# facebookresearch/baspacho

Measured on AMD Instinct MI355X. Metric: factor_gflops_fp64_bal871_schur, higher is better.
Workload: dtype f64; 1 GPU; bal871; description=synthetic BAL-871 stand-in: 871 cams x 9, 527480 pts x 3, 2789783 obs, order=1590279, matrices_per_gpu=1, batch=1, numeric_data=mock: uniform(-1,1) seed 37(+q), damp(0, 1.2*order), as the reference's benches, parallelism=one matrix per GPU x1 (replicas; a single factorisation is not sharded)

## Files before the change

### baspacho_amd/__init__.py

```python
import ctypes
from dataclasses import dataclass
from typing import Optional, Sequence

import numpy as np

from . import _lib

__all__ = ["Settings", "Solver", "Assembly", "create_solver", "SparseStructure", "BackendHip", "BackendCuda",
           "BackendRef", "BackendFast", "AddFillComplete", "AddFillForAutoElims",
           "AddFillForGivenElims", "AddFillNone"]

BackendRef, BackendFast, BackendCuda, BackendHip = 0, 1, 2, 3
AddFillComplete, AddFillForAutoElims, AddFillForGivenElims, AddFillNone = 0, 1, 2, 3

_I64P = ctypes.POINTER(ctypes.c_int64)

_SKEL_IDS = {
    "spanStart": 0, "spanToLump": 1, "lumpStart": 2, "lumpToSpan": 3, "spanOffsetInLump": 4,
    "chainColPtr": 5, "chainRowSpan": 6, "chainData": 7, "chainRowsTillEnd": 8,
    "boardColPtr": 9, "boardRowLump": 10, "boardChainColOrd": 11, "boardRowPtr": 12,
    "boardColLump": 13, "boardColOrd": 14,
}

PROF_KINDS = ["elim_factor", "elim_update", "potrf", "trsm", "update", "chain_update"]


class _CSettings(ctypes.Structure):
    _fields_ = [("find_sparse_elimination_ranges", ctypes.c_int32),
                ("num_threads", ctypes.c_int32), ("backend", ctypes.c_int32),
                ("add_fill_policy", ctypes.c_int32),
                ("computation_model", ctypes.POINTER(ctypes.c_double))]


_HIP_OPTION_INTS = ["lookahead", "due_stream", "split_k", "gather_max_pairs", "gather_overlap",
                    "sub_batch_min", "sub_batches", "tail_blocks", "lazy_plan", "block_solve", "solve_inv",
                    "solve_sweep", "sweep_min_width", "solve_wide", "chain_contraction", "dense_merge", "expected_batch"]
_HIP_OPTION_REALS = ["lookahead_min_gf", "bulk_ahead", "level_cost_us"]


class _CHipOptions(ctypes.Structure):
    _fields_ = [(n, ctypes.c_int32) for n in _HIP_OPTION_INTS] + [(n, ctypes.c_double) for n in _HIP_OPTION_REALS]


class _CPlanStats(ctypes.Structure):
    _fields_ = [(n, ctypes.c_double) for n in
                ["flops", "upd_elems", "upd_flops", "elim_pair_elems", "elim_pair_flops",
                 "elim_col_elems", "upd_flops_direct", "elim_pair_operand_elems",
                 "elim_target_elems", "trsm_flops", "potrf_flops", "trsm_flops_merged",
                 "potrf_flops_fused"]] + \
               [(n, ctypes.c_int64) for n in
                ["num_launches", "num_levels", "num_panels", "num_segs", "num_upd_tasks",
                 "num_trsm_tasks", "chain_tab_entries", "max_panels_in_level",
                 "num_atomic_upd_tasks", "num_gather_groups", "num_fork_levels"]] + \
               [("deferred_flops", ctypes.c_double), ("tail_upd_flops", ctypes.c_double),
                ("num_tail_panels", ctypes.c_int64)]


class _CRunCounters(ctypes.Structure):
    _fields_ = [(n, ctypes.c_int64) for n in
                ["sweep_launches", "sweep_timeouts", "split_lists_used", "sub_batches_enqueued",
                 "lookahead_forks", "sweeps_retired", "sweep_error_pending",
                 "gather_chunks_overlapped", "tail_launches", "sweep_mfma_launches",
                 "solve_wide_launches", "inv_reused", "potrf_folded_levels", "selinv_launches",
                 "selinv_chunks"]]


@dataclass
class Settings:
    findSparseEliminationRanges: bool = True
    numThreads: int = 16
    backend: int = BackendHip
    addFillPolicy: int = AddFillComplete
    computationModel: Optional[Sequence[float]] = None
    hipOptions: Optional[dict] = None


@dataclass
class SparseStructure:
    ptrs: np.ndarray
    inds: np.ndarray

    def __post_init__(self):
        self.ptrs = np.ascontiguousarray(self.ptrs, dtype=np.int64)
        self.inds = np.ascontiguousarray(self.inds, dtype=np.int64)

    def order(self):
        return len(self.ptrs) - 1

    def transpose(self):
        return _ss_op(self, SS_TRANSPOSE)

    def clear(self, clearLower=True):
        return _ss_op(self, SS_CLEAR, flag=int(clearLower))

    def symmetricPermutation(self, mapPerm, lowerHalf=True):
        return _ss_op(self, SS_SYM_PERMUTATION, mapPerm, int(lowerHalf))

    def addIndependentEliminationFill(self, start, end):
        return _ss_op(self, SS_INDEP_ELIM_FILL, [start, end])

    def addFullEliminationFill(self):
        return _ss_op(self, SS_FULL_ELIM_FILL)

    def fillReducingPermutation(self):
        return _ss_op(self, SS_FILL_REDUCING_PERM)

    def extractRightBottom(self, start):
        return _ss_op(self, SS_EXTRACT_RIGHT_BOTTOM, [start])


SS_TRANSPOSE, SS_CLEAR, SS_SYM_PERMUTATION, SS_INDEP_ELIM_FILL, SS_FULL_ELIM_FILL, \
    SS_FILL_REDUCING_PERM, SS_EXTRACT_RIGHT_BOTTOM = range(7)


def _ss_op(ss, op, arg=(), flag=0):
    lib = _lib.load()
    n = ss.order()
    a = _i64(arg)
    cap = max(16, 4 * len(ss.inds) + n)
    while True:
        out_ptrs = np.zeros(n + 2, dtype=np.int64)
        out_inds = np.zeros(cap, dtype=np.int64)
        on, onnz = ctypes.c_int64(0), ctypes.c_int64(0)
        rc = lib.bsp_sparse_structure_op(
            op, ctypes.c_int64(n), ss.ptrs.ctypes.data_as(_I64P), ss.inds.ctypes.data_as(_I64P),
            a.ctypes.data_as(_I64P), ctypes.c_int64(len(a)), ctypes.c_int32(flag),
            out_ptrs.ctypes.data_as(_I64P), out_inds.ctypes.data_as(_I64P), ctypes.c_int64(cap),
            ctypes.byref(on), ctypes.byref(onnz))
        if rc != 0 and onnz.value > cap:
            cap = onnz.value
            continue
        _check(rc)
        if op == SS_FILL_REDUCING_PERM:
            return out_inds[:onnz.value].copy()
        return SparseStructure(out_ptrs[:on.value + 1].copy(), out_inds[:onnz.value].copy())


def _check(rc):
    if rc != 0:
        raise RuntimeError(_lib.load().bsp_last_error().decode("utf-8", "replace"))


def _i64(a):
    return np.ascontiguousarray(a, dtype=np.int64)


def _ptr_of(t):
# ... 85 lines not shown
        _check(self._lib.bsp_skeleton_array(self._h, which, ctypes.byref(p), ctypes.byref(n)))
        if n.value == 0:
            return np.zeros(0, dtype=np.int64)
        return np.ctypeslib.as_array(p, shape=(n.value,)).copy()

    def skel(self):
        if self._skel is None:
            self._skel = {k: self._array(v) for k, v in _SKEL_IDS.items()}
        return self._skel

    def paramToSpan(self):
        return self._array(15)

    def sparseEliminationRanges(self):
        return self._array(16)

    def blockOffset(self, row_param, col_param):
        off, st, fl = ctypes.c_int64(0), ctypes.c_int64(0), ctypes.c_int32(0)
        _check(self._lib.bsp_block_offset(self._h, ctypes.c_int64(row_param),
                                          ctypes.c_int64(col_param), ctypes.byref(off),
                                          ctypes.byref(st), ctypes.byref(fl)))
        return off.value, st.value, bool(fl.value)

    def diagBlockOffset(self, param):
        off, st = ctypes.c_int64(0), ctypes.c_int64(0)
        _check(self._lib.bsp_diag_block_offset(self._h, ctypes.c_int64(param), ctypes.byref(off),
                                               ctypes.byref(st)))
        return off.value, st.value

    def diagBlockOffsetOfSpan(self, span):
        sk = self.skel()
        lump = int(sk["spanToLump"][span])
        idx = span - int(sk["lumpToSpan"][lump])
        off = int(sk["chainData"][int(sk["chainColPtr"][lump]) + idx]) + int(sk["spanOffsetInLump"][span])
        return off, int(sk["lumpStart"][lump + 1] - sk["lumpStart"][lump])

    def deviceAccessor(self):
        arr = (_I64P * 8)()
        _check(self._lib.bsp_device_accessor(self._h, arr))
        return [ctypes.cast(a, ctypes.c_void_p).value for a in arr]

    def setStream(self, stream):
        addr = 0 if stream is None else getattr(stream, "cuda_stream", stream)
        self._lib.bsp_set_stream(self._h, ctypes.c_void_p(addr))
        self._stream = stream

    def _check_data(self, t):
        if t.numel() != self.dataSize():
            raise ValueError("data has %d elements, factor needs %d" % (t.numel(), self.dataSize()))

    def factor(self, data):
        if isinstance(data, (list, tuple)):
            sfx = _suffix(data[0])
            for t in data:
                self._check_data(t)
            ptrs = (ctypes.c_void_p * len(data))(*[_ptr_of(t) for t in data])
            _check(getattr(self._lib, "bsp_factor_batched_" + sfx)(self._h, ptrs,
                                                                   ctypes.c_int32(len(data))))
        else:
            self._check_data(data)
            _check(getattr(self._lib, "bsp_factor_" + _suffix(data))(
                self._h, ctypes.c_void_p(_ptr_of(data))))

    def factorPerOp(self, data):
        self._check_data(data)
        _check(getattr(self._lib, "bsp_factor_per_op_" + _suffix(data))(
            self._h, ctypes.c_void_p(_ptr_of(data))))

    def forcePerOp(self, on=True):
        _check(self._lib.bsp_force_per_op(self._h, ctypes.c_int32(1 if on else 0)))
        solver = self

        class _Scope:
            def __enter__(self_inner):
                return solver

            def __exit__(self_inner, *exc):
                _check(solver._lib.bsp_force_per_op(solver._h, ctypes.c_int32(0)))
                return False
        return _Scope()

    def _testSetFault(self, kind):
        _check(self._lib.bsp_test_set_fault(self._h, ctypes.c_int32(kind)))

    def _testSetSelInvBatchChunk(self, max_matrices):
        _check(self._lib.bsp_test_set_selinv_batch_chunk(self._h, ctypes.c_int32(max_matrices)))

    _SELINV_SMALL_FIELDS = ("lump", "level", "n", "r", "k")
    _SELINV_NODE_FIELDS = ("lump", "level", "c0", "w", "r", "nRest", "kChunk", "nk", "nTiles", "tileBase")

    def _testSelInvPlan(self, upToSpan=None):
        if upToSpan is None:
            def call(buf, cap, need):
                return self._lib.bsp_test_selinv_plan(self._h, buf, cap, need)
        else:
            def call(buf, cap, need):
                return self._lib.bsp_test_selinv_plan_up_to(self._h, ctypes.c_int64(upToSpan), buf, cap, need)
        need = ctypes.c_int64(0)
        _check(call(None, ctypes.c_int64(0), ctypes.byref(need)))
        buf = np.empty(need.value, dtype=np.int64)
        _check(call(buf.ctypes.data_as(_I64P), need, ctypes.byref(need)))
        nlev, ns, nn = (int(x) for x in buf[:3])
        out = {"numLevels": nlev, "linvElems": int(buf[3]), "uElems": int(buf[4]), "pElems": int(buf[5]),
               "wElems": int(buf[6])}
        fs, fn = self._SELINV_SMALL_FIELDS, self._SELINV_NODE_FIELDS
        sm = buf[7:7 + ns * len(fs)].reshape(ns, len(fs))
        nd = buf[7 + ns * len(fs):].reshape(nn, len(fn))
        out["small"] = {f: sm[:, i].copy() for i, f in enumerate(fs)}
        out["node"] = {f: nd[:, i].copy() for i, f in enumerate(fn)}
        return out

    def collectOpStats(self, on=True):
        _check(self._lib.bsp_collect_op_stats(self._h, ctypes.c_int32(1 if on else 0)))

    def opStats(self):
        out = {}
        for which, (name, nsz) in enumerate((("potrf", 1), ("trsm", 2), ("syge", 3), ("asmbl", 2))):
            cnt = ctypes.c_int64(0)
            _check(self._lib.bsp_read_op_stats(self._h, ctypes.c_int32(which), None, ctypes.c_int64(0),
                                               ctypes.byref(cnt)))
            buf = np.zeros((cnt.value, 4))
            if cnt.value:
                _check(self._lib.bsp_read_op_stats(
                    self._h, ctypes.c_int32(which), buf.ctypes.data_as(ctypes.POINTER(ctypes.c_double)),
                    ctypes.c_int64(cnt.value), ctypes.byref(cnt)))
            out[name] = np.concatenate([buf[:, :nsz], buf[:, 3:4]], axis=1)
        return out

    def _factor_partial_batched(self, which, data, span_index):
        for t in data:
            self._check_data(t)
        ptrs = (ctypes.c_void_p * len(data))(*[_ptr_of(t) for t in data])
        _check(getattr(self._lib, "bsp_factor_partial_batched_" + _suffix(data[0]))(
            self._h, ptrs, ctypes.c_int32(len(data)), ctypes.c_int64(span_index), ctypes.c_int32(which)))

    def factorUpTo(self, data, span_index):
        if isinstance(data, (list, tuple)):
            return self._factor_partial_batched(0, data, span_index)
        self._check_data(data)
        _check(getattr(self._lib, "bsp_factor_up_to_" + _suffix(data))(
            self._h, ctypes.c_void_p(_ptr_of(data)), ctypes.c_int64(span_index)))

    def factorFrom(self, data, span_index):
        if isinstance(data, (list, tuple)):
            return self._factor_partial_batched(1, data, span_index)
        self._check_data(data)
        _check(getattr(self._lib, "bsp_factor_from_" + _suffix(data))(
            self._h, ctypes.c_void_p(_ptr_of(data)), ctypes.c_int64(span_index)))

    def doElimination(self, data, elim_range_index):
        self._check_data(data)
        _check(getattr(self._lib, "bsp_do_elimination_" + _suffix(data))(
            self._h, ctypes.c_void_p(_ptr_of(data)), ctypes.c_int64(elim_range_index)))

    def _solve(self, name, mat, vec, stride, nrhs):
        if stride is None:
            stride = self.order()
        if isinstance(mat, (list, tuple)):
            assert isinstance(vec, (list, tuple)) and len(vec) == len(mat)
            for t in mat:
                self._check_data(t)
            which = {"bsp_solve_": 0, "bsp_solve_l_": 1, "bsp_solve_lt_": 2}[name]
            mats = (ctypes.c_void_p * len(mat))(*[_ptr_of(t) for t in mat])
            vecs = (ctypes.c_void_p * len(vec))(*[_ptr_of(t) for t in vec])
            _check(getattr(self._lib, "bsp_solve_batched_" + _suffix(mat[0]))(
                self._h, mats, vecs, ctypes.c_int32(len(mat)), ctypes.c_int64(stride),
# ... 249 lines not shown
            self._check_data(t)
        sfx = _suffix(gs[0])
        if batched:
            def arr(xs):
                return (ctypes.c_void_p * len(xs))(*[_ptr_of(t) for t in xs])
            _check(getattr(self._lib, "bsp_factor_adjoint_up_to_batched_" + sfx)(
                self._h, arr(ps), arr(gs), ctypes.c_int32(len(gs)), ctypes.c_int64(span)))
            return
        _check(getattr(self._lib, "bsp_factor_adjoint_up_to_" + sfx)(
            self._h, ctypes.c_void_p(_ptr_of(ps[0])), ctypes.c_void_p(_ptr_of(gs[0])), ctypes.c_int64(span)))

    def _schur_dense(self, what, name, src, span, out, dest, to_dense):
        import torch
        m = self._schurOrder(span)
        batched = isinstance(src, (list, tuple))
        srcs = list(src) if batched else [src]
        if len(srcs) == 0:
            raise ValueError("%s: empty batch" % what)
        dense_shape, n_dense, n_data = (m, m), m * m, self.dataSize()
        if out is None:
            outs = [torch.empty(dense_shape if to_dense else (n_data,), dtype=t.dtype, device=t.device) for t in srcs]
            out = outs if batched else outs[0]
        batched, (srcs, outs) = self._same_kind(what, "%s and out" % name, src, out)
        for t in srcs:
            if t.numel() != (n_data if to_dense else n_dense):
                raise ValueError("%s: %s has %d elements, expected %d" % (
                    what, name, t.numel(), n_data if to_dense else n_dense))
        for t in outs:
            if t.numel() != (n_dense if to_dense else n_data):
                raise ValueError("%s: out has %d elements, expected %d" % (
                    what, t.numel(), n_dense if to_dense else n_data))
        dp = None
        if dest is not None:
            if dest.dtype != torch.int32 or dest.numel() != m or dest.device != srcs[0].device:
                raise ValueError("%s: dest must be an int32 tensor of %d elements on %s" % (what, m, srcs[0].device))
            dp = _ptr_of(dest)
        sfx = _suffix(srcs[0])
        fn = "bsp_schur_to_dense_" if to_dense else "bsp_schur_from_dense_"
        if batched:
            def arr(xs):
                return (ctypes.c_void_p * len(xs))(*[_ptr_of(t) for t in xs])
            _check(getattr(self._lib, fn + "batched_" + sfx)(
                self._h, arr(srcs), ctypes.c_int64(span), arr(outs), ctypes.c_void_p(dp), ctypes.c_int32(len(outs))))
        else:
            _check(getattr(self._lib, fn + sfx)(
                self._h, ctypes.c_void_p(_ptr_of(srcs[0])), ctypes.c_int64(span), ctypes.c_void_p(_ptr_of(outs[0])),
                ctypes.c_void_p(dp)))
        return out

    def schurComplement(self, P, span, out=None, dest=None):
        return self._schur_dense("schurComplement", "P", P, span, out, dest, True)

    def schurComplementAdjoint(self, gradDense, span, out=None, dest=None):
        return self._schur_dense("schurComplementAdjoint", "gradDense", gradDense, span, out, dest, False)

    def assembly(self, rows, cols, triangle="lower"):
        return Assembly(self, rows, cols, triangle)

    def scalarPermutation(self):
        out = np.empty(self.order(), dtype=np.int64)
        _check(self._lib.bsp_scalar_permutation(self._h, out.ctypes.data_as(_I64P)))
        return out

    def factorFlops(self):
        return float(self._lib.bsp_factor_flops(self._h))

    def planLevels(self):
        self._lib.bsp_plan_levels.restype = ctypes.c_int64
        n = self._lib.bsp_plan_levels(self._h, None, ctypes.c_int64(0))
        if n < 0:
            raise RuntimeError(_lib.load().bsp_last_error().decode("utf-8", "replace"))
        out = np.zeros(n, dtype=np.int64)
        self._lib.bsp_plan_levels(self._h, out.ctypes.data_as(ctypes.POINTER(ctypes.c_int64)), ctypes.c_int64(n))
        return out.reshape(-1, 8)

    def planStats(self):
        st = _CPlanStats()
        _check(self._lib.bsp_plan_stats_full(self._h, ctypes.byref(st)))
        return {n: getattr(st, n) for n, _ in _CPlanStats._fields_}

    def runCounters(self):
        st = _CRunCounters()
        _check(self._lib.bsp_run_counters_get(self._h, ctypes.byref(st)))
        return {n: getattr(st, n) for n, _ in _CRunCounters._fields_}

    def factorProfiled(self, data, in_situ=False, busy=False):
        self._check_data(data)
        ms = (ctypes.c_double * 6)()
        ln = (ctypes.c_int64 * 6)()
        if in_situ and busy:
            bs = (ctypes.c_double * 6)()
            _check(self._lib.bsp_factor_profiled_busy_f64(self._h, ctypes.c_void_p(_ptr_of(data)), ms, ln, bs))
            return {k: (ms[i], ln[i], bs[i]) for i, k in enumerate(PROF_KINDS)}
        fn = self._lib.bsp_factor_profiled_insitu_f64 if in_situ else self._lib.bsp_factor_profiled_f64
        _check(fn(self._h, ctypes.c_void_p(_ptr_of(data)), ms, ln))
        return {k: (ms[i], ln[i]) for i, k in enumerate(PROF_KINDS)}

    def densify(self, data, fill_upper_half=False, start_span_index=0):
        sk = self.skel()
        data = np.asarray(data)
        off = int(sk["spanStart"][start_span_index])
        n = self.order() - off
        dense = np.zeros((n, n), dtype=data.dtype)
        ls, ss = sk["lumpStart"], sk["spanStart"]
        for l in range(int(sk["spanToLump"][start_span_index]), self.numLumps()):
            w = int(ls[l + 1] - ls[l])
            for c in range(int(sk["chainColPtr"][l]), int(sk["chainColPtr"][l + 1])):
                sp = int(sk["chainRowSpan"][c])
                r0, rows = int(ss[sp]) - off, int(ss[sp + 1] - ss[sp])
                d0 = int(sk["chainData"][c])
                dense[r0:r0 + rows, int(ls[l]) - off:int(ls[l]) - off + w] = \
                    data[d0:d0 + rows * w].reshape(rows, w)
        if fill_upper_half:
            dense = np.tril(dense) + np.tril(dense, -1).T
        return dense

    def lowerMask(self):
        sk = self.skel()
        ls = sk["lumpStart"]
        w = (ls[1:] - ls[:-1]).astype(np.int64)
        d0 = sk["chainData"][sk["chainColPtr"][:-1]]
        mask = np.ones(self.dataSize(), dtype=bool)
        for width in np.unique(w):
            if width < 2:
                continue
            i, j = np.triu_indices(int(width), 1)
            upper = (i * width + j).astype(np.int64)
            starts = d0[w == width]
            mask[(starts[:, None] + upper[None, :]).ravel()] = False
        return mask

    def damp(self, data, alpha, beta):
        sk = self.skel()
        ls = sk["lumpStart"]
        w = (ls[1:] - ls[:-1]).astype(np.int64)
        d0 = sk["chainData"][sk["chainColPtr"][:-1]]
        idx = np.concatenate([d0[i] + np.arange(w[i]) * (w[i] + 1) for i in range(len(w))])
        data[idx] = data[idx] * (1 + alpha) + beta
        return data


_TRIANGLES = {"lower": 0, "full": 1}


def _host_indices(a, name):
    if hasattr(a, "detach"):
        a = a.detach().cpu().numpy()
    a = np.asarray(a)
    if a.ndim != 1:
        raise ValueError("assembly: %s must be one-dimensional, got shape %s" % (name, a.shape))
    if a.size and not np.issubdtype(a.dtype, np.integer):
        raise TypeError("assembly: %s must hold integers, got %s" % (name, a.dtype))
    return _i64(a)


class Assembly:

    def __init__(self, solver, rows, cols, triangle="lower"):
        if triangle not in _TRIANGLES:
            raise ValueError("assembly: triangle must be 'lower' or 'full', got %r" % (triangle,))
        self._lib = solver._lib
        self._h = None
        r, c = _host_indices(rows, "rows"), _host_indices(cols, "cols")
        if len(r) != len(c):
            raise ValueError("assembly: %d rows for %d cols" % (len(r), len(c)))
        h = ctypes.c_void_p()
        _check(self._lib.bsp_assembly_create(solver._h, ctypes.c_int64(len(r)), r.ctypes.data_as(_I64P),
                                             c.ctypes.data_as(_I64P), ctypes.c_int32(_TRIANGLES[triangle]),
                                             ctypes.byref(h)))
        self._h = h
        self.solver = solver
        self.nnz = len(r)
        self.triangle = triangle

    def __del__(self):
        h, self._h = getattr(self, "_h", None), None
        if h:
            self._lib.bsp_assembly_destroy(h)

    def entryOffsets(self):
        out = np.empty(self.nnz, dtype=np.int64)
        _check(self._lib.bsp_assembly_entry_offsets(self._h, out.ctypes.data_as(_I64P)))
        return out

    def info(self):
        out = (ctypes.c_int64 * 7)()
        _check(self._lib.bsp_assembly_info(self._h, out))
        keys = ["nnz", "kept", "elements", "max_run", "long_runs", "tiles", "device_bytes"]
        return dict(zip(keys, [int(x) for x in out]))

    def _run(self, name, x, n_in, n_out, out, adjoint):
        import torch
        if not isinstance(x, torch.Tensor):
            raise TypeError("%s: expected a torch.Tensor, got %s" % (name, type(x).__name__))
        if x.dim() not in (1, 2) or x.shape[-1] != n_in:
            raise ValueError("%s: expected [%d] or [B, %d], got shape %s" % (name, n_in, n_in, tuple(x.shape)))
        if x.dim() == 2 and x.shape[0] == 0:
            raise ValueError("%s: empty batch" % name)
        sfx = _suffix(x)
        shape = x.shape[:-1] + (n_out,)
        if out is None:
            out = torch.empty(shape, dtype=x.dtype, device=x.device)
        elif out.shape != shape or out.dtype != x.dtype or out.device != x.device:
            raise ValueError("%s: out must be %s %s on %s, got %s %s on %s" % (
                name, tuple(shape), x.dtype, x.device, tuple(out.shape), out.dtype, out.device))
        _ptr_of(x), _ptr_of(out)
        fn = "bsp_assemble_adjoint_" if adjoint else "bsp_assemble_"
        if x.dim() == 2:
            B_ = x.shape[0]
            ins = (ctypes.c_void_p * B_)(*[x[q].data_ptr() for q in range(B_)])
            outs = (ctypes.c_void_p * B_)(*[out[q].data_ptr() for q in range(B_)])
            _check(getattr(self._lib, fn + "batched_" + sfx)(self.solver._h, self._h, ins, outs,
                                                            ctypes.c_int32(B_)))
        else:
            _check(getattr(self._lib, fn + sfx)(self.solver._h, self._h, ctypes.c_void_p(x.data_ptr()),
                                               ctypes.c_void_p(out.data_ptr())))
        return out

    def assemble(self, values, out=None):
        return self._run("assemble", values, self.nnz, self.solver.dataSize(), out, False)

    def adjoint(self, gradData, out=None):
        return self._run("adjoint", gradData, self.solver.dataSize(), self.nnz, out, True)


def probe_mfma_f64_tflops():
    out = ctypes.c_double(0)
    _check(_lib.load().bsp_probe_mfma_f64(ctypes.byref(out)))
    return out.value


def debug_read_trace(max_records=8192):
    out = np.zeros((max_records, 8), dtype=np.int64)
    n = ctypes.c_int(0)
    _check(_lib.load().bsp_debug_read_trace(out.ctypes.data_as(ctypes.c_void_p), max_records,
                                            ctypes.byref(n)))
    return out[:n.value]


def debug_read_extents(max_launches=2048):
    out = np.zeros((max_launches, 4), dtype=np.uint64)
    n = ctypes.c_int(0)
    _check(_lib.load().bsp_debug_read_extents(out.ctypes.data_as(ctypes.c_void_p), max_launches,
                                              ctypes.byref(n)))
    return out[:n.value]


def create_solver(settings: Optional[Settings], param_sizes, ss: SparseStructure,
                  sparse_elim_ranges=(), elim_last_ids=()) -> Solver:
    lib = _lib.load()
    st = settings or Settings()
    cs = _CSettings(int(st.findSparseEliminationRanges), int(st.numThreads), int(st.backend),
                    int(st.addFillPolicy), None)
    model = None
    if st.computationModel is not None:
        model = (ctypes.c_double * 20)(*[float(x) for x in st.computationModel])
        cs.computation_model = ctypes.cast(model, ctypes.POINTER(ctypes.c_double))
    ps = _i64(param_sizes)
    if len(ps) != ss.order():
        raise ValueError("param_sizes and sparse structure disagree on the number of params")
    er, el = _i64(sparse_elim_ranges), _i64(sorted(elim_last_ids))
    h = ctypes.c_void_p()
    ho = None
    if st.hipOptions:
        ho = _CHipOptions()
        lib.bsp_hip_options_default(ctypes.byref(ho))
        for k, v in st.hipOptions.items():
            if k in _HIP_OPTION_INTS:
                setattr(ho, k, int(v))
            elif k in _HIP_OPTION_REALS:
                setattr(ho, k, float(v))
            else:
                raise ValueError("unknown backend option %r (bsp_hip_options has: %s)" %
                                 (k, ", ".join(_HIP_OPTION_INTS + _HIP_OPTION_REALS)))
    _check(lib.bsp_create_solver_opts(
        ctypes.byref(cs), ctypes.byref(ho) if ho is not None else None,
        ctypes.c_int64(len(ps)), ps.ctypes.data_as(_I64P),
        ss.ptrs.ctypes.data_as(_I64P), ss.inds.ctypes.data_as(_I64P), ctypes.c_int64(len(er)),
        er.ctypes.data_as(_I64P), ctypes.c_int64(len(el)), el.ctypes.data_as(_I64P),
        ctypes.byref(h)))
    return Solver(h)
```

### baspacho_amd/csrc/backend_options.h

```cpp
#pragma once

#include <cmath>
#include <cstdint>

namespace BaSpaCho {

struct HipBackendOptions {
  int32_t lookahead = -1;
  int32_t dueStream = -1;
  int32_t splitK = -1;
  int32_t gatherMaxPairs = -1;
  int32_t gatherOverlap = -1;
  int32_t subBatchMin = -1;
  int32_t subBatches = -1;
  int32_t tailBlocks = -1;
  int32_t lazyPlan = -1;
  int32_t blockSolve = -1;
  int32_t solveInv = -1;
  int32_t solveSweep = -1;
  int32_t sweepMinWidth = -1;
  int32_t solveWide = -1;
  int32_t chainContraction = -1;
  int32_t denseMerge = -1;
  int32_t expectedBatch = -1;
  double lookaheadMinGF = NAN;
  double bulkAhead = NAN;
  double levelCostUs = NAN;

  void applyEnv();
  static bool on(int32_t v, bool dflt) { return v < 0 ? dflt : v != 0; }
};

}
```

### baspacho_amd/csrc/bsp_utils.cpp

```cpp
#include "bsp_utils.h"
#include "backend_options.h"
#include <cstdlib>
#include <algorithm>

#include <chrono>
#include <cmath>
#include <ctime>
#include <iomanip>

namespace BaSpaCho {

void throwError(const char* file, int line, const std::string& msg) {
  using namespace std::chrono;
  auto now = system_clock::now();
  std::time_t tt = system_clock::to_time_t(now);
  struct tm lt;
  localtime_r(&tt, &lt);
  auto ms = duration_cast<milliseconds>(now.time_since_epoch()).count() % 1000;
  std::ostringstream os;
  os << "[" << std::put_time(&lt, "%T") << "." << std::setfill('0') << std::setw(3) << ms << " "
     << file << ":" << line << "] Check failed: " << msg;
  throw std::runtime_error(os.str());
}

int64_t cumSumVec(std::vector<int64_t>& v) {
  int64_t running = 0;
  for (size_t i = 0; i + 1 < v.size(); i++) {
    int64_t cur = v[i];
    v[i] = running;
    running += cur;
  }
  v.back() = running;
  return running;
}

void rewindVec(std::vector<int64_t>& v, int64_t downTo, int64_t value) {
  for (int64_t i = (int64_t)v.size() - 1; i > downTo; i--) v[i] = v[i - 1];
  v[downTo] = value;
}

std::vector<int64_t> inversePermutation(const std::vector<int64_t>& p) {
  std::vector<int64_t> inv(p.size());
  for (size_t i = 0; i < p.size(); i++) inv[p[i]] = (int64_t)i;
  return inv;
}

std::vector<int64_t> composePermutations(const std::vector<int64_t>& v,
                                         const std::vector<int64_t>& w) {
  BASPACHO_CHECK_EQ(v.size(), w.size());
  std::vector<int64_t> out(v.size());
  for (size_t i = 0; i < v.size(); i++) out[i] = v[w[i]];
  return out;
}

std::string secondsToString(double secs, int precision) {
  std::ostringstream os;
  os << std::fixed << std::setprecision(precision);
  if (secs < 1e-3) {
    os << secs * 1e6 << "us";
  } else if (secs < 1.0) {
    os << secs * 1e3 << "ms";
  } else {
    os << secs << "s";
  }
  return os.str();
}

std::string OpStat::toString() const {
  std::ostringstream os;
  os << "#=" << numRuns << ", time=" << secondsToString(totTime)
     << ", last=" << secondsToString(lastTime) << ", max=" << secondsToString(maxTime);
  return os.str();
}

void HipBackendOptions::applyEnv() {
  auto flag = [](const char* name, int32_t& dst, bool invert = false) {
    if (const char* e = std::getenv(name)) dst = ((e[0] != '0') != invert) ? 1 : 0;
  };
  auto num = [](const char* name, int32_t& dst, long lo) {
    if (const char* e = std::getenv(name)) dst = (int32_t)std::max<long>(lo, std::strtol(e, nullptr, 0));
  };
  auto real = [](const char* name, double& dst) {
    if (const char* e = std::getenv(name)) dst = std::atof(e);
  };
  flag("BSP_NO_LOOKAHEAD", lookahead, true);
  flag("BSP_DUE_STREAM", dueStream);
  flag("BSP_SPLIT_K", splitK);
  num("BSP_GATHER_MAX_PAIRS", gatherMaxPairs, 8);
  flag("BSP_GATHER_OVERLAP", gatherOverlap);
  num("BSP_SUB_BATCH_MIN", subBatchMin, 0);
  num("BSP_SUB_BATCHES", subBatches, 2);
  num("BSP_TAIL_BLOCKS", tailBlocks, 0);
  if (std::getenv("BSP_LAZY_PLAN")) lazyPlan = 1;
  flag("BSP_BLOCK_SOLVE", blockSolve);
  flag("BSP_SOLVE_INV", solveInv);
  flag("BSP_SOLVE_SWEEP", solveSweep);
  num("BSP_SWEEP_MIN_WIDTH", sweepMinWidth, 1);
  flag("BSP_SOLVE_WIDE", solveWide);
  flag("BSP_CHAIN_CONTRACTION", chainContraction);
  if (std::getenv("BSP_DENSE_MERGE_OFF")) denseMerge = 0;
  num("BSP_EXPECTED_BATCH", expectedBatch, 1);
  real("BSP_LOOKAHEAD_MIN_GF", lookaheadMinGF);
  real("BSP_BULK_AHEAD", bulkAhead);
  real("BSP_LEVEL_COST_US", levelCostUs);
}

}
```

### baspacho_amd/csrc/c_api.cpp

```cpp
#include "../../include/baspacho_amd.h"

#include <cmath>
#include <cstring>
#include <numeric>
#include <string>
#include <unordered_map>
#include <unordered_set>

#include "assembly.h"
#include "bal_pipeline.h"
#include "../../include/baspacho_amd_testing.h"
#include "computation_model.h"
#include "hip_backend.h"
#include "hip_plan.h"
#include "solver.h"

using namespace BaSpaCho;

struct bsp_solver {
  SolverPtr solver;
  ComputationModel model;
  int64_t balOk[3] = {-1, -1, -1};
};

static thread_local std::string g_lastError;

const char* bsp_last_error(void) { return g_lastError.c_str(); }
const char* bsp_version(void) { return "baspacho_amd 0.1 (gfx950)"; }

#define BSP_TRY try {
#define BSP_CATCH                      \
  }                                    \
  catch (const std::exception& e) {    \
    g_lastError = e.what();            \
    return 1;                          \
  }                                    \
  catch (...) {                        \
    g_lastError = "unknown exception"; \
    return 1;                          \
  }                                    \
  return 0;

void bsp_hip_options_default(bsp_hip_options* o) {
  o->lookahead = o->due_stream = o->split_k = o->gather_max_pairs = o->gather_overlap = o->sub_batch_min =
      o->sub_batches = o->tail_blocks = o->lazy_plan = o->block_solve = o->solve_inv = o->solve_sweep =
          o->sweep_min_width = o->solve_wide = o->chain_contraction = o->dense_merge = o->expected_batch = -1;
  o->lookahead_min_gf = o->bulk_ahead = o->level_cost_us = NAN;
}

int bsp_create_solver_opts(const bsp_settings* st, const bsp_hip_options* ho, int64_t numParams,
                           const int64_t* paramSizes, const int64_t* ptrs, const int64_t* inds,
                           int64_t numElimRanges, const int64_t* elimRanges, int64_t numElimLast,
                           const int64_t* elimLast, bsp_solver** out) {
  BSP_TRY
  BASPACHO_CHECK_NOTNULL(out);
  std::unique_ptr<bsp_solver> h(new bsp_solver);
  Settings settings;
  HipBackendOptions options;
  if (ho) {
    options.lookahead = ho->lookahead;
    options.dueStream = ho->due_stream;
    options.splitK = ho->split_k;
    options.gatherMaxPairs = ho->gather_max_pairs;
    options.gatherOverlap = ho->gather_overlap;
    options.subBatchMin = ho->sub_batch_min;
    options.subBatches = ho->sub_batches;
    options.tailBlocks = ho->tail_blocks;
    options.lazyPlan = ho->lazy_plan;
    options.blockSolve = ho->block_solve;
    options.solveInv = ho->solve_inv;
    options.solveSweep = ho->solve_sweep;
    options.sweepMinWidth = ho->sweep_min_width;
    options.solveWide = ho->solve_wide;
    options.chainContraction = ho->chain_contraction;
    options.denseMerge = ho->dense_merge;
    options.expectedBatch = ho->expected_batch;
    options.lookaheadMinGF = ho->lookahead_min_gf;
    options.bulkAhead = ho->bulk_ahead;
    options.levelCostUs = ho->level_cost_us;
    settings.hipOptions = &options;
  }
  if (st) {
    settings.findSparseEliminationRanges = st->find_sparse_elimination_ranges != 0;
    settings.numThreads = st->num_threads;
    settings.backend = (BackendType)st->backend;
    settings.addFillPolicy = (AddFillPolicy)st->add_fill_policy;
    if (st->computation_model) {
      const double* p = st->computation_model;
      std::copy(p, p + 4, h->model.potrfParams.begin());
      std::copy(p + 4, p + 10, h->model.trsmParams.begin());
      std::copy(p + 10, p + 16, h->model.sygeParams.begin());
      std::copy(p + 16, p + 20, h->model.asmblParams.begin());
      settings.computationModel = &h->model;
    }
  }
  std::vector<int64_t> sizes(paramSizes, paramSizes + numParams);
  SparseStructure ss(std::vector<int64_t>(ptrs, ptrs + numParams + 1),
                     std::vector<int64_t>(inds, inds + ptrs[numParams]));
  std::vector<int64_t> ranges(elimRanges, elimRanges + (elimRanges ? numElimRanges : 0));
  std::unordered_set<int64_t> last(elimLast, elimLast + (elimLast ? numElimLast : 0));
  h->solver = createSolver(settings, sizes, ss, ranges, last);
  *out = h.release();
  BSP_CATCH
}

int bsp_create_solver(const bsp_settings* st, int64_t numParams, const int64_t* paramSizes,
                      const int64_t* ptrs, const int64_t* inds, int64_t numElimRanges,
                      const int64_t* elimRanges, int64_t numElimLast, const int64_t* elimLast,
                      bsp_solver** out) {
  return bsp_create_solver_opts(st, nullptr, numParams, paramSizes, ptrs, inds, numElimRanges, elimRanges,
                                numElimLast, elimLast, out);
}

int bsp_create_solver_from_skeleton(int64_t numSpans, const int64_t* spanStart, int64_t numLumps,
                                    const int64_t* lumpToSpan, const int64_t* colPtr,
                                    const int64_t* rowInd, int64_t numElimRanges,
                                    const int64_t* elimRanges, bsp_solver** out) {
  BSP_TRY
  BASPACHO_CHECK_NOTNULL(out);
  std::vector<int64_t> ss(spanStart, spanStart + numSpans + 1);
  std::vector<int64_t> l2s(lumpToSpan, lumpToSpan + numLumps + 1);
  std::vector<int64_t> cp(colPtr, colPtr + numLumps + 1);
  std::vector<int64_t> ri(rowInd, rowInd + colPtr[numLumps]);
  std::vector<int64_t> ranges(elimRanges, elimRanges + (elimRanges ? numElimRanges : 0));
  CoalescedBlockMatrixSkel skel(ss, l2s, cp, ri);
  std::unique_ptr<bsp_solver> h(new bsp_solver);
  h->solver.reset(new Solver(std::move(skel), std::move(ranges), {}, hipOps()));
  *out = h.release();
  BSP_CATCH
}

void bsp_destroy_solver(bsp_solver* s) { delete s; }

int64_t bsp_order(const bsp_solver* s) { return s->solver->order(); }
int64_t bsp_data_size(const bsp_solver* s) { return s->solver->dataSize(); }
int64_t bsp_num_spans(const bsp_solver* s) { return s->solver->skel().numSpans(); }
int64_t bsp_num_lumps(const bsp_solver* s) { return s->solver->skel().numLumps(); }
int64_t bsp_can_factor_up_to_span(const bsp_solver* s) { return s->solver->canFactorUpToSpan(); }
int64_t bsp_span_vector_offset(const bsp_solver* s, int64_t span) {
  return s->solver->spanVectorOffset(span);
}
int64_t bsp_span_matrix_offset(const bsp_solver* s, int64_t span, int64_t* out) {
  BSP_TRY
  *out = s->solver->spanMatrixOffset(span);
  BSP_CATCH
}

int bsp_skeleton_array(const bsp_solver* s, int which, const int64_t** data, int64_t* len) {
  BSP_TRY
  const CoalescedBlockMatrixSkel& k = s->solver->skel();
  const std::vector<int64_t>* v = nullptr;
  switch (which) {
    case BSP_SKEL_SPAN_START: v = &k.spanStart; break;
    case BSP_SKEL_SPAN_TO_LUMP: v = &k.spanToLump; break;
    case BSP_SKEL_LUMP_START: v = &k.lumpStart; break;
    case BSP_SKEL_LUMP_TO_SPAN: v = &k.lumpToSpan; break;
    case BSP_SKEL_SPAN_OFFSET_IN_LUMP: v = &k.spanOffsetInLump; break;
    case BSP_SKEL_CHAIN_COL_PTR: v = &k.chainColPtr; break;
    case BSP_SKEL_CHAIN_ROW_SPAN: v = &k.chainRowSpan; break;
// ... 72 lines not shown
  s->solver->factor(&v);
  BSP_CATCH
}
int bsp_factor_batched_f32(bsp_solver* s, float* const* ptrs, int32_t batch) {
  BSP_TRY
  std::vector<float*> v(ptrs, ptrs + batch);
  s->solver->factor(&v);
  BSP_CATCH
}
int bsp_factor_up_to_f64(bsp_solver* s, double* d, int64_t span) {
  BSP_TRY
  s->solver->factorUpTo(d, span);
  BSP_CATCH
}
int bsp_factor_from_f64(bsp_solver* s, double* d, int64_t span) {
  BSP_TRY
  s->solver->factorFrom(d, span);
  BSP_CATCH
}
int bsp_factor_up_to_f32(bsp_solver* s, float* d, int64_t span) {
  BSP_TRY
  s->solver->factorUpTo(d, span);
  BSP_CATCH
}
int bsp_factor_from_f32(bsp_solver* s, float* d, int64_t span) {
  BSP_TRY
  s->solver->factorFrom(d, span);
  BSP_CATCH
}

template <typename T>
static void factorPerOp(bsp_solver* s, T* d) {
  SymbolicCtx& sym = s->solver->internalSymbolicContext();
  hipBackendForcePerOp(sym, true);
  try {
    s->solver->factor(d);
  } catch (...) {
    hipBackendForcePerOp(sym, false);
    throw;
  }
  hipBackendForcePerOp(sym, false);
}
int bsp_factor_per_op_f64(bsp_solver* s, double* d) {
  BSP_TRY
  factorPerOp(s, d);
  BSP_CATCH
}
int bsp_factor_per_op_f32(bsp_solver* s, float* d) {
  BSP_TRY
  factorPerOp(s, d);
  BSP_CATCH
}

int bsp_collect_op_stats(bsp_solver* s, int32_t on) {
  BSP_TRY
  SymbolicCtx& sym = s->solver->internalSymbolicContext();
  s->solver->enableStats(on != 0);
  s->solver->resetStats();
  for (OpStat* st : {&sym.potrfStat, &sym.trsmStat, &sym.sygeStat, &sym.asmblStat}) st->keepSamples = on != 0;
  BSP_CATCH
}
int bsp_read_op_stats(bsp_solver* s, int32_t which, double* out, int64_t capacity, int64_t* count) {
  BSP_TRY
  SymbolicCtx& sym = s->solver->internalSymbolicContext();
  const OpStat* sts[4] = {&sym.potrfStat, &sym.trsmStat, &sym.sygeStat, &sym.asmblStat};
  BASPACHO_CHECK(which >= 0 && which < 4);
  const auto& v = sts[which]->samples;
  *count = (int64_t)v.size();
  for (int64_t i = 0; i < std::min<int64_t>(capacity, (int64_t)v.size()); i++) {
    for (int j = 0; j < 4; j++) out[4 * i + j] = v[i][j];
  }
  BSP_CATCH
}

int bsp_force_per_op(bsp_solver* s, int32_t on) {
  BSP_TRY
  hipBackendForcePerOp(s->solver->internalSymbolicContext(), on != 0);
  BSP_CATCH
}

int bsp_test_read_sweep_trace(bsp_solver* s, long long* out, int32_t max_blocks, int32_t* n_blocks) {
  BSP_TRY
  *n_blocks = hipBackendReadSweepTrace(s->solver->internalSymbolicContext(), out, max_blocks);
  BSP_CATCH
}

int bsp_test_set_fault(bsp_solver* s, int32_t kind) {
  BSP_TRY
  hipBackendSetFault(s->solver->internalSymbolicContext(), kind);
  BSP_CATCH
}

static int selinvPlanRecords(const bsp_solver* s, bool upTo, int64_t span, int64_t* buf, int64_t capacity,
                             int64_t* needed);
int bsp_test_selinv_plan(const bsp_solver* s, int64_t* buf, int64_t capacity, int64_t* needed) {
  return selinvPlanRecords(s, false, 0, buf, capacity, needed);
}
int bsp_test_selinv_plan_up_to(const bsp_solver* s, int64_t span, int64_t* buf, int64_t capacity, int64_t* needed) {
  return selinvPlanRecords(s, true, span, buf, capacity, needed);
}
static int selinvPlanRecords(const bsp_solver* s, bool upTo, int64_t span, int64_t* buf, int64_t capacity,
                             int64_t* needed) {
  BSP_TRY
  const CoalescedBlockMatrixSkel& sk = s->solver->skel();
  const SelInvPlanHost p =
      upTo ? buildSelInvPlan(sk, s->solver->partialCutLump("bsp_test_selinv_plan_up_to", span)) : buildSelInvPlan(sk);
  std::unordered_map<int64_t, int64_t> lumpOfOff;
  for (int64_t l = 0; l < sk.numLumps(); l++) lumpOfOff[sk.chainData[sk.chainColPtr[l]]] = l;
  std::vector<int64_t> out = {(int64_t)p.levels.size(), (int64_t)p.smalls.size(), (int64_t)p.nodes.size(),
                              p.linvElems, p.uElems, p.pElems, p.wElems};
  for (int64_t lv = 0; lv < (int64_t)p.levels.size(); lv++) {
    const SelInvLevel& L = p.levels[lv];
    for (int64_t i = L.smallBegin; i < L.smallEnd; i++) {
      const SelInvSmall& q = p.smalls[i];
      out.insert(out.end(), {lumpOfOff.at(q.diagOff), lv, (int64_t)q.n, (int64_t)q.r, (int64_t)q.k});
    }
  }
  for (int64_t lv = 0; lv < (int64_t)p.levels.size(); lv++) {
    const SelInvLevel& L = p.levels[lv];
    for (int64_t i = L.nodeBegin; i < L.nodeEnd; i++) {
      const SelInvNode& q = p.nodes[i];
      out.insert(out.end(), {lumpOfOff.at(q.lumpOff), lv, (int64_t)q.c0, (int64_t)q.w, (int64_t)q.r,
                             (int64_t)q.nRest, (int64_t)q.kChunk, (int64_t)q.nk, (int64_t)q.nTiles,
                             (int64_t)q.tileBase});
    }
  }
  *needed = (int64_t)out.size();
  if (buf != nullptr) std::copy(out.begin(), out.begin() + std::min(capacity, *needed), buf);
  BSP_CATCH
}

template <typename T>
static void doElim(bsp_solver* s, T* d, int64_t idx) {
  const auto& ranges = s->solver->sparseEliminationRanges();
  BASPACHO_CHECK(idx >= 0 && idx + 1 < (int64_t)ranges.size());
  NumericCtxPtr<T> ctx = s->solver->internalSymbolicContext().createNumericCtx<T>(0, d);
  ctx->doElimination(s->solver->internalGetElimCtx((size_t)idx), d, ranges[idx], ranges[idx + 1]);
}
int bsp_do_elimination_f64(bsp_solver* s, double* d, int64_t idx) {
  BSP_TRY
  doElim(s, d, idx);
  BSP_CATCH
}
int bsp_do_elimination_f32(bsp_solver* s, float* d, int64_t idx) {
  BSP_TRY
  doElim(s, d, idx);
  BSP_CATCH
}

int bsp_solve_f64(bsp_solver* s, const double* m, double* v, int64_t stride, int32_t nrhs) {
  BSP_TRY
  s->solver->solve(m, v, stride, nrhs);
  BSP_CATCH
}
int bsp_solve_l_f64(bsp_solver* s, const double* m, double* v, int64_t stride, int32_t nrhs) {
  BSP_TRY
  s->solver->solveL(m, v, stride, nrhs);
  BSP_CATCH
}
int bsp_solve_lt_f64(bsp_solver* s, const double* m, double* v, int64_t stride, int32_t nrhs) {
  BSP_TRY
  s->solver->solveLt(m, v, stride, nrhs);
  BSP_CATCH
}
int bsp_solve_f32(bsp_solver* s, const float* m, float* v, int64_t stride, int32_t nrhs) {
  BSP_TRY
// ... 537 lines not shown
  BSP_CATCH
}
int bsp_bal_fill_hessian_se3_f32(bsp_solver* s, int64_t numPts, int64_t numCams, int64_t numObs,
                                 const int64_t* obsCam, const int64_t* obsPt, const double* Jc,
                                 const double* Jp, const double* res, float lambda, float* data,
                                 float* grad, void* stream) {
  BSP_TRY
  checkBalLayout(s, numPts, numCams, 6);
  balFillHessian<float>(s->solver->deviceAccessor(), 6, numPts, numCams, numObs, obsCam, obsPt, Jc, Jp,
                        res, lambda, data, grad, nullptr, stream);
  BSP_CATCH
}

double bsp_factor_flops(const bsp_solver* s) { return s->solver->factorFlops(); }

int64_t bsp_plan_levels(bsp_solver* s, int64_t* out, int64_t capacity) {
  try {
    std::vector<int64_t> v = hipBackendPlanLevels(s->solver->internalSymbolicContext(), 0,
                                                  s->solver->skel().numLumps());
    const int64_t n = (int64_t)v.size();
    if (out) std::copy(v.begin(), v.begin() + std::min(n, capacity), out);
    return n;
  } catch (const std::exception& e) {
    g_lastError = e.what();
    return -1;
  }
}

int bsp_plan_stats_full(bsp_solver* s, bsp_plan_stats* out) {
  BSP_TRY
  HipPlanStats p = hipBackendPlanStats(s->solver->internalSymbolicContext(), 0,
                                       s->solver->skel().numLumps());
  out->flops = p.flops;
  out->upd_elems = p.updElems;
  out->upd_flops = p.updFlops;
  out->elim_pair_elems = p.elimPairElems;
  out->elim_pair_flops = p.elimPairFlops;
  out->elim_col_elems = p.elimColElems;
  out->upd_flops_direct = p.updFlopsDirect;
  out->elim_pair_operand_elems = p.elimPairOperandElems;
  out->elim_target_elems = p.elimTargetElems;
  out->trsm_flops = p.trsmFlops;
  out->potrf_flops = p.potrfFlops;
  out->trsm_flops_merged = p.trsmFlopsMerged;
  out->potrf_flops_fused = p.potrfFlopsFused;
  out->num_launches = p.numLaunches;
  out->num_levels = p.numLevels;
  out->num_panels = p.numPanels;
  out->num_segs = p.numSegs;
  out->num_upd_tasks = p.numUpdTasks;
  out->num_trsm_tasks = p.numTrsmTasks;
  out->chain_tab_entries = p.chainTabEntries;
  out->max_panels_in_level = p.maxPanelsInLevel;
  out->num_atomic_upd_tasks = p.numAtomicUpdTasks;
  out->num_gather_groups = p.numGatherGroups;
  out->num_fork_levels = p.numForkLevels;
  out->deferred_flops = p.deferredFlops;
  out->tail_upd_flops = p.tailUpdFlops;
  out->num_tail_panels = p.numTailPanels;
  BSP_CATCH
}

int bsp_run_counters_get(bsp_solver* s, bsp_run_counters* out) {
  BSP_TRY
  const HipRunCounters c = hipBackendRunCounters(s->solver->internalSymbolicContext());
  out->sweep_launches = c.sweepLaunches;
  out->sweep_timeouts = c.sweepTimeouts;
  out->split_lists_used = c.splitListsUsed;
  out->sub_batches_enqueued = c.subBatchesEnqueued;
  out->lookahead_forks = c.lookaheadForks;
  out->sweeps_retired = c.sweepsRetired;
  out->sweep_error_pending = c.sweepErrorPending;
  out->gather_chunks_overlapped = c.gatherChunksOverlapped;
  out->tail_launches = c.tailLaunches;
  out->sweep_mfma_launches = c.sweepMfmaLaunches;
  out->solve_wide_launches = c.solveWideLaunches;
  out->inv_reused = c.invReused;
  out->potrf_folded_levels = c.potrfFoldedLevels;
  out->selinv_launches = c.selinvLaunches;
  out->selinv_chunks = c.selinvChunks;
  BSP_CATCH
}

int bsp_probe_mfma_f64(double* tflops) {
  BSP_TRY
  *tflops = hipBackendMfmaF64ProbeTflops();
  BSP_CATCH
}

int bsp_debug_read_extents(unsigned long long* out, int max_launches, int* n) {
  BSP_TRY
  *n = hipBackendReadExtents(out, max_launches);
  BSP_CATCH
}
int bsp_debug_read_trace(long long* out, int max_records, int* n_records) {
  BSP_TRY
  *n_records = hipBackendReadTrace(out, max_records);
  BSP_CATCH
}

static void factorProfiled(bsp_solver* s, double* d, bool inSitu, double ms[6], int64_t launches[6],
                           double* busy = nullptr) {
  HipKernelProfile prof;
  SymbolicCtx& sym = s->solver->internalSymbolicContext();
  hipBackendSetProfile(sym, &prof, inSitu);
  try {
    s->solver->factor(d);
  } catch (...) {
    hipBackendSetProfile(sym, nullptr);
    throw;
  }
  hipBackendSetProfile(sym, nullptr);
  for (int i = 0; i < kProfNumKinds; i++) {
    ms[i] = prof.ms[i];
    launches[i] = prof.launches[i];
    if (busy) busy[i] = prof.busyMs[i];
  }
}
int bsp_factor_profiled_f64(bsp_solver* s, double* d, double ms[6], int64_t launches[6]) {
  BSP_TRY
  factorProfiled(s, d, false, ms, launches);
  BSP_CATCH
}
int bsp_factor_profiled_insitu_f64(bsp_solver* s, double* d, double ms[6], int64_t launches[6]) {
  BSP_TRY
  factorProfiled(s, d, true, ms, launches);
  BSP_CATCH
}
int bsp_factor_profiled_busy_f64(bsp_solver* s, double* d, double ms[6], int64_t launches[6],
                                 double busy_ms[6]) {
  BSP_TRY
  factorProfiled(s, d, true, ms, launches, busy_ms);
  BSP_CATCH
}

static const int64_t kPlanMagic = 0x42535041434d4431LL;

int bsp_plan_serialize(const bsp_solver* s, int64_t* buf, int64_t capacity, int64_t* needed) {
  BSP_TRY
  const CoalescedBlockMatrixSkel& k = s->solver->skel();
  const auto& ranges = s->solver->sparseEliminationRanges();
  const auto& perm = s->solver->paramToSpan();
  const int64_t nSpans = k.numSpans(), nLumps = k.numLumps();
  const int64_t nRow = (int64_t)k.chainRowSpan.size(), nRanges = (int64_t)ranges.size();
  const int64_t total = 6 + (nSpans + 1) + (nLumps + 1) + (nLumps + 1) + nRow + nRanges + nSpans;
  *needed = total;
  if (!buf || capacity < total) return 0;
  int64_t* p = buf;
  *p++ = kPlanMagic;
  *p++ = s->solver->canFactorUpToSpan();
  *p++ = nSpans;
  *p++ = nLumps;
  *p++ = nRow;
  *p++ = nRanges;
  p = std::copy(k.spanStart.begin(), k.spanStart.end(), p);
  p = std::copy(k.lumpToSpan.begin(), k.lumpToSpan.end(), p);
  p = std::copy(k.chainColPtr.begin(), k.chainColPtr.end(), p);
  p = std::copy(k.chainRowSpan.begin(), k.chainRowSpan.end(), p);
  p = std::copy(ranges.begin(), ranges.end(), p);
  p = std::copy(perm.begin(), perm.end(), p);
  BSP_CATCH
}

int bsp_create_solver_from_plan(const int64_t* buf, int64_t len, bsp_solver** out) {
  BSP_TRY
  BASPACHO_CHECK_NOTNULL(out);
// ... 68 lines not shown
```

### baspacho_amd/csrc/hip_backend.h

```cpp
#pragma once

#include <cstdint>
#include <vector>

#include "mat_ops.h"

namespace BaSpaCho {

enum HipProfKind {
  kProfElimFactor = 0,
  kProfElimUpdate = 1,
  kProfPotrf = 2,
  kProfTrsm = 3,
  kProfUpdate = 4,
  kProfChainUpdate = 5,
  kProfNumKinds = 6
};

struct HipKernelProfile {
  double ms[kProfNumKinds] = {0, 0, 0, 0, 0, 0};
  int64_t launches[kProfNumKinds] = {0, 0, 0, 0, 0, 0};
  double busyMs[kProfNumKinds] = {0, 0, 0, 0, 0, 0};
};

struct HipPlanStats {
  double flops = 0, updElems = 0, updFlops = 0, elimPairElems = 0, elimPairFlops = 0,
         elimColElems = 0, updFlopsDirect = 0, elimPairOperandElems = 0, elimTargetElems = 0,
         trsmFlops = 0, potrfFlops = 0, trsmFlopsMerged = 0, potrfFlopsFused = 0;
  int64_t numLaunches = 0, numLevels = 0, numPanels = 0, numSegs = 0, numUpdTasks = 0,
          numTrsmTasks = 0, chainTabEntries = 0, maxPanelsInLevel = 0, numAtomicUpdTasks = 0,
          numGatherGroups = 0,
          numForkLevels = 0;
  double deferredFlops = 0;
  double tailUpdFlops = 0;
  int64_t numTailPanels = 0;
};

void hipBackendSetProfile(SymbolicCtx& sym, HipKernelProfile* prof, bool inSitu = false);

double hipBackendMfmaF64ProbeTflops();
int hipBackendReadTrace(long long* out, int maxRecords);
int hipBackendReadExtents(unsigned long long* out, int maxLaunches);

void hipBackendForcePerOp(SymbolicCtx& sym, bool on);

void hipBackendSetFault(SymbolicCtx& sym, int kind);

struct HipRunCounters {
  int64_t sweepLaunches = 0;
  int64_t sweepTimeouts = 0;
  int64_t splitListsUsed = 0;
  int64_t subBatchesEnqueued = 0;
  int64_t lookaheadForks = 0;
  int64_t gatherChunksOverlapped = 0;
  int64_t tailLaunches = 0;
  int64_t solveWideLaunches = 0;
  int64_t invReused = 0;
  int64_t potrfFoldedLevels = 0;
  int64_t sweepMfmaLaunches = 0;
  int64_t sweepsRetired = 0;
  int64_t sweepErrorPending = 0;
  int64_t selinvLaunches = 0;
  int64_t selinvChunks = 0;
};
HipRunCounters hipBackendRunCounters(SymbolicCtx& sym);
int hipBackendReadSweepTrace(SymbolicCtx& sym, long long* out, int maxBlocks);

std::vector<int64_t> hipBackendPlanLevels(SymbolicCtx& sym, int64_t startLump, int64_t upToLump);

template <typename T>
void hipBackendSelectedInverse(SymbolicCtx& sym, T* data);
template <typename T>
void hipBackendSelectedInverse(SymbolicCtx& sym, const std::vector<T*>& data);
void hipBackendSetSelInvBatchChunk(SymbolicCtx& sym, int64_t maxMatrices);

template <typename T>
void hipBackendLogDet(SymbolicCtx& sym, const T* const* factors, int64_t batch, bool single, T* out);
template <typename T>
struct HipGradArgs {
  int64_t batch = 1;
  bool single = true;
  const T* const* z = nullptr;
  const T* zScale = nullptr;
  const T* const* u = nullptr;
  const T* const* v = nullptr;
  int64_t ld = 0;
  int nRHS = 0;
  T alpha = T(0);
  T* const* out = nullptr;
  bool outer = false;
};
template <typename T>
void hipBackendPatternGrad(SymbolicCtx& sym, const HipGradArgs<T>& a);
template <typename T>
void hipBackendFactorAdjoint(SymbolicCtx& sym, const T* const* L, T* const* grad, int64_t batch, bool single);
template <typename T>
void hipBackendFactorAdjointUpTo(SymbolicCtx& sym, const T* const* P, T* const* grad, int64_t batch, bool single,
                                 int64_t upToLump);
template <typename T>
void hipBackendSchurDense(SymbolicCtx& sym, const T* const* in, T* const* out, int64_t batch, bool single,
                          int64_t fromLump, const int32_t* dest, bool toDense);

struct AssemblyMap;
struct HipAssemblyDev;
template <typename T>
void hipBackendAssemble(SymbolicCtx& sym, const AssemblyMap& map, const T* const* in, T* const* out,
                        int64_t batch, bool single, bool adjoint);
void hipBackendFreeAssembly(HipAssemblyDev* dev);

HipPlanStats hipBackendPlanStats(SymbolicCtx& sym, int64_t startLump, int64_t upToLump);

}
```

### baspacho_amd/csrc/hip_backend.hip

```cpp
#include <hip/hip_runtime.h>

#include <atomic>
#include <cstdlib>
#include <cstring>
#include <map>
#include <mutex>

#include "backend_options.h"
#include "hip_backend.h"
#include "hip_kernels.h"
#include "hip_solve_kernels.h"
#include "hip_sweep_kernels.h"
#include "hip_solve_wide.h"
#include "hip_sweep_mfma.h"
#include "hip_tail_kernel.h"
#include "hip_selinv_kernels.h"
#include "hip_chol_adjoint_kernels.h"
#include "hip_grad_kernels.h"
#include "hip_assembly_kernels.h"
#include "mat_ops.h"

namespace BaSpaCho {

using std::vector;

#define hipCHECK(expr)                                                                    \
  do {                                                                                    \
    hipError_t bsp_err_ = (expr);                                                         \
    if (bsp_err_ != hipSuccess) {                                                         \
      throw std::runtime_error(std::string("HIP error: ") + hipGetErrorString(bsp_err_) + \
                               " in " #expr " (" __FILE__ ":" + std::to_string(__LINE__) + ")"); \
    }                                                                                     \
  } while (0)

namespace {

struct DevBuf {
  void* ptr = nullptr;
  size_t bytes = 0;
  DevBuf() {}
  DevBuf(const DevBuf&) = delete;
  DevBuf& operator=(const DevBuf&) = delete;
  DevBuf(DevBuf&& o) noexcept : ptr(o.ptr), bytes(o.bytes) { o.ptr = nullptr; o.bytes = 0; }
  ~DevBuf() { release(); }
  void release() {
    if (ptr) (void)hipFree(ptr);
    ptr = nullptr;
    bytes = 0;
  }
  void resize(size_t n) {
    if (n <= bytes) return;
    release();
    hipCHECK(hipMalloc(&ptr, n));
    bytes = n;
  }
  template <typename U>
  void upload(const vector<U>& v) {
    resize(std::max<size_t>(v.size() * sizeof(U), 16));
    if (!v.empty()) hipCHECK(hipMemcpy(ptr, v.data(), v.size() * sizeof(U), hipMemcpyHostToDevice));
  }
  template <typename U>
  const U* as() const { return reinterpret_cast<const U*>(ptr); }
};

}

struct HipAssemblyDev {
  DevBuf entryOff, tileFirst, tileLongFirst, runStart, runEntry, destLocal, longDest;
  void upload(const AssemblyMap& m) {
    entryOff.upload(m.entryOff);
    tileFirst.upload(m.tileFirst);
    tileLongFirst.upload(m.tileLongFirst);
    runStart.upload(m.runStart);
    runEntry.upload(m.runEntry);
    destLocal.upload(m.destLocal);
    longDest.upload(m.longDest);
  }
};

namespace {

struct SolveSchedItem {
  enum Kind : int32_t { kLevel = 0, kBlockGroup = 1, kSweep = 2 };
  int32_t kind = kLevel;
  int32_t slot = -1;
  int64_t l = 0, e = 0;
  hipk::SweepDesc sweep{};
  int32_t sweepFwdWgs = 0, sweepBwdWgs = 0;
};
struct SolveInvList {
  bool built = false;
  int64_t count = 0;
  DevBuf list;
  vector<SolveSchedItem> items;
  int32_t numSweeps = 0;
  int64_t sweepInstStride = 0;
  int64_t maxSweepWgs = 0, maxSweepWgsM = 0;
  int32_t maxSweepW = 0, maxSweepBelow = 0;
};

struct DevPlan {
  HipPlanHost host;
  std::map<std::pair<const void*, int>, SolveInvList> solveInvLists;
// ... 370 lines not shown
    partSlices = n;
  }
};

struct SelInvScratch {
  DevBuf linv, dd, U, P, Wp;
  int64_t linvCap = 0, uCap = 0, pCap = 0, wCap = 0;
  bool allocated = false;
  void release() {
    allocated = false;
    for (DevBuf* b : {&linv, &dd, &U, &P, &Wp}) b->release();
    linvCap = uCap = pCap = wCap = 0;
  }
  int64_t slicesFor(const SelInvPlanHost& h) const {
    if (!allocated) return 0;
    int64_t n = INT64_MAX;
    const auto fit = [&n](int64_t cap, int64_t elems) {
      if (elems > 0) n = std::min(n, cap / elems);
    };
    fit(linvCap, h.linvElems);
    fit(uCap, h.uElems);
    fit(pCap, h.pElems);
    fit(wCap, h.wElems);
    return n;
  }
  void reserve(const SelInvPlanHost& h, int64_t n) {
    if (n <= slicesFor(h)) return;
    if (allocated) hipCHECK(hipDeviceSynchronize());
    allocated = false;
    for (DevBuf* b : {&linv, &dd, &U, &P, &Wp}) b->release();
    const int64_t lc = std::max(linvCap, h.linvElems * n), uc = std::max(uCap, h.uElems * n);
    const int64_t pc = std::max(pCap, h.pElems * n), wc = std::max(wCap, h.wElems * n);
    linvCap = uCap = pCap = wCap = 0;
    const auto bytes = [](int64_t elems) { return (size_t)std::max<int64_t>(elems, 1) * sizeof(double); };
    linv.resize(bytes(lc));
    dd.resize(bytes(lc));
    U.resize(bytes(uc));
    P.resize(bytes(pc));
    Wp.resize(bytes(wc));
    linvCap = lc, uCap = uc, pCap = pc, wCap = wc;
    allocated = true;
  }
};

struct SelInvDev {
  SelInvPlanHost host;
  DevBuf smalls, nodes, tiles, zTasks, rowChain, rowLocal, pairOff, pairStr;
  SelInvScratch* scratch = nullptr;
  hipk::SelInvStrides strides() const { return {host.linvElems, host.uElems, host.pElems, host.wElems}; }
  int64_t sliceBytes() const {
    return (2 * host.linvElems + host.uElems + host.pElems + host.wElems) * (int64_t)sizeof(double);
  }
  int64_t slices() const { return scratch->slicesFor(host); }
  void reserve(int64_t n) { scratch->reserve(host, n); }
  void upload(SelInvScratch* sc) {
    scratch = sc;
    smalls.upload(host.smalls);
    nodes.upload(host.nodes);
    tiles.upload(host.tiles);
    zTasks.upload(host.zTasks);
    rowChain.upload(host.rowChain);
    rowLocal.upload(host.rowLocal);
    pairOff.upload(host.pairOff);
    pairStr.upload(host.pairStr);
    reserve(1);
  }
};

struct HipSymbolicCtx : SymbolicCtx {
  HipSymbolicCtx(const CoalescedBlockMatrixSkel& skel_, const vector<int64_t>& permutation_,
                 const HipBackendOptions& o)
      : skel(skel_), permutation(permutation_) {
    lookaheadEnabled = HipBackendOptions::on(o.lookahead, true);
    blockSolve = HipBackendOptions::on(o.blockSolve, true);
    solveInv = HipBackendOptions::on(o.solveInv, true);
    if (o.subBatchMin >= 0) subBatchMin = o.subBatchMin == 0 ? INT32_MAX : std::max(2, o.subBatchMin);
    if (o.subBatches >= 0) subBatchParts = std::max(2, o.subBatches);
    splitK = HipBackendOptions::on(o.splitK, true);
    sweepEnabled = HipBackendOptions::on(o.solveSweep, true);
    solveWide = HipBackendOptions::on(o.solveWide, true);
    gatherOverlap = HipBackendOptions::on(o.gatherOverlap, false);
    if (o.sweepMinWidth >= 0) sweepMinWidth = std::max(1, o.sweepMinWidth);
    lazyPlan = HipBackendOptions::on(o.lazyPlan, false);
    if (!std::isnan(o.lookaheadMinGF)) lookaheadMinFlops = 1e9 * o.lookaheadMinGF;
    planOpts.dueStream = HipBackendOptions::on(o.dueStream, planOpts.dueStream);
    if (o.gatherMaxPairs >= 0) planOpts.gatherMaxPairs = std::max(8, o.gatherMaxPairs);
    if (!std::isnan(o.bulkAhead)) planOpts.bulkAhead = o.bulkAhead;
    if (o.tailBlocks >= 0) planOpts.tailBlocks = o.tailBlocks;
    planOpts.gatherOverlap = gatherOverlap;
    planOpts.applyDeveloperEnv();
    if (const char* e = std::getenv("BSP_TAIL_FLAGS")) tailFlags = std::atoi(e);
    if (const char* e = std::getenv("BSP_GATHER_OVERLAP_LDS")) gatherOverlapLds = (unsigned)std::max(0, std::atoi(e));
    if (const char* e = std::getenv("BSP_SWEEP_TRACE")) sweepTraceOn = e[0] != '0';
    if (const char* e = std::getenv("BSP_SWEEP_MFMA_MIN")) sweepMfmaMinRhs = std::max(1, std::atoi(e));
    if (const char* e = std::getenv("BSP_SWEEP_MFMA_MIN_WIDTH")) sweepMfmaMinWidth = std::max(0, std::atoi(e));
    if (const char* e = std::getenv("BSP_SOLVE_WIDE_MIN")) solveWideMinRhs = std::max(2, std::atoi(e));
    if (const char* e = std::getenv("BSP_POTRF_IN_TRSM")) potrfInTrsm = e[0] != '0';
    if (const char* e = std::getenv("BSP_TAIL_IN_BATCH")) tailInBatch = e[0] != '0';
    if (const char* e = std::getenv("BSP_FOLD_MAX_TILES")) foldMaxTiles = std::min<int64_t>(DevPlan::kFoldMaxTiles, std::max(1, std::atoi(e)));
  }

  virtual ~HipSymbolicCtx() override {
    for (hipEvent_t e : events) (void)hipEventDestroy(e);
    if (sweepHostErr) (void)hipHostFree(sweepHostErr);
  }

  virtual void setSparseElimRanges(const vector<int64_t>& ranges) override {
    sparseElimRanges = ranges;
    plans.clear();
  }

  virtual void prepareFactor(int64_t upToLump) override {
    try {
      prepareDevice(upToLump);
    } catch (const std::exception&) {
      (void)hipGetLastError();
      releaseDeviceState();
      device = -1;
      eagerOnly = false;
      inPrepare = false;
    }
  }

  void releaseDeviceState() {
    plans.clear();
    selinv.reset();
    selinvUpTo.clear();
    selinvScratch.release();
    grad.reset();
    for (hipEvent_t e : events) (void)hipEventDestroy(e);
    events.clear();
    nextEvent = 0;
    dinvScratch.release();
    rawScratch.release();
    yieldBuf.release();
    solveInvScratch.release();
    sweepXchg.release();
    tailCtl.release();
    tailDinv.release();
    for (DevBuf* b : {&dSpanStart, &dSpanToLump, &dLumpStart, &dSpanOffsetInLump, &dChainColPtr,
                      &dChainRowSpan, &dChainData, &dChainRowsTillEnd, &dBoardColPtr,
                      &dBoardChainColOrd, &dPermutation}) {
      b->release();
    }
    skelUploaded = false;
    shared = nullptr;
    sweepAttr[0] = sweepAttr[1] = 0;
  }

  void prepareDevice(int64_t upToLump) {
    int count = 0;
    if (hipGetDeviceCount(&count) != hipSuccess || count <= 0) {
      (void)hipGetLastError();
      return;
    }
    if (lazyPlan) return;
    struct Scope {
      bool& f;
      explicit Scope(bool& f_) : f(f_) { f = true; }
      ~Scope() { f = false; }
    } scope(inPrepare);
    if (upToLump <= 0) return;
    DevPlan& plan = planFor(sparseElimRanges, 0, upToLump, 0);
    ensureSkelOnDevice();
    (void)streams();
    (void)yieldWord();
    dinvScratch.resize((size_t)hipk::kDinvBatchStride * sizeof(double));
    if (plan.host.maxChainRows > 0) {
      rawScratch.resize((size_t)2 * plan.host.maxChainRows * kTile * sizeof(double));
    }
    const size_t wantEvents = 8 + 4 * (size_t)plan.host.numForkLevels;
    while (events.size() < wantEvents) {
      hipEvent_t e;
      hipCHECK(hipEventCreateWithFlags(&e, hipEventDisableTiming));
      events.push_back(e);
    }
    {
      hipStream_t warm = nullptr;
      hipCHECK(hipStreamCreateWithFlags(&warm, hipStreamNonBlocking));
      hipk::warmupKernel<<<1, 64, 0, warm>>>();
      const hipError_t werr = hipStreamSynchronize(warm);
      (void)hipStreamDestroy(warm);
      hipCHECK(werr);
    }
    eagerOnly = true;
  }

  virtual void setStream(void* s) override { stream = (hipStream_t)s; }

  void checkDevice() {
    int cur = -1;
    hipCHECK(hipGetDevice(&cur));
    if (device < 0) device = cur;
    if (cur != device && eagerOnly) {
      releaseDeviceState();
      device = cur;
    }
    if (!inPrepare) eagerOnly = false;
    if (cur != device) {
      throw std::runtime_error("HIP backend: this Solver was first used on device " +
                               std::to_string(device) + " but the current device is " +
                               std::to_string(cur) + " (make its device current before the call)");
    }
  }

  void ensureSkelOnDevice() {
    if (skelUploaded) return;
    checkDevice();
    dSpanStart.upload(skel.spanStart);
    dSpanToLump.upload(skel.spanToLump);
    dLumpStart.upload(skel.lumpStart);
    dSpanOffsetInLump.upload(skel.spanOffsetInLump);
    dChainColPtr.upload(skel.chainColPtr);
    dChainRowSpan.upload(skel.chainRowSpan);
    dChainData.upload(skel.chainData);
    dChainRowsTillEnd.upload(skel.chainRowsTillEnd);
    dBoardColPtr.upload(skel.boardColPtr);
    dBoardChainColOrd.upload(skel.boardChainColOrd);
    dPermutation.upload(permutation);
    skelUploaded = true;
  }

  hipk::SkelDev skelDev() {
    ensureSkelOnDevice();
    hipk::SkelDev d;
    d.spanStart = dSpanStart.as<int64_t>();
    d.spanToLump = dSpanToLump.as<int64_t>();
    d.lumpStart = dLumpStart.as<int64_t>();
    d.spanOffsetInLump = dSpanOffsetInLump.as<int64_t>();
    d.chainColPtr = dChainColPtr.as<int64_t>();
    d.chainRowSpan = dChainRowSpan.as<int64_t>();
    d.chainData = dChainData.as<int64_t>();
    d.chainRowsTillEnd = dChainRowsTillEnd.as<int64_t>();
    d.boardColPtr = dBoardColPtr.as<int64_t>();
    d.boardChainColOrd = dBoardChainColOrd.as<int64_t>();
    return d;
  }

  virtual PermutedCoalescedAccessor deviceAccessor() override {
    ensureSkelOnDevice();
    PermutedCoalescedAccessor acc;
    acc.init(dSpanStart.as<int64_t>(), dSpanToLump.as<int64_t>(), dLumpStart.as<int64_t>(),
             dSpanOffsetInLump.as<int64_t>(), dChainColPtr.as<int64_t>(),
             dChainRowSpan.as<int64_t>(), dChainData.as<int64_t>(), dPermutation.as<int64_t>());
    return acc;
  }

  virtual SymElimCtxPtr prepareElimination(int64_t lumpsBegin, int64_t lumpsEnd) override {
    HipSymElimCtx* e = new HipSymElimCtx;
    e->lumpsBegin = lumpsBegin;
    e->lumpsEnd = lumpsEnd;
    return SymElimCtxPtr(e);
  }

  template <typename T>
// ... 273 lines not shown
      p->upload(&selinvScratch);
      slot = std::move(p);
    }
    return *slot;
  }

  template <typename T>
  void selInvLevels(const SelInvDev& d, hipk::DataRef<T> data, unsigned nMats) {
    const hipk::SkelDev sk = skelDev();
    const hipk::SelInvStrides st = d.strides();
    T* linv = reinterpret_cast<T*>(d.scratch->linv.ptr);
    T* dd = reinterpret_cast<T*>(d.scratch->dd.ptr);
    T* U = reinterpret_cast<T*>(d.scratch->U.ptr);
    T* P = reinterpret_cast<T*>(d.scratch->P.ptr);
    T* Wp = reinterpret_cast<T*>(d.scratch->Wp.ptr);
    const SelInvNode* nodes = d.nodes.as<SelInvNode>();
    const int2* tiles = d.tiles.as<int2>();
    const int4* zTasks = d.zTasks.as<int4>();
    int64_t launches = 0;
    for (const SelInvLevel& L : d.host.levels) {
      if (L.smallEnd > L.smallBegin) {
        hipk::selinvSmallLumps<T><<<dim3((unsigned)(L.smallEnd - L.smallBegin), nMats), 64, 0, stream>>>(
            d.smalls.as<SelInvSmall>() + L.smallBegin, sk, data);
        launches++;
      }
      const unsigned nNodes = (unsigned)(L.nodeEnd - L.nodeBegin);
      if (nNodes == 0) continue;
      const SelInvNode* nd = nodes + L.nodeBegin;
      hipk::selinvDiagInverse<T><<<dim3(nNodes, nMats), 256, 0, stream>>>(nd, data, linv, dd, st);
      const unsigned nTiles = (unsigned)(L.tileEnd - L.tileBegin);
      if (nTiles > 0) {
        hipk::selinvFormU<T><<<dim3(nTiles, nMats), 256, 0, stream>>>(nd, tiles + L.tileBegin, data, linv, U, st);
        hipk::selinvZrrTimesU<T><<<dim3((unsigned)(L.zEnd - L.zBegin), nMats), 256, 0, stream>>>(
            nd, zTasks + L.zBegin, d.rowChain.as<int32_t>(), d.rowLocal.as<int32_t>(),
            d.pairOff.as<int64_t>(), d.pairStr.as<int32_t>(), data, U, P, st);
        hipk::selinvReduceZ<T><<<dim3(nTiles, nMats), 256, 0, stream>>>(nd, tiles + L.tileBegin, data, U, P, Wp, st);
        launches += 3;
      }
      hipk::selinvDiagBlock<T><<<dim3(nNodes, nMats), 256, 0, stream>>>(nd, data, dd, Wp, st);
      launches += 2;
    }
    counters.selinvLaunches += launches;
    counters.selinvChunks++;
  }

  DevPlan& planFor(const vector<int64_t>& ranges, int64_t startLump, int64_t upToLump, int tag) {
    checkDevice();
    auto key = std::make_tuple(tag, startLump, upToLump);
    auto it = plans.find(key);
    if (it == plans.end()) {
      std::unique_ptr<DevPlan> p(new DevPlan);
      HipPlanOptions po = planOpts;
      if (tag == 2) po.tailBlocks = 0;
      p->host = buildHipPlan(skel, ranges, startLump, upToLump, po);
      p->upload();
      it = plans.emplace(key, std::move(p)).first;
    }
    return *it->second;
  }

  virtual NumericCtxBase* createNumericCtxForType(std::type_index tIdx, int64_t tempBufSize,
                                                  int batchSize) override;

  virtual SolveCtxBase* createSolveCtxForType(std::type_index tIdx, int nRHS,
                                              int batchSize) override;

  SharedStreams& streams() {
    if (!shared) {
      checkDevice();
      shared = &sharedStreams();
    }
    return *shared;
  }
  hipStream_t sideStream() { return streams().side; }
  unsigned* yieldWord() {
    if (!yieldBuf.ptr) {
      const size_t bytes = 256;
      yieldBuf.resize(bytes);
      hipCHECK(hipMemset(yieldBuf.ptr, 0, bytes));
    }
    return reinterpret_cast<unsigned*>(yieldBuf.ptr);
  }
  hipStream_t dueSideStream() { return streams().due; }
  hipEvent_t eventFromPool() {
    if (nextEvent == events.size()) {
      hipEvent_t e;
      hipCHECK(hipEventCreateWithFlags(&e, hipEventDisableTiming));
      events.push_back(e);
    }
    return events[nextEvent++];
  }
  void resetEventPool() { nextEvent = 0; }

  const CoalescedBlockMatrixSkel& skel;
  vector<int64_t> permutation;
  vector<int64_t> sparseElimRanges;
  hipStream_t stream = nullptr;
  HipKernelProfile* profile = nullptr;
  bool profileInSitu = false;
  bool lookaheadEnabled = true;
  bool lazyPlan = false;
  static constexpr unsigned bulkExtraLds = 6 * 1024, dueExtraLds = 6 * 1024;
  bool forcePerOp = false;
  bool faultDropElimUpdate = false;
  SharedStreams* shared = nullptr;
  HipPlanOptions planOpts;
  double lookaheadMinFlops = HipPlanHost::kMinDeferredFlopsPerFork;
  bool blockSolve = true;
  bool tailInBatch = false;
  bool potrfInTrsm = true;
  int64_t foldMaxTiles = 512;
  bool splitK = true;
  unsigned gatherOverlapLds = 0;
  bool gatherOverlap = false;
  static constexpr int64_t splitKMaxWgs = 1024;
  int subBatchMin = 16;
  int subBatchParts = 2;
  vector<hipEvent_t> events;
  size_t nextEvent = 0;
  int device = -1;
  bool inPrepare = false;
  bool eagerOnly = false;
  int traceLaunchId = 0;
  DevBuf dinvScratch, rawScratch, yieldBuf;
  DevBuf solveInvScratch;
  uint64_t solveInvGen = 0;
  bool solveInv = true;
  bool sweepEnabled = true;
  int sweepMinWidth = 768;
  int sweepMfmaMinWidth = 7000;
  int sweepMfmaMinRhs = 8;
  bool sweepBroken = false;
  int sweepFault = 0;
  double sweepSpinLimitS = 2.0;
  int tailFlags = 1;
  DevBuf tailCtl, tailDinv;
  bool solveWide = true;
  int solveWideMinRhs = 2;
  size_t solveWideMaxBytes = (size_t)1 << 30;
  DevBuf solveWideBuf;
  DevBuf sweepXchg;
  DevBuf sweepTrace;
  bool sweepTraceOn = false;
  unsigned* sweepHostErr = nullptr;
  unsigned* sweepHostErrDev = nullptr;
  int sweepCapacity = 0;
  size_t sweepMaxLds = 0;
  int sweepAttr[2] = {0, 0};
  struct RunCounters {
    int64_t sweepLaunches = 0, sweepTimeouts = 0, splitListsUsed = 0, subBatchesEnqueued = 0,
            lookaheadForks = 0, gatherChunksOverlapped = 0, tailLaunches = 0, sweepMfmaLaunches = 0, invReused = 0, solveWideLaunches = 0, potrfFoldedLevels = 0;
    int64_t selinvLaunches = 0, selinvChunks = 0;
  } counters;
  void checkAsyncError() {
    if (sweepHostErr && *reinterpret_cast<volatile unsigned*>(sweepHostErr) != 0u) {
      *reinterpret_cast<volatile unsigned*>(sweepHostErr) = 0u;
      sweepBroken = true;
      counters.sweepTimeouts++;
      if (planOpts.tailBlocks > 0) {
        (void)hipDeviceSynchronize();
        planOpts.tailBlocks = 0;
        plans.clear();
      }
      throw std::runtime_error(
          "HIP backend: a persistent launch (solve sweep / factor tail) of an EARLIER call on this "
          "Solver timed out (watchdog); the result of that call is invalid.  The persistent kernels "
          "are retired for this Solver: it takes the multi-launch paths from now on");
    }
  }
  bool sweepUsable() {
    checkAsyncError();
    return sweepEnabled && !sweepBroken && solveInv && blockSolve;
  }
  long long* tailTrace() {
    if (!sweepTraceOn) return nullptr;
    if (!sweepTrace.ptr) {
      sweepTrace.resize(8 * 4096 * sizeof(long long));
      hipCHECK(hipMemset(sweepTrace.ptr, 0, 8 * 4096 * sizeof(long long)));
    }
    return reinterpret_cast<long long*>(sweepTrace.ptr);
  }
  unsigned* asyncErrWord() {
    if (!sweepHostErr) {
      void* hp = nullptr;
      hipCHECK(hipHostMalloc(&hp, 64, hipHostMallocMapped));
      sweepHostErr = reinterpret_cast<unsigned*>(hp);
      *sweepHostErr = 0u;
      void* dp = nullptr;
      hipCHECK(hipHostGetDevicePointer(&dp, hp, 0));
      sweepHostErrDev = reinterpret_cast<unsigned*>(dp);
    }
    return sweepHostErrDev;
  }
  template <typename BT>
  bool sweepReady() {
    int& st = sweepAttr[sizeof(BT) == 8 ? 0 : 1];
    if (st == 0) {
      st = -1;
      checkDevice();
      hipDeviceProp_t prop;
      if (hipGetDeviceProperties(&prop, device) == hipSuccess) {
        sweepCapacity = prop.multiProcessorCount;
        sweepMaxLds = std::min<size_t>(prop.maxSharedMemoryPerMultiProcessor, 160 * 1024) - 1024;
        const int lds = (int)sweepMaxLds;
        bool ok = hipFuncSetAttribute(reinterpret_cast<const void*>(&hipk::solveSweep<BT, false>),
                                      hipFuncAttributeMaxDynamicSharedMemorySize, lds) == hipSuccess;
        ok = ok && hipFuncSetAttribute(reinterpret_cast<const void*>(&hipk::solveSweep<BT, true>),
                                       hipFuncAttributeMaxDynamicSharedMemorySize, lds) == hipSuccess;
        ok = ok && hipFuncSetAttribute(reinterpret_cast<const void*>(&hipk::solveSweepM<BT, false>),
                                       hipFuncAttributeMaxDynamicSharedMemorySize, lds) == hipSuccess;
        ok = ok && hipFuncSetAttribute(reinterpret_cast<const void*>(&hipk::solveSweepM<BT, true>),
                                       hipFuncAttributeMaxDynamicSharedMemorySize, lds) == hipSuccess;
        if (ok && !sweepHostErr) {
          void* hp = nullptr;
          ok = hipHostMalloc(&hp, 64, hipHostMallocMapped) == hipSuccess;
          if (ok) {
            sweepHostErr = reinterpret_cast<unsigned*>(hp);
            *sweepHostErr = 0u;
            void* dp = nullptr;
            ok = hipHostGetDevicePointer(&dp, hp, 0) == hipSuccess;
            sweepHostErrDev = reinterpret_cast<unsigned*>(dp);
          }
        }
        if (ok) st = 1;
      }
      if (st < 0) (void)hipGetLastError();
    }
    return st > 0;
  }
#ifndef BSP_UPD_PREFETCH_MAX_WGS
#define BSP_UPD_PREFETCH_MAX_WGS 2048
#endif
  static constexpr int64_t updPrefetchMaxWgs = BSP_UPD_PREFETCH_MAX_WGS;
  PtrRing ptrRing;
  std::map<std::pair<int64_t, int64_t>, std::pair<std::unique_ptr<DevBuf>, size_t>> addMvTileLists;

  bool skelUploaded = false;
  DevBuf dSpanStart, dSpanToLump, dLumpStart, dSpanOffsetInLump, dChainColPtr, dChainRowSpan,
      dChainData, dChainRowsTillEnd, dBoardColPtr, dBoardChainColOrd, dPermutation;
  std::map<std::tuple<int, int64_t, int64_t>, std::unique_ptr<DevPlan>> plans;
  std::unique_ptr<SelInvDev> selinv;
  std::map<int64_t, std::unique_ptr<SelInvDev>> selinvUpTo;
  SelInvScratch selinvScratch;
  std::unique_ptr<GradDev> grad;
  int64_t selInvChunkCap = 0;
};

template <typename T>
struct HipNumericCtx : NumericCtx<T> {
  using BT = BaseType<T>;

  HipNumericCtx(HipSymbolicCtx& sym_, int batchSize_, int64_t tempBufSize_)
      : sym(sym_), batchSize(batchSize_), tempBufSize(std::max<int64_t>(tempBufSize_, 1)) {}

  hipk::DataRef<BT> makeRef(T* data);

  void launchUpdate(DevPlan& plan, int64_t begin, int64_t end, hipk::DataRef<BT> ref,
                    hipStream_t stream, BT* altTarget = nullptr, int64_t altStride = 0,
                    unsigned extraLds = 0, int atomicMask = 1) {
    if (altTarget == nullptr && end < (int64_t)plan.slowPrefix.size() &&
        plan.slowPrefix[end] == plan.slowPrefix[begin]) {
      const unsigned pad = extraLds ? extraLds + 3072 : 0;
      const unsigned* yf = (extraLds && batchSize == 1) ? sym.yieldWord() : nullptr;
      hipk::updateTileBulk<BT><<<dim3((unsigned)(end - begin), (unsigned)batchSize), 256, pad,
                                stream>>>(plan.updTasksFat.as<UpdTaskFat>() + begin, ref, yf, atomicMask);
      return;
    }
    const int64_t wgs = (end - begin) * (int64_t)batchSize;
    const bool few = wgs <= sym.updPrefetchMaxWgs;
    auto kern = few ? hipk::updateTile<BT, true> : hipk::updateTile<BT, false>;
    kern<<<dim3((unsigned)(end - begin), (unsigned)batchSize), 256, extraLds, stream>>>(
        plan.updTasksWide.as<UpdTaskWide>() + begin,
        plan.chainOffTab.as<int64_t>(), plan.rowChain.as<int32_t>(), plan.rowLocal.as<int32_t>(),
        plan.rowColOff.as<int32_t>(), ref, altTarget, altStride, atomicMask);
  }

  bool lookaheadOn() const {
    return (sym.profile == nullptr || sym.profileInSitu) && sym.lookaheadEnabled;
  }

  void launchLevels(DevPlan& plan, const vector<LevelRange>& levels, hipk::DataRef<BT> ref,
                    LaunchTimer& timer) {
    const dim3 gy(1, (unsigned)batchSize, 1);
    const bool lookahead = lookaheadOn() && plan.host.lookaheadPays(batchSize, sym.lookaheadMinFlops);
    vector<hipEvent_t> defDone(levels.size(), nullptr);
    vector<hipEvent_t> optDone(levels.size(), nullptr);
    const bool dueStream = plan.host.opts.dueStream && sizeof(BT) == 8;
    const int sideMask = dueStream ? 3 : 1;
    int64_t nFold = 0;
    if (sym.potrfInTrsm && &levels == &plan.host.levels) {
      while (nFold < (int64_t)plan.foldTiles.size() &&
             plan.foldTiles[nFold] * (int64_t)batchSize <= sym.foldMaxTiles) {
        nFold++;
      }
    }
    auto prevFork = [&](int64_t f) -> int64_t { return f >= 0 ? levels[f].waitDefLevel : -1; };
    auto waitDeferred = [&](int64_t f) {
      if (f < 0 || !defDone[f]) return;
      hipCHECK(hipStreamWaitEvent(sym.stream, defDone[f], 0));
      const int64_t pf = prevFork(f);
      if (dueStream && pf >= 0 && optDone[pf]) hipCHECK(hipStreamWaitEvent(sym.stream, optDone[pf], 0));
    };
    bool potrfFused = false;
    bool sideUsed = false, dueUsed = false;
    const int64_t scratchBatch = std::max<int64_t>(batchSize, subBatchTotal);
    sym.dinvScratch.resize((size_t)scratchBatch * hipk::kDinvBatchStride * sizeof(BT));
    BT* dinvBase = const_cast<BT*>(sym.dinvScratch.as<BT>()) + (size_t)subBatchBase * hipk::kDinvBatchStride;
    int dinvSlot = 0;
    const int64_t rawSlot = plan.host.maxChainRows * kTile;
    BT* rawBase = nullptr;
    if (rawSlot > 0) {
      sym.rawScratch.resize((size_t)scratchBatch * 2 * rawSlot * sizeof(BT));
      rawBase = const_cast<BT*>(sym.rawScratch.as<BT>()) + (size_t)subBatchBase * 2 * rawSlot;
    }
    bool rawValid = false;
    int extraApplied = 0;
    bool extraBroken = false;
    const bool chunks = &levels == &plan.host.levels && !gatherChunkDone.empty();
    int waitedExec = 0, waitedDue = 0, waitedSide = 0;
    hipEvent_t lastOpt = nullptr;
    auto waitChunk = [&](hipStream_t st, int& waited, int32_t chunk) {
      if (!chunks || chunk <= waited || chunk >= (int32_t)gatherChunkDone.size()) return;
      hipCHECK(hipStreamWaitEvent(st, gatherChunkDone[chunk], 0));
      waited = chunk;
    };
    for (size_t li = 0; li < levels.size(); li++) {
      const LevelRange& lr = levels[li];
      const unsigned nP = (unsigned)(lr.panelEnd - lr.panelBegin);
      const unsigned nT = (unsigned)(lr.trsmEnd - lr.trsmBegin);
      const bool direct = lr.directPanel >= 0;
      waitChunk(sym.stream, waitedExec, lr.gatherNow);
      if (lr.tail) {
        if (lr.tail == 1) {
          auto joinStream = [&](hipStream_t st) {
            hipEvent_t e = sym.eventFromPool();
            hipCHECK(hipEventRecord(e, st));
            hipCHECK(hipStreamWaitEvent(sym.stream, e, 0));
          };
          if (sideUsed) joinStream(sym.sideStream());
          if (dueUsed) joinStream(sym.dueSideStream());
          sideUsed = dueUsed = false;
          const PanelDesc& p0 = plan.host.panels[lr.directPanel];
          hipk::TailDesc td;
          td.diagOff = p0.diagOff;
          td.lda = p0.lda;
          td.K = p0.nb + p0.nRest;
          td.nP = (td.K + kTile - 1) / kTile;
          td.ctlStride = hipk::tailCtlWords(td.nP);
          td.flags = sym.tailFlags;
          td.pad = 0;
          BASPACHO_CHECK_EQ(td.nP, lr.tailPanels);
          const size_t ctlBytes = ((size_t)td.ctlStride * scratchBatch * sizeof(unsigned) + 255) / 256 * 256;
          const size_t xchPerMat = (size_t)td.nP * kTile * kTile * sizeof(BT);
          sym.tailCtl.resize(ctlBytes + xchPerMat * scratchBatch);
          sym.tailDinv.resize((size_t)scratchBatch * td.nP * hipk::kDinvSlot * sizeof(BT));
          unsigned* ctl = reinterpret_cast<unsigned*>(sym.tailCtl.ptr) + (size_t)subBatchBase * td.ctlStride;
          BT* xch = reinterpret_cast<BT*>(reinterpret_cast<char*>(sym.tailCtl.ptr) + ctlBytes + xchPerMat * subBatchBase);
          BT* tdinv = const_cast<BT*>(sym.tailDinv.as<BT>()) + (size_t)subBatchBase * td.nP * hipk::kDinvSlot;
          if (subBatchTotal > 0) {
            hipCHECK(hipMemsetAsync(ctl, 0xff, (size_t)td.ctlStride * batchSize * sizeof(unsigned), sym.stream));
            hipCHECK(hipMemsetAsync(xch, 0xff, xchPerMat * batchSize, sym.stream));
          } else {
            hipCHECK(hipMemsetAsync(sym.tailCtl.ptr, 0xff, ctlBytes + xchPerMat * scratchBatch, sym.stream));
          }
          timer.begin(kProfChainUpdate);
          hipk::tailFactor<BT><<<dim3((unsigned)hipk::tailRoles(td.nP), gy.y), 256, 0, sym.stream>>>(
              td, ref, tdinv, ctl, xch, sym.asyncErrWord(), (long long)(sym.sweepSpinLimitS * 1e8), sym.tailTrace());
          timer.end();
          sym.counters.tailLaunches++;
        }
        rawValid = false;
        potrfFused = false;
        continue;
      }
      const int slot = dinvSlot;
      dinvSlot ^= 1;
      BT* dinvCur = dinvBase + slot * hipk::kDinvSlot;
      BT* dinvNext = dinvBase + (slot ^ 1) * hipk::kDinvSlot;
      BT* rawCur = rawBase ? rawBase + slot * rawSlot : nullptr;
      BT* rawNext = rawBase ? rawBase + (slot ^ 1) * rawSlot : nullptr;
      const bool fold = nFold > 0 && !potrfFused && plan.foldRank[li] >= 0 && plan.foldRank[li] < nFold;
      if (potrfFused) {
        potrfFused = false;
      } else if (fold) {
        sym.counters.potrfFoldedLevels++;
      } else if (nP) {
        timer.begin(kProfPotrf);
        if (direct) {
          hipk::potrfPanelDirect<BT><<<dim3(1, gy.y), 256, 0, sym.stream>>>(
              plan.host.panels[lr.directPanel], ref, dinvCur);
        } else {
          hipk::potrfPanel<BT><<<dim3(nP, gy.y), 256, 0, sym.stream>>>(
              plan.levelPanelDescs.as<PanelDesc>() + lr.panelBegin, ref);
        }
        timer.end();
      }
      const bool fuse = direct && lr.directSeg >= 0 && lr.fuseNext && li + 1 < levels.size() &&
                        levels[li + 1].directPanel >= 0 && lr.updEnd > lr.updBegin;
      int splitK = (fuse && nT) ? lr.splitK : 0;
      const bool directUpd = direct && lr.directSeg >= 0 && lr.updEnd > lr.updBegin;
      const bool stage = rawBase && directUpd && lr.rawNext && li + 1 < levels.size() &&
                         levels[li + 1].directPanel >= 0;
      const PanelDesc nextPanel = (stage || fuse) ? plan.host.panels[levels[li + 1].directPanel]
                                                  : PanelDesc{};
      bool merged = false;
      int64_t memOff = 0;
      int kMem = 0;
      if (rawValid && directUpd && nT) {
        const SegDesc& sd = plan.host.segs[lr.directSeg];
        const SrcDesc& sr = plan.host.srcs[sd.src];
        const PanelDesc& pdc = plan.host.panels[lr.directPanel];
        if (!sd.outer && sr.K == pdc.nb) {
          merged = true;
        } else if (sd.outer == 1 && sr.K > pdc.nb && (sr.K - pdc.nb) % kTile == 0 &&
                   sr.rowsBelow == pdc.rowsBelow && sr.lda == pdc.lda) {
          merged = true;
          memOff = sr.off;
          kMem = sr.K - pdc.nb;
        }
      }
      if (merged) splitK = 0;
      bool waitedDef = false;
      if (splitK && lookahead && lr.waitDefLevel >= 0 && defDone[lr.waitDefLevel]) {
        waitDeferred(lr.waitDefLevel);
        waitedDef = true;
      }
      if (nT && !merged) {
        timer.begin(kProfTrsm);
        if (splitK) {
          const SegDesc& sd = plan.host.segs[lr.directSeg];
          SrcDesc part = plan.host.srcs[sd.src];
          part.K = splitK;
          hipk::trsmPanelDirectPlus<BT><<<dim3(nT + 1, gy.y), 256, 0, sym.stream>>>(
              plan.host.panels[lr.directPanel], part, sd, ref, dinvCur);
        } else if (direct) {
          hipk::trsmPanelDirect<BT><<<dim3(nT, gy.y), 256, 0, sym.stream>>>(
              plan.host.panels[lr.directPanel], ref, dinvCur);
        } else if (fold) {
          hipk::trsmPanelPotrf<BT><<<dim3(nT, gy.y), 256, 0, sym.stream>>>(
              plan.trsmTasksFat.as<TrsmTaskFat>() + lr.trsmBegin, ref);
        } else {
          hipk::trsmPanel<BT><<<dim3(nT, gy.y), 256, 0, sym.stream>>>(
              plan.trsmTasksFat.as<TrsmTaskFat>() + lr.trsmBegin, ref);
        }
        timer.end();
      }
      if (!waitedDef && lookahead && lr.waitDefLevel >= 0 && defDone[lr.waitDefLevel]) {
        waitDeferred(lr.waitDefLevel);
      }
      const bool anyDef = lr.defEnd > lr.defBegin;
      auto forkSide = [&]() {
        hipEvent_t fork = sym.eventFromPool();
        hipCHECK(hipEventRecord(fork, sym.stream));
        hipCHECK(hipStreamWaitEvent(sym.sideStream(), fork, 0));
        sym.counters.lookaheadForks++;
        if (dueStream) {
          hipStream_t due = sym.dueSideStream();
          hipCHECK(hipStreamWaitEvent(due, fork, 0));
          waitChunk(due, waitedDue, lr.gatherDue);
          waitChunk(sym.sideStream(), waitedSide, lr.gatherOpt);
          if (lr.flushDue && lastOpt) hipCHECK(hipStreamWaitEvent(due, lastOpt, 0));
          const int64_t f2 = lr.optWaitLevel;
          if (f2 >= 0 && optDone[f2]) hipCHECK(hipStreamWaitEvent(due, optDone[f2], 0));
          if (lr.defMid > lr.defBegin) {
            timer.begin(kProfUpdate, due);
            launchUpdate(plan, lr.defBegin, lr.defMid, ref, due, nullptr, 0, sym.dueExtraLds, sideMask);
            timer.end();
          }
          defDone[li] = sym.eventFromPool();
          hipCHECK(hipEventRecord(defDone[li], due));
          if (lr.defEnd > lr.defMid) {
            timer.begin(kProfUpdate, sym.sideStream());
            launchUpdate(plan, lr.defMid, lr.defEnd, ref, sym.sideStream(), nullptr, 0, sym.bulkExtraLds, sideMask);
            timer.end();
            optDone[li] = sym.eventFromPool();
            hipCHECK(hipEventRecord(optDone[li], sym.sideStream()));
            lastOpt = optDone[li];
          }
          sideUsed = dueUsed = true;
          return;
        }
        waitChunk(sym.sideStream(), waitedSide, std::max(lr.gatherDue, lr.gatherOpt));
        if (lr.defMid > lr.defBegin) {
          timer.begin(kProfUpdate, sym.sideStream());
          launchUpdate(plan, lr.defBegin, lr.defMid, ref, sym.sideStream(), nullptr, 0, sym.bulkExtraLds, sideMask);
          timer.end();
        }
        defDone[li] = sym.eventFromPool();
        hipCHECK(hipEventRecord(defDone[li], sym.sideStream()));
        if (lr.defEnd > lr.defMid) {
          timer.begin(kProfUpdate, sym.sideStream());
          launchUpdate(plan, lr.defMid, lr.defEnd, ref, sym.sideStream(), nullptr, 0, sym.bulkExtraLds, sideMask);
          timer.end();
        }
        sideUsed = true;
      };
      const bool forkEarly = !merged;
      if (lookahead && anyDef && forkEarly) forkSide();
      const int64_t updBegin = lr.updBegin;
      if (lr.updEnd > updBegin) {
        timer.begin(direct && lr.directSeg >= 0 ? kProfChainUpdate : kProfUpdate);
        const unsigned nUpd = (unsigned)(lr.updEnd - updBegin);
        if (merged) {
          int kMem0 = kMem, extra = 0;
          if (kMem == 0) {
            kMem0 = 0;
            if (lr.extraDiag && !extraBroken && fuse) {
              extra = 1;
              extraApplied++;
            } else {
              extraBroken = true;
            }
          } else {
            kMem0 = std::max(0, kMem - kTile * extraApplied);
            extraApplied = 0;
            extraBroken = false;
          }
          hipk::chainStep<BT><<<dim3(nUpd + extra, gy.y), 256, 0, sym.stream>>>(
              plan.host.panels[lr.directPanel], plan.host.segs[lr.directSeg], (int)nUpd, nextPanel,
              fuse ? 1 : 0, ref, rawCur, stage ? rawNext : nullptr, 2 * rawSlot, dinvCur, dinvNext,
              memOff, kMem, (lookahead && batchSize == 1) ? sym.yieldWord() : nullptr,
              sym.traceLaunchId++, kMem0, extra);
          potrfFused = fuse;
        } else if (fuse) {
          if (extraApplied > 0) {
            throw std::runtime_error("HIP backend: internal error (early diagonal updates applied "
                                     "before a step that is not merged)");
          }
          extraBroken = true;
          const SegDesc& sd = plan.host.segs[lr.directSeg];
          hipk::updateTileDirectPotrf<BT><<<dim3(nUpd, gy.y), 256, 0, sym.stream>>>(
              plan.host.srcs[sd.src], sd, (int)nUpd, nextPanel, ref, splitK, dinvNext,
              stage ? rawNext : nullptr, 2 * rawSlot);
          potrfFused = true;
        } else if (direct && lr.directSeg >= 0) {
          if (extraApplied > 0) {
            throw std::runtime_error("HIP backend: internal error (early diagonal updates applied "
                                     "before a step that is not merged)");
          }
          extraBroken = true;
          const SegDesc& sd = plan.host.segs[lr.directSeg];
          hipk::updateTileDirect<BT><<<dim3(nUpd, gy.y), 256, 0, sym.stream>>>(
              plan.host.srcs[sd.src], sd, (int)nUpd, ref, stage ? rawNext : nullptr, nextPanel.nb,
              2 * rawSlot);
        } else {
          auto sp = sym.splitK ? plan.splitRange.find(updBegin) : plan.splitRange.end();
          if (sp != plan.splitRange.end() &&
              (sp->second.second - sp->second.first) * (int64_t)batchSize <= sym.splitKMaxWgs) {
            sym.counters.splitListsUsed++;
            hipk::updateTile<BT, true><<<dim3((unsigned)(sp->second.second - sp->second.first),
                                              (unsigned)batchSize), 256, 0, sym.stream>>>(
                plan.updTasksSplit.as<UpdTaskWide>() + sp->second.first, plan.chainOffTab.as<int64_t>(),
                plan.rowChain.as<int32_t>(), plan.rowLocal.as<int32_t>(), plan.rowColOff.as<int32_t>(), ref,
                nullptr, 0, 1);
          } else {
            launchUpdate(plan, updBegin, lr.updEnd, ref, sym.stream);
          }
        }
        timer.end();
      }
      rawValid = stage;
      if (lookahead && anyDef && !forkEarly) forkSide();
      if (!lookahead) {
        if (lr.defMid > lr.defBegin) {
          timer.begin(kProfUpdate);
          launchUpdate(plan, lr.defBegin, lr.defMid, ref, sym.stream);
          timer.end();
        }
        if (lr.defEnd > lr.defMid) {
          timer.begin(kProfUpdate);
          launchUpdate(plan, lr.defMid, lr.defEnd, ref, sym.stream);
          timer.end();
        }
      }
    }
    if (nFold > 0) {
      timer.begin(kProfPotrf);
      hipk::potrfPanel<BT><<<dim3((unsigned)plan.foldPanelEnd[nFold - 1], gy.y), 256, 0, sym.stream>>>(
          plan.foldDescs.as<PanelDesc>(), ref);
      timer.end();
    }
    if (sideUsed) {
      hipEvent_t join = sym.eventFromPool();
      hipCHECK(hipEventRecord(join, sym.sideStream()));
      hipCHECK(hipStreamWaitEvent(sym.stream, join, 0));
    }
    if (dueUsed) {
      hipEvent_t join = sym.eventFromPool();
      hipCHECK(hipEventRecord(join, sym.dueSideStream()));
      hipCHECK(hipStreamWaitEvent(sym.stream, join, 0));
    }
    if (chunks) {
      waitChunk(sym.stream, waitedExec, (int32_t)gatherChunkDone.size() - 1);
      gatherChunkDone.clear();
    }
  }

  void launchElim(DevPlan& plan, const ElimRangePlan& er, hipk::DataRef<BT> ref,
                  LaunchTimer& timer) {
    hipk::SkelDev sk = sym.skelDev();
    const unsigned gy = (unsigned)batchSize;
    const int64_t nLumps = er.lumpEnd - er.lumpBegin;
    if (nLumps <= 0) return;
    const unsigned gF = (unsigned)((nLumps + 3) / 4);
    timer.begin(kProfElimFactor);
    if (er.maxWidth <= 4) {
      const int64_t perWg = 4 * hipk::kTinyPerWave;
      hipk::elimFactorTinyStaged<BT><<<dim3((unsigned)((nLumps + perWg - 1) / perWg), gy), 256, 0,
                                      sym.stream>>>(
          plan.elimLumpDesc.as<ElimLumpDesc>() + er.descBegin, ref, (int)nLumps);
    } else if (er.maxWidth <= 8) {
      hipk::elimFactorSmall<BT, 8><<<dim3(gF, gy), 256, 0, sym.stream>>>(sk, ref, er.lumpBegin,
                                                                        er.lumpEnd);
    } else {
      hipk::elimFactorSmall<BT, kElimSmallMax><<<dim3(gF, gy), 256, 0, sym.stream>>>(
          sk, ref, er.lumpBegin, er.lumpEnd);
    }
    timer.end();
    launchLevels(plan, er.bigLevels, ref, timer);
    const int64_t nChains = er.chainEnd - er.chainBegin;
    if (sym.faultDropElimUpdate) {
      static std::atomic<bool> warned{false};
      if (!warned.exchange(true)) {
        fprintf(stderr, "baspacho_amd: FAULT INJECTION ACTIVE -- sparse-elimination update dropped (tests only)\n");
      }
      return;
    }
    if (er.useGather) {
      const int64_t nItems = er.itemEnd - er.itemBegin;
      auto gatherRange = [&](int64_t b, int64_t e, hipStream_t st, unsigned extraLds = 0) {
        if (e <= b) return;
        timer.begin(kProfElimUpdate, st);
        hipk::elimGatherMfma<BT><<<dim3((unsigned)((e - b + 3) / 4), gy), 256, extraLds, st>>>(
            plan.elimItems.as<ElimGatherItem>() + b, plan.elimPairOffJ.as<uint32_t>(),
            plan.elimPairOffI.as<uint32_t>(), ref, (int)(e - b));
        timer.end();
      };
      gatherChunkDone.clear();
      if (!er.chunkItemPtr.empty()) {
        const size_t nChunks = er.chunkItemPtr.size() - 1;
        const bool overlap = er.overlapLump >= 0 && sym.gatherOverlap && lookaheadOn() &&
                             plan.host.lookaheadPays(batchSize, sym.lookaheadMinFlops);
        if (overlap) {
          hipStream_t gs = sym.streams().batch[0];
          hipEvent_t factored = sym.eventFromPool();
          hipCHECK(hipEventRecord(factored, sym.stream));
          hipCHECK(hipStreamWaitEvent(gs, factored, 0));
          gatherRange(er.chunkItemPtr[0], er.chunkItemPtr[1], sym.stream);
          gatherChunkDone.assign(nChunks, nullptr);
          for (size_t c = 1; c < nChunks; c++) {
            gatherRange(er.chunkItemPtr[c], er.chunkItemPtr[c + 1], gs, sym.gatherOverlapLds);
            gatherChunkDone[c] = sym.eventFromPool();
            hipCHECK(hipEventRecord(gatherChunkDone[c], gs));
          }
          sym.counters.gatherChunksOverlapped += (int64_t)nChunks - 1;
        } else {
          for (size_t c = 0; c < nChunks; c++) gatherRange(er.chunkItemPtr[c], er.chunkItemPtr[c + 1], sym.stream);
        }
      } else {
        gatherRange(er.itemBegin, er.itemBegin + nItems, sym.stream);
      }
      const int64_t nWide = er.ldsEnd - er.ldsBegin;
      if (nWide > 0) {
        timer.begin(kProfElimUpdate);
        hipk::elimGather<BT><<<dim3((unsigned)((nWide + 3) / 4), gy), 256, 0, sym.stream>>>(
            plan.elimItems.as<ElimGatherItem>() + er.ldsBegin, plan.elimPairOffJ.as<uint32_t>(),
            plan.elimPairOffI.as<uint32_t>(), ref, (int)nWide);
        timer.end();
      }
      const int64_t nTiny9 = er.tiny9End - er.tinyBegin, nTiny = er.tinyEnd - er.tiny9End;
      if (nTiny9 > 0) {
        timer.begin(kProfElimUpdate);
        hipk::elimGatherTiny<BT, 9><<<dim3((unsigned)((nTiny9 + 27) / 28), gy), 256, 0, sym.stream>>>(
            plan.elimItems.as<ElimGatherItem>() + er.tinyBegin, plan.elimPairOffJ.as<uint32_t>(),
            plan.elimPairOffI.as<uint32_t>(), ref, (int)nTiny9);
        timer.end();
      }
      if (nTiny > 0) {
        timer.begin(kProfElimUpdate);
        hipk::elimGatherTiny<BT, 16><<<dim3((unsigned)((nTiny + 15) / 16), gy), 256, 0, sym.stream>>>(
            plan.elimItems.as<ElimGatherItem>() + er.tiny9End, plan.elimPairOffJ.as<uint32_t>(),
            plan.elimPairOffI.as<uint32_t>(), ref, (int)nTiny);
        timer.end();
      }
    } else if (nChains > 0) {
      timer.begin(kProfElimUpdate);
      hipk::elimUpdate<BT><<<dim3((unsigned)((nChains + 3) / 4), gy), 256, 0, sym.stream>>>(
          sk, plan.elimChainLump.as<int32_t>() + er.chainLumpOff, ref, er.chainBegin, er.chainEnd);
      timer.end();
    }
  }

  virtual bool hasFusedFactor() const override { return !sym.forcePerOp; }

  void enqueueFactor(DevPlan& plan, hipk::DataRef<BT> ref, LaunchTimer& timer) {
    sym.resetEventPool();
    const bool lookahead = lookaheadOn() && plan.host.lookaheadPays(batchSize, sym.lookaheadMinFlops);
    if (ref.many && !lookahead && sym.profile == nullptr && batchSize >= sym.subBatchMin) {
      const int total = batchSize;
      const int parts = std::max(2, std::min({sym.subBatchParts, 4, total / std::max(1, sym.subBatchMin / 2)}));
      hipStream_t mainStream = sym.stream;
      hipEvent_t fork = sym.eventFromPool();
      hipCHECK(hipEventRecord(fork, mainStream));
      struct Restore {
        HipNumericCtx& c;
        hipStream_t st;
        int bs;
        ~Restore() {
          c.sym.stream = st;
          c.batchSize = bs;
          c.subBatchBase = c.subBatchTotal = 0;
        }
      } restore{*this, mainStream, total};
      subBatchTotal = total;
      for (int g = 0; g < parts; g++) {
        const int b0 = (int)((int64_t)total * g / parts), b1 = (int)((int64_t)total * (g + 1) / parts);
        subBatchBase = b0;
        batchSize = b1 - b0;
        sym.stream = g ? sym.streams().batch[g - 1] : mainStream;
        if (g) hipCHECK(hipStreamWaitEvent(sym.stream, fork, 0));
        sym.counters.subBatchesEnqueued++;
        hipk::DataRef<BT> sub{nullptr, ref.many + subBatchBase};
        for (const ElimRangePlan& er : plan.host.elimRanges) launchElim(plan, er, sub, timer);
        launchLevels(plan, plan.host.levels, sub, timer);
        if (g) {
          hipEvent_t join = sym.eventFromPool();
          hipCHECK(hipEventRecord(join, sym.stream));
          hipCHECK(hipStreamWaitEvent(mainStream, join, 0));
        }
      }
      return;
    }
    for (const ElimRangePlan& er : plan.host.elimRanges) launchElim(plan, er, ref, timer);
    launchLevels(plan, plan.host.levels, ref, timer);
  }

  virtual void factorRange(T* data, int64_t startLump, int64_t upToLump) override {
    sym.checkAsyncError();
    DevPlan* planPtr = &sym.planFor(sym.sparseElimRanges, startLump, upToLump, 0);
    if (batchSize > 1 && planPtr->host.hasTail && !sym.tailInBatch) {
      planPtr = &sym.planFor(sym.sparseElimRanges, startLump, upToLump, 2);
    }
    DevPlan& plan = *planPtr;
    hipk::DataRef<BT> ref = makeRef(data);
    LaunchTimer timer(sym.stream, sym.profile);
    enqueueFactor(plan, ref, timer);
    hipCHECK(hipGetLastError());
    timer.finish();
  }

  void dataPointers(T* data, vector<BT*>& out);

  virtual void doElimination(const SymElimCtx& elimData, T* data, int64_t lumpsBegin,
                             int64_t lumpsEnd) override {
    const HipSymElimCtx* e = dynamic_cast<const HipSymElimCtx*>(&elimData);
    BASPACHO_CHECK_NOTNULL(e);
    BASPACHO_CHECK_EQ(e->lumpsBegin, lumpsBegin);
    BASPACHO_CHECK_EQ(e->lumpsEnd, lumpsEnd);
    DevPlan& plan = sym.planFor({lumpsBegin, lumpsEnd}, lumpsBegin, lumpsEnd, 1);
    hipk::DataRef<BT> ref = makeRef(data);
    LaunchTimer timer(sym.stream, sym.profile);
    sym.resetEventPool();
    for (const ElimRangePlan& er : plan.host.elimRanges) launchElim(plan, er, ref, timer);
    hipCHECK(hipGetLastError());
    timer.finish();
  }

  DevPlan& adoptPlan(HipPlanHost&& host) {
    opPlans.emplace_back(new DevPlan);
    opPlans.back()->host = std::move(host);
    opPlans.back()->upload();
    return *opPlans.back();
  }

  virtual void potrf(int64_t n, T* data, int64_t offA) override {
    sym.potrfBiggestN = std::max(sym.potrfBiggestN, n);
    DevPlan& plan = adoptPlan(buildDenseOpPlan(n, 0, offA, true));
    OpTimer opTimer(sym.potrfStat, sym.stream, (double)n);
    LaunchTimer timer(sym.stream, nullptr);
    {
      FlagOff noLookahead(sym.lookaheadEnabled);
      launchLevels(plan, plan.host.levels, makeRef(data), timer);
    }
    hipCHECK(hipGetLastError());
  }

  virtual void trsm(int64_t n, int64_t k, T* data, int64_t offA, int64_t offB) override {
    BASPACHO_CHECK_EQ(offB, offA + n * n);
    DevPlan& plan = adoptPlan(buildDenseOpPlan(n, k, offA, false));
    OpTimer opTimer(sym.trsmStat, sym.stream, (double)n, (double)k);
    LaunchTimer timer(sym.stream, nullptr);
    {
      FlagOff noLookahead(sym.lookaheadEnabled);
      launchLevels(plan, plan.host.levels, makeRef(data), timer);
    }
    hipCHECK(hipGetLastError());
  }

  virtual void saveSyrkGemm(int64_t m, int64_t n, int64_t k, const T* data, int64_t offset) override {
    BASPACHO_CHECK_LE(m * n, tempBufSize);
    temp.resize((size_t)(tempBufSize * batchSize) * sizeof(BT));
    hipCHECK(hipMemsetAsync(temp.ptr, 0, (size_t)(tempBufSize * batchSize) * sizeof(BT), sym.stream));
    HipPlanHost host;
    SrcDesc sr{};
    sr.off = offset;
    sr.lda = (int32_t)k;
    sr.K = (int32_t)k;
    sr.rowsBelow = (int32_t)n;
    sr.nRest = (int32_t)n;
    host.srcs.push_back(sr);
    SegDesc sd{};
    sd.src = 0;
    sd.kind = kSegIntra;
    sd.q0 = 0;
    sd.m = (int32_t)m;
    sd.tgtBase = 0;
    sd.tgtStride = (int32_t)m;
    host.segs.push_back(sd);
    for (int32_t cT = 0; cT < m; cT += kTile) {
      for (int32_t rT = cT; rT < n; rT += kTile) host.updTasks.push_back({0, rT, cT, 0});
    }
    DevPlan& plan = adoptPlan(std::move(host));
    sym.gemmCalls++;
    OpTimer opTimer(sym.sygeStat, sym.stream, (double)m, (double)n, (double)k);
    launchUpdate(plan, 0, plan.numUpdTasks, makeRef(const_cast<T*>(data)),
                 sym.stream, temp.as<BT>() ? const_cast<BT*>(temp.as<BT>()) : nullptr, tempBufSize);
    hipCHECK(hipGetLastError());
  }

  virtual void prepareAssemble(int64_t targetLump) override {
    hipk::SkelDev sk = sym.skelDev();
    spanToChainOffset.resize((size_t)(sym.skel.numSpans() + 1) * sizeof(int64_t));
    const int64_t n = sym.skel.chainColPtr[targetLump + 1] - sym.skel.chainColPtr[targetLump];
    hipk::prepareAssembleKernel<<<dim3((unsigned)((n + 255) / 256)), 256, 0, sym.stream>>>(
        sk, reinterpret_cast<int64_t*>(spanToChainOffset.ptr), targetLump);
  }

  virtual void assemble(T* data, int64_t rectRowBegin, int64_t dstStride, int64_t srcColDataOffset,
                        int64_t srcRectWidth, int64_t numBlockRows, int64_t numBlockCols) override {
    hipk::SkelDev sk = sym.skelDev();
    OpTimer opTimer(sym.asmblStat, sym.stream, (double)numBlockRows, (double)numBlockCols);
    hipk::assembleKernel<BT><<<dim3((unsigned)numBlockRows, (unsigned)batchSize), 256, 0, sym.stream>>>(
        sk, spanToChainOffset.as<int64_t>(), temp.as<BT>(), tempBufSize, makeRef(data),
        rectRowBegin, dstStride, srcColDataOffset, srcRectWidth, numBlockRows, numBlockCols);
    hipCHECK(hipGetLastError());
  }

  virtual void pseudoFactorSpans(T* data, int64_t spanBegin, int64_t spanEnd) override {
    if (spanEnd <= spanBegin) return;
    const CoalescedBlockMatrixSkel& sk = sym.skel;
    hipk::DataRef<BT> ref = makeRef(data);
    auto narrowRun = [&](int64_t b, int64_t e) {
      if (e <= b) return;
      hipk::pseudoFactorSpansKernel<BT><<<dim3((unsigned)((e - b + 3) / 4), (unsigned)batchSize), 256,
                                          0, sym.stream>>>(sym.skelDev(), ref, b, e);
    };
    FlagOff noLookahead(sym.lookaheadEnabled);
    int64_t runBegin = spanBegin;
    for (int64_t s = spanBegin; s < spanEnd; s++) {
      const int64_t n = sk.spanStart[s + 1] - sk.spanStart[s];
      if (n <= kElimSmallMax) continue;
      narrowRun(runBegin, s);
      runBegin = s + 1;
      const int64_t lump = sk.spanToLump[s];
      const int64_t lda = sk.lumpStart[lump + 1] - sk.lumpStart[lump];
      const int64_t c0 = sk.chainColPtr[lump], nCh = sk.chainColPtr[lump + 1] - c0;
      const int64_t idxInLump = s - sk.lumpToSpan[lump];
      const int64_t offD = sk.chainData[c0 + idxInLump] + sk.spanOffsetInLump[s];
      const int64_t rowsBelow = sk.chainRowsTillEnd[c0 + nCh - 1] - sk.chainRowsTillEnd[c0 + idxInLump];
      LaunchTimer timer(sym.stream, nullptr);
      DevPlan& pf = adoptPlan(buildDenseOpPlan(n, 0, offD, true, 0, lda));
      launchLevels(pf, pf.host.levels, ref, timer);
      if (rowsBelow > 0) {
        DevPlan& ps = adoptPlan(buildDenseOpPlan(n, rowsBelow, offD, false, 0, lda));
        launchLevels(ps, ps.host.levels, ref, timer);
      }
    }
    narrowRun(runBegin, spanEnd);
    hipCHECK(hipGetLastError());
  }

  HipSymbolicCtx& sym;
  int batchSize;
  int subBatchBase = 0, subBatchTotal = 0;
  vector<hipEvent_t> gatherChunkDone;
  int64_t tempBufSize = 0;
  DevBuf temp, spanToChainOffset;
  vector<std::unique_ptr<DevPlan>> opPlans;
};

template <>
hipk::DataRef<double> HipNumericCtx<double>::makeRef(double* data) {
  return {data, nullptr};
}
template <>
hipk::DataRef<float> HipNumericCtx<float>::makeRef(float* data) {
  return {data, nullptr};
}
template <>
void HipNumericCtx<double>::dataPointers(double* data, vector<double*>& out) { out = {data}; }
template <>
void HipNumericCtx<float>::dataPointers(float* data, vector<float*>& out) { out = {data}; }
template <>
void HipNumericCtx<vector<double*>>::dataPointers(vector<double*>* data, vector<double*>& out) {
  BASPACHO_CHECK_EQ((int)data->size(), batchSize);
  out = *data;
}
template <>
void HipNumericCtx<vector<float*>>::dataPointers(vector<float*>* data, vector<float*>& out) {
  BASPACHO_CHECK_EQ((int)data->size(), batchSize);
  out = *data;
}
template <>
hipk::DataRef<double> HipNumericCtx<vector<double*>>::makeRef(vector<double*>* data) {
  BASPACHO_CHECK_EQ((int)data->size(), batchSize);
  return {nullptr, (double* const*)sym.ptrRing.push(data->data(), data->size() * sizeof(double*),
                                                    sym.stream)};
}
template <>
hipk::DataRef<float> HipNumericCtx<vector<float*>>::makeRef(vector<float*>* data) {
  BASPACHO_CHECK_EQ((int)data->size(), batchSize);
  return {nullptr, (float* const*)sym.ptrRing.push(data->data(), data->size() * sizeof(float*),
                                                   sym.stream)};
}

NumericCtxBase* HipSymbolicCtx::createNumericCtxForType(std::type_index tIdx, int64_t tempSize,
                                                        int batch) {
  if (tIdx == std::type_index(typeid(double))) return new HipNumericCtx<double>(*this, 1, tempSize);
  if (tIdx == std::type_index(typeid(float))) return new HipNumericCtx<float>(*this, 1, tempSize);
  if (tIdx == std::type_index(typeid(vector<double*>))) {
    return new HipNumericCtx<vector<double*>>(*this, batch, tempSize);
  }
  if (tIdx == std::type_index(typeid(vector<float*>))) {
    return new HipNumericCtx<vector<float*>>(*this, batch, tempSize);
  }
  return nullptr;
}

template <typename T>
struct HipSolveCtx : SolveCtx<T> {
  using BT = BaseType<T>;
  HipSolveCtx(HipSymbolicCtx& sym_, int nRHS_, int batch_) : sym(sym_), nRHS(nRHS_), batch(batch_) {}

  virtual bool hasFusedSolve() const override { return !sym.forcePerOp; }

  dim3 grid(unsigned x) const { return dim3(x, (unsigned)nRHS, (unsigned)batch); }

  template <bool BACKWARD>
  void elimRange(DevPlan& plan, const ElimRangePlan& er, hipk::SolveRef<BT> ref) {
    hipk::SkelDev sk = sym.skelDev();
    const int64_t nLumps = er.lumpEnd - er.lumpBegin;
    if (nLumps <= 0) return;
    auto small = [&] {
      const dim3 gL = grid((unsigned)((nLumps + 255) / 256));
      plan.ensureSolveGather(sym.skel);
      if (BACKWARD) {
        if (er.maxWidth <= 4) {
          const int64_t d0 = plan.solveGather.rangeLumpDesc[&er - plan.host.elimRanges.data()];
          auto launch = [&](auto kern, int rb) {
            kern<<<dim3((unsigned)((nLumps + 15) / 16), (unsigned)((nRHS + rb - 1) / rb), (unsigned)batch),
                   256, 0, sym.stream>>>(plan.solveLumpDescs.as<SolveLumpDesc>() + d0,
                                         plan.solveLumpBlocks.as<SolveLumpBlock>(), ref, (int)nLumps, nRHS);
          };
          const auto wide = plan.solveGather.rangeWide[&er - plan.host.elimRanges.data()];
          const int64_t wideRows = sym.skel.order() - wide.rowBelow;
          const int64_t wideSpans = (int64_t)sym.skel.spanStart.size() - 1 - wide.spanBelow;
          const unsigned wideGroups = (unsigned)((nRHS + hipk::kWideRhs - 1) / hipk::kWideRhs);
          const size_t wideBytes = (size_t)hipk::wideGroupStride(wideRows) * wideGroups * (size_t)batch * sizeof(BT);
// ... 555 lines not shown
int hipBackendReadExtents(unsigned long long* out, int maxLaunches) {
#if defined(BSP_KTRACE) && defined(BSP_TRACE_TILE)
  hipCHECK(hipDeviceSynchronize());
  const int n = std::min(maxLaunches, 2048);
  hipCHECK(hipMemcpyFromSymbol(out, HIP_SYMBOL(hipk::bspLaunchExtent), sizeof(unsigned long long) * 4 * n));
  std::vector<unsigned long long> init(2048 * 4, 0ull);
  for (int i = 0; i < 2048; i++) init[4 * i] = ~0ull;
  hipCHECK(hipMemcpyToSymbol(HIP_SYMBOL(hipk::bspLaunchExtent), init.data(), sizeof(unsigned long long) * 4 * 2048));
  return n;
#else
  (void)out;
  (void)maxLaunches;
  return 0;
#endif
}

int hipBackendReadTrace(long long* out, int maxRecords) {
#if defined(BSP_KTRACE) || defined(BSP_TRACE_UPD)
  unsigned n = 0;
  hipCHECK(hipDeviceSynchronize());
  hipCHECK(hipMemcpyFromSymbol(&n, HIP_SYMBOL(hipk::bspTraceCount), sizeof n));
  const int cnt = (int)std::min<unsigned>(n, (unsigned)std::min(maxRecords, 8192));
  hipCHECK(hipMemcpyFromSymbol(out, HIP_SYMBOL(hipk::bspTrace), sizeof(long long) * hipk::kTraceW * cnt));
  n = 0;
  hipCHECK(hipMemcpyToSymbol(HIP_SYMBOL(hipk::bspTraceCount), &n, sizeof n));
  return cnt;
#else
  (void)out;
  (void)maxRecords;
  return 0;
#endif
}

double hipBackendMfmaF64ProbeTflops() {
  const int blocks = 1024, iters = 4000;
  double* out = nullptr;
  hipCHECK(hipMalloc(&out, sizeof(double) * 256 * blocks));
  hipEvent_t a, b;
  hipCHECK(hipEventCreate(&a));
  hipCHECK(hipEventCreate(&b));
  hipk::mfmaF64Probe<<<blocks, 256>>>(out, iters);
  hipCHECK(hipEventRecord(a, nullptr));
  hipk::mfmaF64Probe<<<blocks, 256>>>(out, iters);
  hipCHECK(hipEventRecord(b, nullptr));
  hipCHECK(hipEventSynchronize(b));
  float ms = 0;
  hipCHECK(hipEventElapsedTime(&ms, a, b));
  (void)hipEventDestroy(a);
  (void)hipEventDestroy(b);
  (void)hipFree(out);
  return double(blocks) * 4 * iters * 4 * 2048.0 / (ms * 1e-3) / 1e12;
}

void hipBackendForcePerOp(SymbolicCtx& sym, bool on) {
  HipSymbolicCtx* h = dynamic_cast<HipSymbolicCtx*>(&sym);
  BASPACHO_CHECK_NOTNULL(h);
  h->forcePerOp = on;
}

std::vector<int64_t> hipBackendPlanLevels(SymbolicCtx& sym, int64_t startLump, int64_t upToLump) {
  HipSymbolicCtx* h = dynamic_cast<HipSymbolicCtx*>(&sym);
  BASPACHO_CHECK_NOTNULL(h);
  HipPlanHost p = buildHipPlan(h->skel, h->sparseElimRanges, startLump, upToLump, h->planOpts);
  std::vector<int64_t> out;
  auto emit = [&](const vector<LevelRange>& levels, int64_t range) {
    for (const LevelRange& lr : levels) {
      int64_t maxNb = 0, maxRows = 0, sumRows = 0;
      for (int64_t q = lr.panelBegin; q < lr.panelEnd; q++) {
        const PanelDesc& pd = p.panels[p.levelPanels[q]];
        maxNb = std::max<int64_t>(maxNb, pd.nb);
        maxRows = std::max<int64_t>(maxRows, pd.rowsBelow);
        sumRows += pd.rowsBelow;
      }
      const int64_t row[8] = {range, lr.panelEnd - lr.panelBegin, maxNb, maxRows, lr.trsmEnd - lr.trsmBegin,
                              lr.updEnd - lr.updBegin, lr.defEnd - lr.defBegin, sumRows};
      out.insert(out.end(), row, row + 8);
    }
  };
  for (size_t r = 0; r < p.elimRanges.size(); r++) emit(p.elimRanges[r].bigLevels, (int64_t)r);
  emit(p.levels, -1);
  return out;
}

void hipBackendSetFault(SymbolicCtx& sym, int kind) {
  HipSymbolicCtx* h = dynamic_cast<HipSymbolicCtx*>(&sym);
  BASPACHO_CHECK_NOTNULL(h);
  h->faultDropElimUpdate = kind == 1;
  h->sweepFault = kind == 2 ? 2 : 0;
  h->sweepSpinLimitS = kind == 2 ? 0.05 : 2.0;
}

int hipBackendReadSweepTrace(SymbolicCtx& sym, long long* out, int maxBlocks) {
  HipSymbolicCtx* h = dynamic_cast<HipSymbolicCtx*>(&sym);
  BASPACHO_CHECK_NOTNULL(h);
  if (!h->sweepTrace.ptr) return 0;
  hipCHECK(hipDeviceSynchronize());
  const int n = std::min(maxBlocks, 4096);
  hipCHECK(hipMemcpy(out, h->sweepTrace.ptr, (size_t)n * 4 * sizeof(long long), hipMemcpyDeviceToHost));
  return n;
}

HipRunCounters hipBackendRunCounters(SymbolicCtx& sym) {
  HipSymbolicCtx* h = dynamic_cast<HipSymbolicCtx*>(&sym);
  BASPACHO_CHECK_NOTNULL(h);
  HipRunCounters c;
  c.sweepLaunches = h->counters.sweepLaunches;
  c.sweepTimeouts = h->counters.sweepTimeouts;
  c.splitListsUsed = h->counters.splitListsUsed;
  c.subBatchesEnqueued = h->counters.subBatchesEnqueued;
  c.lookaheadForks = h->counters.lookaheadForks;
  c.gatherChunksOverlapped = h->counters.gatherChunksOverlapped;
  c.tailLaunches = h->counters.tailLaunches;
  c.sweepMfmaLaunches = h->counters.sweepMfmaLaunches;
  c.solveWideLaunches = h->counters.solveWideLaunches;
  c.invReused = h->counters.invReused;
  c.potrfFoldedLevels = h->counters.potrfFoldedLevels;
  c.selinvLaunches = h->counters.selinvLaunches;
  c.selinvChunks = h->counters.selinvChunks;
  c.sweepsRetired = h->sweepBroken ? 1 : 0;
  c.sweepErrorPending = (h->sweepHostErr && *reinterpret_cast<volatile unsigned*>(h->sweepHostErr)) ? 1 : 0;
  return c;
}

void hipBackendSetProfile(SymbolicCtx& sym, HipKernelProfile* prof, bool inSitu) {
  HipSymbolicCtx* h = dynamic_cast<HipSymbolicCtx*>(&sym);
  BASPACHO_CHECK_NOTNULL(h);
  h->profile = prof;
  h->profileInSitu = prof != nullptr && inSitu;
}

HipPlanStats hipBackendPlanStats(SymbolicCtx& sym, int64_t startLump, int64_t upToLump) {
  HipSymbolicCtx* h = dynamic_cast<HipSymbolicCtx*>(&sym);
  BASPACHO_CHECK_NOTNULL(h);
  HipPlanHost p = buildHipPlan(h->skel, h->sparseElimRanges, startLump, upToLump, h->planOpts);
  HipPlanStats s;
  s.flops = p.flops;
  s.updElems = p.updElems;
  s.updFlops = p.updFlops;
  s.elimPairElems = p.elimPairElems;
  s.elimPairFlops = p.elimPairFlops;
  s.elimColElems = p.elimColElems;
  s.updFlopsDirect = p.updFlopsDirect;
  s.elimPairOperandElems = p.elimPairOperandElems;
  s.elimTargetElems = p.elimTargetElems;
  s.trsmFlops = p.trsmFlops;
  s.potrfFlops = p.potrfFlops;
  s.trsmFlopsMerged = p.trsmFlopsMerged;
  s.potrfFlopsFused = p.potrfFlopsFused;
  s.numLaunches = p.numLaunches;
  s.numLevels = (int64_t)p.levels.size();
  s.numPanels = (int64_t)p.panels.size();
  s.numSegs = (int64_t)p.segs.size();
  s.numUpdTasks = (int64_t)p.updTasks.size();
  s.numTrsmTasks = (int64_t)p.trsmTasks.size();
  s.chainTabEntries = (int64_t)p.chainOffTab.size();
  s.maxPanelsInLevel = p.maxPanelsInLevel;
  int64_t atomicTasks = 0;
  for (auto& t : p.updTasks) atomicTasks += t.atomic ? 1 : 0;
  s.numAtomicUpdTasks = atomicTasks;
  s.numForkLevels = p.numForkLevels;
  s.deferredFlops = p.deferredFlops;
  s.tailUpdFlops = p.tailUpdFlops;
  for (const LevelRange& lr : p.levels) s.numTailPanels += lr.tail ? 1 : 0;
  return s;
}

template <typename T>
void hipBackendSelectedInverse(SymbolicCtx& sym, T* data) {
  HipSymbolicCtx* h = dynamic_cast<HipSymbolicCtx*>(&sym);
  BASPACHO_CHECK_NOTNULL(h);
  h->selectedInverse(data);
}
template void hipBackendSelectedInverse<double>(SymbolicCtx&, double*);
template void hipBackendSelectedInverse<float>(SymbolicCtx&, float*);

template <typename T>
void hipBackendSelectedInverse(SymbolicCtx& sym, const vector<T*>& data) {
  HipSymbolicCtx* h = dynamic_cast<HipSymbolicCtx*>(&sym);
  BASPACHO_CHECK_NOTNULL(h);
  h->selectedInverse(data);
}
template void hipBackendSelectedInverse<double>(SymbolicCtx&, const vector<double*>&);
template void hipBackendSelectedInverse<float>(SymbolicCtx&, const vector<float*>&);

void hipBackendSetSelInvBatchChunk(SymbolicCtx& sym, int64_t maxMatrices) {
  HipSymbolicCtx* h = dynamic_cast<HipSymbolicCtx*>(&sym);
  BASPACHO_CHECK_NOTNULL(h);
  BASPACHO_CHECK_GE(maxMatrices, 0);
  h->selInvChunkCap = maxMatrices;
}

template <typename T>
void hipBackendLogDet(SymbolicCtx& sym, const T* const* factors, int64_t batch, bool single, T* out) {
  HipSymbolicCtx* h = dynamic_cast<HipSymbolicCtx*>(&sym);
  BASPACHO_CHECK_NOTNULL(h);
  h->logDet(factors, batch, single, out);
}
template void hipBackendLogDet<double>(SymbolicCtx&, const double* const*, int64_t, bool, double*);
template void hipBackendLogDet<float>(SymbolicCtx&, const float* const*, int64_t, bool, float*);

template <typename T>
// ... 57 lines not shown
```

### baspacho_amd/csrc/hip_plan.cpp

```cpp
#include "hip_plan.h"

#include <algorithm>
#include <chrono>
#include <cstdlib>
#include <iostream>
#include <atomic>
#include <map>
#include <thread>

namespace BaSpaCho {

using std::vector;

namespace {

struct LumpCols {
  int64_t width, diagOff, rowsBelow, diagChains, chain0, nChains;
};

LumpCols lumpCols(const CoalescedBlockMatrixSkel& sk, int64_t l) {
  LumpCols g;
  g.width = sk.lumpStart[l + 1] - sk.lumpStart[l];
  g.chain0 = sk.chainColPtr[l];
  g.nChains = sk.chainColPtr[l + 1] - g.chain0;
// ... 696 lines not shown
            if (forks.empty() || forks.back() != levelIdx) {
              if (forks.size() >= 2) lr.optWaitLevel = std::max(lr.optWaitLevel, forks[forks.size() - 2]);
              forks.push_back(levelIdx);
            }
            lastDeferredLevel[sd.lump] = levelIdx;
          }
          const double R = double(sr.rowsBelow - sd.q0), m = double(sd.m);
          plan.updElems += m * R - m * (m - 1) / 2;
          plan.updFlops += 2.0 * sr.K * (m * R - m * (m - 1) / 2);
          if (anyDeferred) plan.deferredFlops += 2.0 * sr.K * (m * R - m * (m - 1) / 2);
        }
      }
      lr.panelEnd = (int64_t)plan.levelPanels.size();
      lr.trsmEnd = (int64_t)plan.trsmTasks.size();
      lr.updEnd = (int64_t)plan.updTasks.size();
      lr.defBegin = lr.updEnd;
      plan.updTasks.insert(plan.updTasks.end(), deferred.begin(), deferred.end());
      lr.defMid = (int64_t)plan.updTasks.size();
      plan.updTasks.insert(plan.updTasks.end(), deferredLate.begin(), deferredLate.end());
      lr.defEnd = (int64_t)plan.updTasks.size();
      auto xcdOrder = [&](int64_t begin, int64_t end) {
        const int64_t cnt = end - begin;
        if (cnt < 64) return;
        vector<UpdTask> tmp(plan.updTasks.begin() + begin, plan.updTasks.begin() + end);
        const int64_t base = cnt / 8, extra = cnt % 8;
        int64_t chunkStart[9];
        chunkStart[0] = 0;
        for (int x = 0; x < 8; x++) chunkStart[x + 1] = chunkStart[x] + base + (x < extra ? 1 : 0);
        for (int64_t p = 0; p < cnt; p++) {
          const int64_t x = p % 8, k = p / 8;
          plan.updTasks[begin + p] = tmp[chunkStart[x] + k];
        }
      };
      if (lr.defEnd > lr.defBegin) {
        plan.hasDeferred = true;
        plan.numForkLevels++;
      }
      if (bucket.size() == 1) {
        lr.directPanel = bucket[0].panel;
        if (nowSegs == 1 && nowPlain) {
          lr.directSeg = nowSeg;
          const SegDesc& sd = plan.segs[nowSeg];
          const SrcDesc& sr = plan.srcs[sd.src];
          const double R = double(sr.rowsBelow - sd.q0);
          const double m = double(sd.outer ? std::min<int32_t>(sd.m, kOuterWidth) : sd.m);
          plan.updFlopsDirect += 2.0 * sr.K * (m * R - m * (m - 1) / 2);
        }
        if (chain && lr.directSeg >= 0) {
          const SegDesc& sd = plan.segs[lr.directSeg];
          const PanelDesc& next = plan.panels[buckets[bi + 1][0].panel];
          {
            const PanelDesc& pd0 = plan.panels[bucket[0].panel];
            const SrcDesc& sr0 = plan.srcs[sd.src];
            if (!sd.outer && sd.kind == kSegIntra && sd.q0 == 0 && sr0.K == pd0.nb &&
                pd0.nb == kPanelWidth && pd0.nRest - sd.m >= kTile) {
              lr.extraDiag = 1;
            }
          }
          if (sd.q0 == 0 && sd.rowMin == 0 && sd.tgtBase == next.diagOff &&
              sd.tgtStride == next.lda) {
            lr.rawNext = 1;
            plan.maxChainRows = std::max<int64_t>(plan.maxChainRows, next.rowsBelow);
          }
          if (sd.q0 == 0 && sd.rowMin == 0 && sd.tgtBase == next.diagOff && next.nb == kTile &&
              sd.tgtStride == next.lda && lr.updEnd - lr.updBegin >= 2) {
            lr.fuseNext = 1;
            const SrcDesc& sr = plan.srcs[sd.src];
            const int32_t nbLast = plan.panels[bucket[0].panel].nb;
            if (sd.outer && sr.K > nbLast) lr.splitK = sr.K - nbLast;
          }
        }
      }
      xcdOrder(lr.updBegin, lr.updEnd);
      xcdOrder(lr.defBegin, lr.defMid);
      xcdOrder(lr.defMid, lr.defEnd);
      plan.maxPanelsInLevel = std::max<int64_t>(plan.maxPanelsInLevel, lr.panelEnd - lr.panelBegin);
      plan.numLaunches += 1 + (lr.trsmEnd > lr.trsmBegin) + (lr.updEnd > lr.updBegin) +
                          (lr.defEnd > lr.defBegin);
      out.push_back(lr);
    }
    for (size_t li = 1; li < out.size(); li++) {
      if (out[li].tail == 1) out[li - 1].flushDue = 1;
    }
    for (size_t li = 0; li < out.size(); li++) {
      const LevelRange& lr = out[li];
      const bool directUpd = lr.directPanel >= 0 && lr.directSeg >= 0 && lr.updEnd > lr.updBegin;
      const bool nextDirect = li + 1 < out.size() && out[li + 1].directPanel >= 0;
      if (directUpd && lr.fuseNext && nextDirect) {
        const double nb = plan.panels[out[li + 1].directPanel].nb;
        plan.potrfFlopsFused += nb * nb * nb / 3.0;
      }
      if (li > 0 && directUpd && lr.trsmEnd > lr.trsmBegin) {
        const LevelRange& pr = out[li - 1];
        const bool staged = pr.directPanel >= 0 && pr.directSeg >= 0 && pr.updEnd > pr.updBegin &&
                            pr.rawNext;
        const SegDesc& sd = plan.segs[lr.directSeg];
        const PanelDesc& pd = plan.panels[lr.directPanel];
        const SrcDesc& sr = plan.srcs[sd.src];
        const bool intraStep = !sd.outer && sr.K == pd.nb;
        const bool blockLast = sd.outer == 1 && sr.K > pd.nb && (sr.K - pd.nb) % kTile == 0 &&
                               sr.rowsBelow == pd.rowsBelow && sr.lda == pd.lda;
        if (staged && (intraStep || blockLast)) {
          plan.trsmFlopsMerged += double(pd.rowsBelow) * pd.nb * pd.nb;
        }
      }
    }
  };
  for (size_t r = 0; r < plan.elimRanges.size(); r++) {
    emitLevels(elimBigBuckets[r], plan.elimRanges[r].bigLevels);
    plan.numLaunches += 2;
  }
  emitLevels(levelBuckets, plan.levels);
  for (ElimRangePlan& er : plan.elimRanges) {
    if (er.chunkItemPtr.empty()) continue;
    bool ok = !plan.levels.empty();
    for (const LevelRange& lr : plan.levels) {
      ok = ok && lr.directPanel >= 0 && plan.panels[lr.directPanel].lump == er.overlapLump;
    }
    if (!ok) {
      er.overlapLump = -1;
      continue;
    }
    const int64_t nBlk = (int64_t)er.chunkOfColBlock.size();
    for (LevelRange& lr : plan.levels) {
      const PanelDesc& pd = plan.panels[lr.directPanel];
      const int64_t b = (pd.lda - pd.nRest - pd.nb) / kOuterWidth;
      lr.gatherNow = er.chunkOfColBlock[std::min(b + 1, nBlk - 1)];
      auto maxChunk = [&](int64_t begin, int64_t end) {
        int32_t m = -1;
        for (int64_t t = begin; t < end; t++) {
          const int64_t cb = std::min(nBlk - 1, (kOuterWidth * (b + 1) + plan.updTasks[t].colTile) / kOuterWidth);
          m = std::max(m, er.chunkOfColBlock[cb]);
        }
        return m;
      };
      lr.gatherDue = maxChunk(lr.defBegin, lr.defMid);
      lr.gatherOpt = maxChunk(lr.defMid, lr.defEnd);
    }
  }

  for (auto& s : plan.segs) {
    if (s.kind == kSegBoard) s.tgtBase = 0;
  }
  BASPACHO_CHECK_LT((int64_t)plan.segs.size(), (int64_t)INT32_MAX);
  return plan;
}

HipPlanHost buildDenseOpPlan(int64_t n, int64_t k, int64_t offA, bool potrfOnly, int64_t vecOff,
                             int64_t ldaIn) {
  HipPlanHost plan;
  const int64_t ld = ldaIn > 0 ? ldaIn : n;
  BASPACHO_CHECK_GE(ld, n);
  BASPACHO_CHECK_LT(ld, (int64_t)INT32_MAX);
  BASPACHO_CHECK_LT(n + k, (int64_t)INT32_MAX);
  const int64_t rowsB = potrfOnly ? 0 : k;
  for (int64_t blockStart = 0; blockStart < n; blockStart += kOuterWidth) {
    const int64_t blockEnd = std::min<int64_t>(n, blockStart + kOuterWidth);
    for (int64_t c0 = blockStart; c0 < blockEnd; c0 += kPanelWidth) {
      const int32_t nb = (int32_t)std::min<int64_t>(kPanelWidth, blockEnd - c0);
      LevelRange lr{};
      lr.waitDefLevel = -1;
      PanelDesc pd{};
      pd.diagOff = offA + c0 * ld + c0;
      pd.lda = (int32_t)ld;
      pd.nb = nb;
      pd.nRest = (int32_t)(n - c0 - nb);
// ... 276 lines not shown
```

### baspacho_amd/csrc/hip_plan.h

```cpp
#pragma once

#include <cstdint>
#include <vector>

#include "skeleton.h"

namespace BaSpaCho {

constexpr int kPanelWidth = 64;
constexpr int kOuterWidth = 256;
constexpr int kTile = 64;
constexpr int kElimSmallMax = 16;

struct PanelDesc {
  int64_t diagOff;
  int32_t lda;
  int32_t nb;
  int32_t rowsBelow;
  int32_t nRest;
  int32_t lumpRowBase;
  int32_t lump;
  int32_t vecOff;
  int32_t pad;
};

struct SrcDesc {
  int64_t off;
  int32_t lda;
  int32_t K;
  int32_t rowsBelow;
  int32_t nRest;
  int32_t lumpRowBase;
  int32_t pad;
};

enum SegKind : int32_t { kSegIntra = 0, kSegBoard = 1 };

struct SegDesc {
  int32_t src;
  int32_t kind;
  int32_t q0;
  int32_t m;
  int64_t tgtBase;
  int32_t tgtStride;
  int32_t firstChainOrd;
  int64_t chainTabPtr;
  int32_t outer;
  int32_t lump;
  int32_t rowMin;
  int32_t pad;
};

struct UpdTask {
  int32_t seg;
  int32_t rowTile;
  int32_t colTile;
  int32_t atomic;
};

struct UpdTaskFat {
  int64_t srcOff;
  int64_t tgtBase;
  int32_t lda, K, rowsBelow, segEnd;
  int32_t rowTile, colTile, tgtStride, rowMin;
  int32_t atomic, fast, pad0, pad1;
};
static_assert(sizeof(UpdTaskFat) == 64, "one scalar load");

struct UpdTaskWide {
  int64_t srcOff;
  int64_t tgtBase;
  int64_t chainTabPtr;
  int32_t lda, K, rowsBelow, nRest;
  int32_t lumpRowBase, kind, segEnd, tgtStride;
  int32_t firstChainOrd, rowMin, rowTile, colTile;
  int32_t atomic, pad0, pad1, pad2, pad3, pad4;
};
static_assert(sizeof(UpdTaskWide) == 96, "two scalar loads");

struct TrsmTask {
  int32_t panel;
  int32_t rowTile;
};

struct TrsmTaskFat {
  int64_t diagOff;
  int32_t lda, nb, rowsBelow, rowTile;
  int32_t pad0, pad1;
};
static_assert(sizeof(TrsmTaskFat) == 32, "one scalar load");

struct LevelRange {
  int64_t panelBegin, panelEnd;
  int64_t trsmBegin, trsmEnd;
  int64_t updBegin, updEnd;
  int64_t defBegin, defEnd;
  int64_t defMid = 0;
  int32_t directPanel = -1, directSeg = -1;
  int32_t fuseNext = 0;
  int32_t splitK = 0;
  int32_t rawNext = 0;
  int64_t waitDefLevel;
  int32_t extraDiag = 0;
  int64_t optWaitLevel = -1;
  int32_t gatherNow = -1, gatherDue = -1, gatherOpt = -1;
  int32_t tail = 0, tailPanels = 0;
  int32_t flushDue = 0;
};

struct ElimGatherItem {
  int64_t tgtOff;
  int32_t pairBegin;
  int32_t pairEnd;
  int32_t tgtStride;
  int16_t rows, cols;
  int16_t n;
  int16_t flags;
  uint32_t firstJ, firstI;
};
constexpr int kGatherMaxElems = 256;
constexpr int kGatherMaxPairs = 64;
constexpr uint32_t kGatherChunkElems = 0xffffffffu;

struct ElimLumpDesc {
  int64_t diagOff;
  int32_t n;
  int32_t rowsBelow;
};

struct ElimRangePlan {
  int64_t lumpBegin, lumpEnd;
  int64_t chainBegin, chainEnd;
  int64_t chainLumpOff;
  int32_t maxWidth;
  int64_t descBegin = 0;
  std::vector<LevelRange> bigLevels;
  bool useGather = false;
  int64_t itemBegin = 0, itemEnd = 0;
  int64_t tinyBegin = 0, tinyEnd = 0;
  int64_t tiny9End = 0;
  int64_t ldsBegin = 0, ldsEnd = 0;
  std::vector<int64_t> chunkItemPtr;
  std::vector<int32_t> chunkOfColBlock;
  int64_t overlapLump = -1;
};

struct HipPlanOptions {
  bool dueStream = true;
  bool planTiming = false;
  int32_t gatherMaxPairs = kGatherMaxPairs;
  double bulkAhead = 0.8;
  bool gatherOverlap = false;
  int32_t overlapFirst = 2;
  int32_t overlapStep = 3;
  int32_t overlapMinBlocks = 8;
  int32_t tailBlocks = 6;
  int32_t tailMinBlocks = 6;
  bool tailWholeNarrow = true;
  int32_t tailNarrowMin = 2;
  int32_t solveSortWindow = 16;
  void applyDeveloperEnv();
};

struct HipPlanHost {
  HipPlanOptions opts;
  bool hasTail = false;
  int64_t startLump = 0, upToLump = 0;
  std::vector<ElimRangePlan> elimRanges;
  std::vector<int32_t> elimChainLump;
  std::vector<ElimLumpDesc> elimLumpDesc;
  std::vector<ElimGatherItem> elimItems;
  std::vector<uint32_t> elimPairOffJ, elimPairOffI;

  std::vector<PanelDesc> panels;
  std::vector<SrcDesc> srcs;
  std::vector<SegDesc> segs;
  std::vector<int64_t> chainOffTab;
  std::vector<int32_t> rowChain, rowLocal, rowColOff;
  std::vector<int32_t> rowGlobal;

  double tailUpdFlops = 0;
  double updFlopsDirect = 0, elimPairOperandElems = 0, elimTargetElems = 0, trsmFlops = 0,
         potrfFlops = 0;
  double trsmFlopsMerged = 0, potrfFlopsFused = 0;
  std::vector<int32_t> levelPanels;
  std::vector<TrsmTask> trsmTasks;
  std::vector<UpdTask> updTasks;
  std::vector<LevelRange> levels;

  double flops = 0;
// ... 109 lines not shown
```

### include/baspacho_amd.h

```cpp
#ifndef BASPACHO_AMD_H_
#define BASPACHO_AMD_H_

#include <stdint.h>

#ifdef __cplusplus
extern "C" {
#endif

typedef struct bsp_solver bsp_solver;

enum { BSP_BACKEND_REF = 0, BSP_BACKEND_FAST = 1, BSP_BACKEND_CUDA = 2, BSP_BACKEND_HIP = 3 };
enum {
  BSP_FILL_COMPLETE = 0,
  BSP_FILL_FOR_AUTO_ELIMS = 1,
  BSP_FILL_FOR_GIVEN_ELIMS = 2,
  BSP_FILL_NONE = 3
};

typedef struct bsp_settings {
  int32_t find_sparse_elimination_ranges;
  int32_t num_threads;
  int32_t backend;
  int32_t add_fill_policy;
  const double* computation_model;
} bsp_settings;

typedef struct bsp_hip_options {
  int32_t lookahead;
  int32_t due_stream;
  int32_t split_k;
  int32_t gather_max_pairs;
  int32_t gather_overlap;
  int32_t sub_batch_min;
  int32_t sub_batches;
  int32_t tail_blocks;
  int32_t lazy_plan;
  int32_t block_solve;
  int32_t solve_inv;
  int32_t solve_sweep;
  int32_t sweep_min_width;
  int32_t solve_wide;
  int32_t chain_contraction;
  int32_t dense_merge;
  int32_t expected_batch;
  double lookahead_min_gf;
  double bulk_ahead;
  double level_cost_us;
} bsp_hip_options;
void bsp_hip_options_default(bsp_hip_options* out);

const char* bsp_last_error(void);
const char* bsp_version(void);

int bsp_create_solver(const bsp_settings* settings, int64_t num_params, const int64_t* param_sizes,
                      const int64_t* ptrs, const int64_t* inds, int64_t num_elim_ranges,
                      const int64_t* elim_ranges, int64_t num_elim_last, const int64_t* elim_last,
                      bsp_solver** out);

int bsp_create_solver_opts(const bsp_settings* settings, const bsp_hip_options* options,
                           int64_t num_params, const int64_t* param_sizes, const int64_t* ptrs,
                           const int64_t* inds, int64_t num_elim_ranges, const int64_t* elim_ranges,
                           int64_t num_elim_last, const int64_t* elim_last, bsp_solver** out);

int bsp_create_solver_from_skeleton(int64_t num_spans, const int64_t* span_start,
                                    int64_t num_lumps, const int64_t* lump_to_span,
                                    const int64_t* col_ptr, const int64_t* row_ind,
                                    int64_t num_elim_ranges, const int64_t* elim_ranges,
                                    bsp_solver** out);

void bsp_destroy_solver(bsp_solver* s);

int64_t bsp_order(const bsp_solver* s);
int64_t bsp_data_size(const bsp_solver* s);
int64_t bsp_num_spans(const bsp_solver* s);
int64_t bsp_num_lumps(const bsp_solver* s);
int64_t bsp_can_factor_up_to_span(const bsp_solver* s);
int64_t bsp_span_vector_offset(const bsp_solver* s, int64_t span);
int64_t bsp_span_matrix_offset(const bsp_solver* s, int64_t span, int64_t* out);

enum {
  BSP_SKEL_SPAN_START = 0,
  BSP_SKEL_SPAN_TO_LUMP = 1,
  BSP_SKEL_LUMP_START = 2,
  BSP_SKEL_LUMP_TO_SPAN = 3,
  BSP_SKEL_SPAN_OFFSET_IN_LUMP = 4,
  BSP_SKEL_CHAIN_COL_PTR = 5,
  BSP_SKEL_CHAIN_ROW_SPAN = 6,
  BSP_SKEL_CHAIN_DATA = 7,
  BSP_SKEL_CHAIN_ROWS_TILL_END = 8,
  BSP_SKEL_BOARD_COL_PTR = 9,
  BSP_SKEL_BOARD_ROW_LUMP = 10,
  BSP_SKEL_BOARD_CHAIN_COL_ORD = 11,
  BSP_SKEL_BOARD_ROW_PTR = 12,
  BSP_SKEL_BOARD_COL_LUMP = 13,
  BSP_SKEL_BOARD_COL_ORD = 14,
  BSP_SKEL_PARAM_TO_SPAN = 15,
  BSP_SKEL_SPARSE_ELIM_RANGES = 16
};
int bsp_skeleton_array(const bsp_solver* s, int which, const int64_t** data, int64_t* len);

int bsp_block_offset(const bsp_solver* s, int64_t row_param, int64_t col_param, int64_t* offset,
                     int64_t* stride, int32_t* flipped);
int bsp_diag_block_offset(const bsp_solver* s, int64_t param, int64_t* offset, int64_t* stride);

int bsp_device_accessor(bsp_solver* s, const int64_t* out_device_arrays[8]);

void bsp_set_stream(bsp_solver* s, void* stream);

int bsp_factor_f64(bsp_solver* s, double* dev_data);
int bsp_factor_f32(bsp_solver* s, float* dev_data);
int bsp_factor_batched_f64(bsp_solver* s, double* const* dev_ptrs, int32_t batch);
int bsp_factor_batched_f32(bsp_solver* s, float* const* dev_ptrs, int32_t batch);
int bsp_factor_up_to_f64(bsp_solver* s, double* dev_data, int64_t span_index);
int bsp_factor_from_f64(bsp_solver* s, double* dev_data, int64_t span_index);
int bsp_factor_up_to_f32(bsp_solver* s, float* dev_data, int64_t span_index);
int bsp_factor_from_f32(bsp_solver* s, float* dev_data, int64_t span_index);
int bsp_factor_per_op_f64(bsp_solver* s, double* dev_data);
int bsp_factor_per_op_f32(bsp_solver* s, float* dev_data);
int bsp_collect_op_stats(bsp_solver* s, int32_t on);
int bsp_read_op_stats(bsp_solver* s, int32_t which, double* out, int64_t capacity, int64_t* count);
int bsp_force_per_op(bsp_solver* s, int32_t on);
int64_t bsp_plan_levels(bsp_solver* s, int64_t* out, int64_t capacity);
int bsp_do_elimination_f64(bsp_solver* s, double* dev_data, int64_t elim_range_index);
int bsp_do_elimination_f32(bsp_solver* s, float* dev_data, int64_t elim_range_index);

int bsp_solve_f64(bsp_solver* s, const double* dev_mat, double* dev_vec, int64_t stride,
                  int32_t nrhs);
// ... 91 lines not shown
                             float* dev_grad_values);
int bsp_assemble_adjoint_batched_f64(bsp_solver* s, const bsp_assembly* a, const double* const* dev_grad_data,
                                     double* const* dev_grad_values, int32_t batch);
int bsp_assemble_adjoint_batched_f32(bsp_solver* s, const bsp_assembly* a, const float* const* dev_grad_data,
                                     float* const* dev_grad_values, int32_t batch);
int bsp_scalar_permutation(const bsp_solver* s, int64_t* out);
int bsp_solve_batched_f64(bsp_solver* s, const double* const* dev_mats, double* const* dev_vecs,
                          int32_t batch, int64_t stride, int32_t nrhs, int32_t which);
int bsp_solve_batched_f32(bsp_solver* s, const float* const* dev_mats, float* const* dev_vecs,
                          int32_t batch, int64_t stride, int32_t nrhs, int32_t which);
int bsp_factor_partial_batched_f64(bsp_solver* s, double* const* dev_ptrs, int32_t batch,
                                   int64_t span_index, int32_t which);
int bsp_factor_partial_batched_f32(bsp_solver* s, float* const* dev_ptrs, int32_t batch,
                                   int64_t span_index, int32_t which);
int bsp_solve_partial_batched_f64(bsp_solver* s, const double* const* dev_mats,
                                  double* const* dev_vecs, int32_t batch, int64_t stride,
                                  int32_t nrhs, int32_t which, int64_t span_index);
int bsp_solve_partial_batched_f32(bsp_solver* s, const float* const* dev_mats, float* const* dev_vecs,
                                  int32_t batch, int64_t stride, int32_t nrhs, int32_t which,
                                  int64_t span_index);

int bsp_bal_linearize_f64(int64_t num_obs, const int64_t* obs_cam, const int64_t* obs_pt,
                          const double* obs_xy, const double* cams, const double* pts, double* res,
                          double* Jc, double* Jp, void* stream);
int bsp_bal_fill_hessian_f64(bsp_solver* s, int64_t num_pts, int64_t num_cams, int64_t num_obs,
                             const int64_t* obs_cam, const int64_t* obs_pt, const double* Jc,
                             const double* Jp, const double* res, double lambda, double* dev_data,
                             double* dev_grad, int64_t* dev_dbg, void* stream);
int bsp_bal_fill_hessian_f32(bsp_solver* s, int64_t num_pts, int64_t num_cams, int64_t num_obs,
                             const int64_t* obs_cam, const int64_t* obs_pt, const double* Jc,
                             const double* Jp, const double* res, float lambda, float* dev_data,
                             float* dev_grad, int64_t* dev_dbg, void* stream);

int bsp_bal_linearize_se3_f64(int64_t num_obs, const int64_t* obs_cam, const int64_t* obs_pt,
                              const double* obs_xy, const double* cams, const double* pts,
                              double* res, double* Jc, double* Jp, void* stream);
int bsp_bal_fill_hessian_se3_f64(bsp_solver* s, int64_t num_pts, int64_t num_cams, int64_t num_obs,
                                 const int64_t* obs_cam, const int64_t* obs_pt, const double* Jc,
                                 const double* Jp, const double* res, double lambda, double* dev_data,
                                 double* dev_grad, void* stream);
int bsp_bal_fill_hessian_se3_f32(bsp_solver* s, int64_t num_pts, int64_t num_cams, int64_t num_obs,
                                 const int64_t* obs_cam, const int64_t* obs_pt, const double* Jc,
                                 const double* Jp, const double* res, float lambda, float* dev_data,
                                 float* dev_grad, void* stream);

double bsp_factor_flops(const bsp_solver* s);

typedef struct bsp_plan_stats {
  double flops, upd_elems, upd_flops, elim_pair_elems, elim_pair_flops, elim_col_elems,
      upd_flops_direct,
      elim_pair_operand_elems,
      elim_target_elems,
      trsm_flops, potrf_flops,
      trsm_flops_merged,
      potrf_flops_fused;
  int64_t num_launches, num_levels, num_panels, num_segs, num_upd_tasks, num_trsm_tasks,
      chain_tab_entries, max_panels_in_level, num_atomic_upd_tasks,
      num_gather_groups,
      num_fork_levels;
  double deferred_flops;
  double tail_upd_flops;
  int64_t num_tail_panels;
} bsp_plan_stats;
int bsp_plan_stats_full(bsp_solver* s, bsp_plan_stats* out);

typedef struct bsp_run_counters {
  int64_t sweep_launches;
  int64_t sweep_timeouts;
  int64_t split_lists_used;
  int64_t sub_batches_enqueued;
  int64_t lookahead_forks;
  int64_t sweeps_retired;
  int64_t sweep_error_pending;
  int64_t gather_chunks_overlapped;
  int64_t tail_launches;
  int64_t sweep_mfma_launches;
  int64_t solve_wide_launches;
  int64_t inv_reused;
  int64_t potrf_folded_levels;
  int64_t selinv_launches;
  int64_t selinv_chunks;
} bsp_run_counters;
int bsp_run_counters_get(bsp_solver* s, bsp_run_counters* out);

enum {
  BSP_PROF_ELIM_FACTOR = 0,
  BSP_PROF_ELIM_UPDATE = 1,
  BSP_PROF_POTRF = 2,
  BSP_PROF_TRSM = 3,
  BSP_PROF_UPDATE = 4,
  BSP_PROF_CHAIN_UPDATE = 5,
  BSP_PROF_NUM_KINDS = 6
};
int bsp_factor_profiled_f64(bsp_solver* s, double* dev_data, double ms[6], int64_t launches[6]);
int bsp_factor_profiled_insitu_f64(bsp_solver* s, double* dev_data, double ms[6],
                                   int64_t launches[6]);
int bsp_factor_profiled_busy_f64(bsp_solver* s, double* dev_data, double ms[6], int64_t launches[6],
                                 double busy_ms[6]);

int bsp_probe_mfma_f64(double* tflops);

int bsp_debug_read_trace(long long* out, int max_records, int* n_records);
int bsp_debug_read_extents(unsigned long long* out, int max_launches, int* n);

int bsp_plan_serialize(const bsp_solver* s, int64_t* buf, int64_t capacity, int64_t* needed);
int bsp_create_solver_from_plan(const int64_t* buf, int64_t len, bsp_solver** out);

enum {
  BSP_SS_TRANSPOSE = 0,
  BSP_SS_CLEAR = 1,
  BSP_SS_SYM_PERMUTATION = 2,
  BSP_SS_INDEP_ELIM_FILL = 3,
  BSP_SS_FULL_ELIM_FILL = 4,
  BSP_SS_FILL_REDUCING_PERM = 5,
  BSP_SS_EXTRACT_RIGHT_BOTTOM = 6
};
int bsp_sparse_structure_op(int op, int64_t n, const int64_t* ptrs, const int64_t* inds,
                            const int64_t* arg, int64_t arg_len, int32_t flag, int64_t* out_ptrs,
                            int64_t* out_inds, int64_t capacity, int64_t* out_n, int64_t* out_nnz);

#ifdef __cplusplus
}
#endif
#endif
```

### include/baspacho_amd_testing.h

```cpp
#ifndef BASPACHO_AMD_TESTING_H
#define BASPACHO_AMD_TESTING_H

#include "baspacho_amd.h"

#ifdef __cplusplus
extern "C" {
#endif

int bsp_test_set_fault(bsp_solver* s, int32_t kind);

int bsp_test_selinv_plan(const bsp_solver* s, int64_t* buf, int64_t capacity, int64_t* needed);
int bsp_test_selinv_plan_up_to(const bsp_solver* s, int64_t span, int64_t* buf, int64_t capacity, int64_t* needed);

int bsp_test_set_selinv_batch_chunk(bsp_solver* s, int32_t max_matrices);

int bsp_test_read_sweep_trace(bsp_solver* s, long long* out, int32_t max_blocks, int32_t* n_blocks);

#ifdef __cplusplus
}
#endif

#endif
```

Measured before the change: 27850 GF/s.

## Elide redundant cross-stream waits via vector clocks and use device-scope events

Adds a host-side vector-clock tracker (StreamOrder) that skips hipStreamWaitEvent calls already implied by earlier synchronisation. Event records on the due stream are dropped when the plan marks them as never waited on. By default, new events are created with device-scope (no system fence) flags to cut fence cost at each inter-stream handoff. The intent is to lower per-level sync overhead in the lookahead schedule. The risk is a missed dependency if the clock logic is wrong, though a bypass switch and test hooks are included.

Result: no change. 28000 GF/s (median of 6 runs) (+0.5%).

```diff
diff --git a/baspacho_amd/__init__.py b/baspacho_amd/__init__.py
--- a/baspacho_amd/__init__.py
+++ b/baspacho_amd/__init__.py
@@ -34,7 +34,8 @@
 
 _HIP_OPTION_INTS = ["lookahead", "due_stream", "split_k", "gather_max_pairs", "gather_overlap",
                     "sub_batch_min", "sub_batches", "tail_blocks", "lazy_plan", "block_solve", "solve_inv",
-                    "solve_sweep", "sweep_min_width", "solve_wide", "chain_contraction", "dense_merge", "expected_batch"]
+                    "solve_sweep", "sweep_min_width", "solve_wide", "chain_contraction", "dense_merge", "expected_batch",
+                    "device_scope_events"]
 _HIP_OPTION_REALS = ["lookahead_min_gf", "bulk_ahead", "level_cost_us"]
 
 
@@ -63,6 +64,10 @@
                  "gather_chunks_overlapped", "tail_launches", "sweep_mfma_launches",
                  "solve_wide_launches", "inv_reused", "potrf_folded_levels", "selinv_launches",
                  "selinv_chunks"]]
+
+
+class _CStreamCounters(ctypes.Structure):
+    _fields_ = [(n, ctypes.c_int64) for n in ["stream_waits", "event_records"]]
 
 
 @dataclass
@@ -314,6 +319,9 @@
 
     def _testSetFault(self, kind):
         _check(self._lib.bsp_test_set_fault(self._h, ctypes.c_int32(kind)))
+
+    def _testSetStreamOrderBypass(self, on):
+        _check(self._lib.bsp_test_set_stream_order_bypass(self._h, ctypes.c_int32(1 if on else 0)))
 
     def _testSetSelInvBatchChunk(self, max_matrices):
         _check(self._lib.bsp_test_set_selinv_batch_chunk(self._h, ctypes.c_int32(max_matrices)))
@@ -729,7 +737,11 @@
     def runCounters(self):
         st = _CRunCounters()
         _check(self._lib.bsp_run_counters_get(self._h, ctypes.byref(st)))
-        return {n: getattr(st, n) for n, _ in _CRunCounters._fields_}
+        out = {n: getattr(st, n) for n, _ in _CRunCounters._fields_}
+        so = _CStreamCounters()
+        _check(self._lib.bsp_stream_counters_get(self._h, ctypes.byref(so)))
+        out.update({n: getattr(so, n) for n, _ in _CStreamCounters._fields_})
+        return out
 
     def factorProfiled(self, data, in_situ=False, busy=False):
         self._check_data(data)
@@ -891,6 +903,14 @@
     _check(_lib.load().bsp_debug_read_extents(out.ctypes.data_as(ctypes.c_void_p), max_launches,
                                               ctypes.byref(n)))
     return out[:n.value]
+
+
+def _test_stream_order(ops):
+    a = np.ascontiguousarray(np.asarray(ops, dtype=np.int32).reshape(-1, 3))
+    out = np.zeros(len(a), dtype=np.int32)
+    _check(_lib.load().bsp_test_stream_order(a.ctypes.data_as(ctypes.c_void_p), ctypes.c_int64(len(a)),
+                                             out.ctypes.data_as(ctypes.c_void_p)))
+    return out.tolist()
 
 
 def create_solver(settings: Optional[Settings], param_sizes, ss: SparseStructure,
diff --git a/baspacho_amd/csrc/backend_options.h b/baspacho_amd/csrc/backend_options.h
--- a/baspacho_amd/csrc/backend_options.h
+++ b/baspacho_amd/csrc/backend_options.h
@@ -15,6 +15,7 @@
   int32_t subBatches = -1;
   int32_t tailBlocks = -1;
   int32_t lazyPlan = -1;
+  int32_t deviceScopeEvents = -1;
   int32_t blockSolve = -1;
   int32_t solveInv = -1;
   int32_t solveSweep = -1;
diff --git a/baspacho_amd/csrc/bsp_utils.cpp b/baspacho_amd/csrc/bsp_utils.cpp
--- a/baspacho_amd/csrc/bsp_utils.cpp
+++ b/baspacho_amd/csrc/bsp_utils.cpp
@@ -92,6 +92,7 @@
   num("BSP_SUB_BATCHES", subBatches, 2);
   num("BSP_TAIL_BLOCKS", tailBlocks, 0);
   if (std::getenv("BSP_LAZY_PLAN")) lazyPlan = 1;
+  num("BSP_DEVICE_SCOPE_EVENTS", deviceScopeEvents, 0);
   flag("BSP_BLOCK_SOLVE", blockSolve);
   flag("BSP_SOLVE_INV", solveInv);
   flag("BSP_SOLVE_SWEEP", solveSweep);
diff --git a/baspacho_amd/csrc/c_api.cpp b/baspacho_amd/csrc/c_api.cpp
--- a/baspacho_amd/csrc/c_api.cpp
+++ b/baspacho_amd/csrc/c_api.cpp
@@ -14,6 +14,7 @@
 #include "hip_backend.h"
 #include "hip_plan.h"
 #include "solver.h"
+#include "stream_order.h"
 
 using namespace BaSpaCho;
 
@@ -44,7 +45,8 @@
 void bsp_hip_options_default(bsp_hip_options* o) {
   o->lookahead = o->due_stream = o->split_k = o->gather_max_pairs = o->gather_overlap = o->sub_batch_min =
       o->sub_batches = o->tail_blocks = o->lazy_plan = o->block_solve = o->solve_inv = o->solve_sweep =
-          o->sweep_min_width = o->solve_wide = o->chain_contraction = o->dense_merge = o->expected_batch = -1;
+          o->sweep_min_width = o->solve_wide = o->chain_contraction = o->dense_merge = o->expected_batch =
+              o->device_scope_events = -1;
   o->lookahead_min_gf = o->bulk_ahead = o->level_cost_us = NAN;
 }
 
@@ -75,6 +77,7 @@
     options.chainContraction = ho->chain_contraction;
     options.denseMerge = ho->dense_merge;
     options.expectedBatch = ho->expected_batch;
+    options.deviceScopeEvents = ho->device_scope_events;
     options.lookaheadMinGF = ho->lookahead_min_gf;
     options.bulkAhead = ho->bulk_ahead;
     options.levelCostUs = ho->level_cost_us;
@@ -313,6 +316,37 @@
 int bsp_test_read_sweep_trace(bsp_solver* s, long long* out, int32_t max_blocks, int32_t* n_blocks) {
   BSP_TRY
   *n_blocks = hipBackendReadSweepTrace(s->solver->internalSymbolicContext(), out, max_blocks);
+  BSP_CATCH
+}
+
+int bsp_test_set_stream_order_bypass(bsp_solver* s, int32_t on) {
+  BSP_TRY
+  hipBackendSetStreamOrderBypass(s->solver->internalSymbolicContext(), on != 0);
+  BSP_CATCH
+}
+
+int bsp_test_stream_order(const int32_t* ops, int64_t n, int32_t* out) {
+  BSP_TRY
+  StreamOrder order;
+  static const char handles[StreamOrder::kMaxStreams + 1] = {};
+  int32_t events = 0;
+  for (int64_t i = 0; i < n; i++) {
+    const int32_t op = ops[3 * i], st = ops[3 * i + 1], ev = ops[3 * i + 2];
+    if (op != 0 && (st < 0 || st > StreamOrder::kMaxStreams)) throw std::runtime_error("bsp_test_stream_order: bad stream");
+    out[i] = 0;
+    if (op == 0) {
+      order.reset();
+      events = 0;
+    } else if (op == 1) {
+      out[i] = order.record(order.streamIndex(handles + st));
+      events++;
+    } else if (op == 2) {
+      if (ev < 0 || ev >= events) throw std::runtime_error("bsp_test_stream_order: unknown event");
+      out[i] = order.wait(order.streamIndex(handles + st), ev) ? 1 : 0;
+    } else {
+      throw std::runtime_error("bsp_test_stream_order: bad op");
+    }
+  }
   BSP_CATCH
 }
 
@@ -1016,6 +1050,14 @@
   BSP_CATCH
 }
 
+int bsp_stream_counters_get(bsp_solver* s, bsp_stream_counters* out) {
+  BSP_TRY
+  const HipRunCounters c = hipBackendRunCounters(s->solver->internalSymbolicContext());
+  out->stream_waits = c.streamWaits;
+  out->event_records = c.eventRecords;
+  BSP_CATCH
+}
+
 int bsp_probe_mfma_f64(double* tflops) {
   BSP_TRY
   *tflops = hipBackendMfmaF64ProbeTflops();
diff --git a/baspacho_amd/csrc/hip_backend.h b/baspacho_amd/csrc/hip_backend.h
--- a/baspacho_amd/csrc/hip_backend.h
+++ b/baspacho_amd/csrc/hip_backend.h
@@ -45,6 +45,7 @@
 void hipBackendForcePerOp(SymbolicCtx& sym, bool on);
 
 void hipBackendSetFault(SymbolicCtx& sym, int kind);
+void hipBackendSetStreamOrderBypass(SymbolicCtx& sym, bool on);
 
 struct HipRunCounters {
   int64_t sweepLaunches = 0;
@@ -62,6 +63,8 @@
   int64_t sweepErrorPending = 0;
   int64_t selinvLaunches = 0;
   int64_t selinvChunks = 0;
+  int64_t streamWaits = 0;
+  int64_t eventRecords = 0;
 };
 HipRunCounters hipBackendRunCounters(SymbolicCtx& sym);
 int hipBackendReadSweepTrace(SymbolicCtx& sym, long long* out, int maxBlocks);
diff --git a/baspacho_amd/csrc/hip_backend.hip b/baspacho_amd/csrc/hip_backend.hip
--- a/baspacho_amd/csrc/hip_backend.hip
+++ b/baspacho_amd/csrc/hip_backend.hip
@@ -19,6 +19,7 @@
 #include "hip_grad_kernels.h"
 #include "hip_assembly_kernels.h"
 #include "mat_ops.h"
+#include "stream_order.h"
 
 namespace BaSpaCho {
 
@@ -555,6 +556,7 @@
     gatherOverlap = HipBackendOptions::on(o.gatherOverlap, false);
     if (o.sweepMinWidth >= 0) sweepMinWidth = std::max(1, o.sweepMinWidth);
     lazyPlan = HipBackendOptions::on(o.lazyPlan, false);
+    deviceScopeEvents = o.deviceScopeEvents < 0 ? 1 : std::min(o.deviceScopeEvents, 2);
     if (!std::isnan(o.lookaheadMinGF)) lookaheadMinFlops = 1e9 * o.lookaheadMinGF;
     planOpts.dueStream = HipBackendOptions::on(o.dueStream, planOpts.dueStream);
     if (o.gatherMaxPairs >= 0) planOpts.gatherMaxPairs = std::max(8, o.gatherMaxPairs);
@@ -575,6 +577,7 @@
 
   virtual ~HipSymbolicCtx() override {
     for (hipEvent_t e : events) (void)hipEventDestroy(e);
+    for (hipEvent_t e : devEvents) (void)hipEventDestroy(e);
     if (sweepHostErr) (void)hipHostFree(sweepHostErr);
   }
 
@@ -603,7 +606,9 @@
     grad.reset();
     for (hipEvent_t e : events) (void)hipEventDestroy(e);
     events.clear();
-    nextEvent = 0;
+    for (hipEvent_t e : devEvents) (void)hipEventDestroy(e);
+    devEvents.clear();
+    nextEvent = nextDevEvent = 0;
     dinvScratch.release();
     rawScratch.release();
     yieldBuf.release();
@@ -643,7 +648,13 @@
       rawScratch.resize((size_t)2 * plan.host.maxChainRows * kTile * sizeof(double));
     }
     const size_t wantEvents = 8 + 4 * (size_t)plan.host.numForkLevels;
-    while (events.size() < wantEvents) {
+    vector<hipEvent_t>& pool = deviceScopeEvents ? devEvents : events;
+    while (pool.size() < wantEvents) {
+      hipEvent_t e;
+      hipCHECK(hipEventCreateWithFlags(&e, deviceScopeEvents ? deviceEventFlags() : hipEventDisableTiming));
+      pool.push_back(e);
+    }
+    while (events.size() < 8) {
       hipEvent_t e;
       hipCHECK(hipEventCreateWithFlags(&e, hipEventDisableTiming));
       events.push_back(e);
@@ -1083,15 +1094,42 @@
     return reinterpret_cast<unsigned*>(yieldBuf.ptr);
   }
   hipStream_t dueSideStream() { return streams().due; }
-  hipEvent_t eventFromPool() {
-    if (nextEvent == events.size()) {
+  unsigned deviceEventFlags() const {
+    return hipEventDisableTiming | (deviceScopeEvents == 2 ? hipEventReleaseToDevice : hipEventDisableSystemFence);
+  }
+  hipEvent_t eventFromPool(bool deviceScope = false) {
+    const bool dev = deviceScope && deviceScopeEvents != 0;
+    vector<hipEvent_t>& pool = dev ? devEvents : events;
+    size_t& next = dev ? nextDevEvent : nextEvent;
+    if (next == pool.size()) {
       hipEvent_t e;
-      hipCHECK(hipEventCreateWithFlags(&e, hipEventDisableTiming));
-      events.push_back(e);
-    }
-    return events[nextEvent++];
-  }
-  void resetEventPool() { nextEvent = 0; }
+      hipCHECK(hipEventCreateWithFlags(&e, dev ? deviceEventFlags() : hipEventDisableTiming));
+      pool.push_back(e);
+    }
+    return pool[next++];
+  }
+  void resetEventPool() {
+    nextEvent = nextDevEvent = 0;
+    order.reset();
+  }
+  struct PoolEvent {
+    hipEvent_t ev = nullptr;
+    int id = -1;
+    explicit operator bool() const { return ev != nullptr; }
+  };
+  PoolEvent recordEvent(hipStream_t on, bool deviceScope = true) {
+    PoolEvent e;
+    e.ev = eventFromPool(deviceScope);
+    hipCHECK(hipEventRecord(e.ev, on));
+    e.id = order.record(order.streamIndex(on));
+    counters.eventRecords++;
+    return e;
+  }
+  void waitEvent(hipStream_t st, const PoolEvent& e) {
+    if (!order.wait(order.streamIndex(st), e.id) && !streamOrderBypass) return;
+    hipCHECK(hipStreamWaitEvent(st, e.ev, 0));
+    counters.streamWaits++;
+  }
 
   const CoalescedBlockMatrixSkel& skel;
   vector<int64_t> permutation;
@@ -1101,6 +1139,8 @@
   bool profileInSitu = false;
   bool lookaheadEnabled = true;
   bool lazyPlan = false;
+  int deviceScopeEvents = 1;
+  bool streamOrderBypass = false;
   static constexpr unsigned bulkExtraLds = 6 * 1024, dueExtraLds = 6 * 1024;
   bool forcePerOp = false;
   bool faultDropElimUpdate = false;
@@ -1117,8 +1157,9 @@
   static constexpr int64_t splitKMaxWgs = 1024;
   int subBatchMin = 16;
   int subBatchParts = 2;
-  vector<hipEvent_t> events;
-  size_t nextEvent = 0;
+  vector<hipEvent_t> events, devEvents;
+  size_t nextEvent = 0, nextDevEvent = 0;
+  StreamOrder order;
   int device = -1;
   bool inPrepare = false;
   bool eagerOnly = false;
@@ -1152,6 +1193,7 @@
     int64_t sweepLaunches = 0, sweepTimeouts = 0, splitListsUsed = 0, subBatchesEnqueued = 0,
             lookaheadForks = 0, gatherChunksOverlapped = 0, tailLaunches = 0, sweepMfmaLaunches = 0, invReused = 0, solveWideLaunches = 0, potrfFoldedLevels = 0;
     int64_t selinvLaunches = 0, selinvChunks = 0;
+    int64_t streamWaits = 0, eventRecords = 0;
   } counters;
   void checkAsyncError() {
     if (sweepHostErr && *reinterpret_cast<volatile unsigned*>(sweepHostErr) != 0u) {
@@ -1284,8 +1326,9 @@
                     LaunchTimer& timer) {
     const dim3 gy(1, (unsigned)batchSize, 1);
     const bool lookahead = lookaheadOn() && plan.host.lookaheadPays(batchSize, sym.lookaheadMinFlops);
-    vector<hipEvent_t> defDone(levels.size(), nullptr);
-    vector<hipEvent_t> optDone(levels.size(), nullptr);
+    using PoolEvent = typename HipSymbolicCtx::PoolEvent;
+    vector<PoolEvent> defDone(levels.size());
+    vector<PoolEvent> optDone(levels.size());
     const bool dueStream = plan.host.opts.dueStream && sizeof(BT) == 8;
     const int sideMask = dueStream ? 3 : 1;
     int64_t nFold = 0;
@@ -1298,9 +1341,9 @@
     auto prevFork = [&](int64_t f) -> int64_t { return f >= 0 ? levels[f].waitDefLevel : -1; };
     auto waitDeferred = [&](int64_t f) {
       if (f < 0 || !defDone[f]) return;
-      hipCHECK(hipStreamWaitEvent(sym.stream, defDone[f], 0));
+      sym.waitEvent(sym.stream, defDone[f]);
       const int64_t pf = prevFork(f);
-      if (dueStream && pf >= 0 && optDone[pf]) hipCHECK(hipStreamWaitEvent(sym.stream, optDone[pf], 0));
+      if (dueStream && pf >= 0 && optDone[pf]) sym.waitEvent(sym.stream, optDone[pf]);
     };
     bool potrfFused = false;
     bool sideUsed = false, dueUsed = false;
@@ -1318,26 +1361,20 @@
     int extraApplied = 0;
     bool extraBroken = false;
     const bool chunks = &levels == &plan.host.levels && !gatherChunkDone.empty();
-    int waitedExec = 0, waitedDue = 0, waitedSide = 0;
-    hipEvent_t lastOpt = nullptr;
-    auto waitChunk = [&](hipStream_t st, int& waited, int32_t chunk) {
-      if (!chunks || chunk <= waited || chunk >= (int32_t)gatherChunkDone.size()) return;
-      hipCHECK(hipStreamWaitEvent(st, gatherChunkDone[chunk], 0));
-      waited = chunk;
+    PoolEvent lastOpt;
+    auto waitChunk = [&](hipStream_t st, int32_t chunk) {
+      if (!chunks || chunk <= 0 || chunk >= (int32_t)gatherChunkDone.size()) return;
+      sym.waitEvent(st, gatherChunkDone[chunk]);
     };
     for (size_t li = 0; li < levels.size(); li++) {
       const LevelRange& lr = levels[li];
       const unsigned nP = (unsigned)(lr.panelEnd - lr.panelBegin);
       const unsigned nT = (unsigned)(lr.trsmEnd - lr.trsmBegin);
       const bool direct = lr.directPanel >= 0;
-      waitChunk(sym.stream, waitedExec, lr.gatherNow);
+      waitChunk(sym.stream, lr.gatherNow);
       if (lr.tail) {
         if (lr.tail == 1) {
-          auto joinStream = [&](hipStream_t st) {
-            hipEvent_t e = sym.eventFromPool();
-            hipCHECK(hipEventRecord(e, st));
-            hipCHECK(hipStreamWaitEvent(sym.stream, e, 0));
-          };
+          auto joinStream = [&](hipStream_t st) { sym.waitEvent(sym.stream, sym.recordEvent(st)); };
           if (sideUsed) joinStream(sym.sideStream());
           if (dueUsed) joinStream(sym.dueSideStream());
           sideUsed = dueUsed = false;
@@ -1451,44 +1488,42 @@
       }
       const bool anyDef = lr.defEnd > lr.defBegin;
       auto forkSide = [&]() {
-        hipEvent_t fork = sym.eventFromPool();
-        hipCHECK(hipEventRecord(fork, sym.stream));
-        hipCHECK(hipStreamWaitEvent(sym.sideStream(), fork, 0));
+        const PoolEvent fork = sym.recordEvent(sym.stream);
+        sym.waitEvent(sym.sideStream(), fork);
         sym.counters.lookaheadForks++;
         if (dueStream) {
           hipStream_t due = sym.dueSideStream();
-          hipCHECK(hipStreamWaitEvent(due, fork, 0));
-          waitChunk(due, waitedDue, lr.gatherDue);
-          waitChunk(sym.sideStream(), waitedSide, lr.gatherOpt);
-          if (lr.flushDue && lastOpt) hipCHECK(hipStreamWaitEvent(due, lastOpt, 0));
+          sym.waitEvent(due, fork);
+          waitChunk(due, lr.gatherDue);
+          waitChunk(sym.sideStream(), lr.gatherOpt);
+          if (lr.flushDue && lastOpt) sym.waitEvent(due, lastOpt);
           const int64_t f2 = lr.optWaitLevel;
-          if (f2 >= 0 && optDone[f2]) hipCHECK(hipStreamWaitEvent(due, optDone[f2], 0));
+          if (f2 >= 0 && optDone[f2]) sym.waitEvent(due, optDone[f2]);
           if (lr.defMid > lr.defBegin) {
             timer.begin(kProfUpdate, due);
             launchUpdate(plan, lr.defBegin, lr.defMid, ref, due, nullptr, 0, sym.dueExtraLds, sideMask);
             timer.end();
           }
-          defDone[li] = sym.eventFromPool();
-          hipCHECK(hipEventRecord(defDone[li], due));
+          if (lr.defWaited || sym.streamOrderBypass) defDone[li] = sym.recordEvent(due);
           if (lr.defEnd > lr.defMid) {
             timer.begin(kProfUpdate, sym.sideStream());
             launchUpdate(plan, lr.defMid, lr.defEnd, ref, sym.sideStream(), nullptr, 0, sym.bulkExtraLds, sideMask);
             timer.end();
-            optDone[li] = sym.eventFromPool();
-            hipCHECK(hipEventRecord(optDone[li], sym.sideStream()));
-            lastOpt = optDone[li];
+            if (lr.optWaited || sym.streamOrderBypass) {
+              optDone[li] = sym.recordEvent(sym.sideStream());
+              lastOpt = optDone[li];
+            }
           }
           sideUsed = dueUsed = true;
           return;
         }
-        waitChunk(sym.sideStream(), waitedSide, std::max(lr.gatherDue, lr.gatherOpt));
+        waitChunk(sym.sideStream(), std::max(lr.gatherDue, lr.gatherOpt));
         if (lr.defMid > lr.defBegin) {
           timer.begin(kProfUpdate, sym.sideStream());
           launchUpdate(plan, lr.defBegin, lr.defMid, ref, sym.sideStream(), nullptr, 0, sym.bulkExtraLds, sideMask);
           timer.end();
         }
-        defDone[li] = sym.eventFromPool();
-        hipCHECK(hipEventRecord(defDone[li], sym.sideStream()));
+        if (lr.defWaited || sym.streamOrderBypass) defDone[li] = sym.recordEvent(sym.sideStream());
         if (lr.defEnd > lr.defMid) {
           timer.begin(kProfUpdate, sym.sideStream());
           launchUpdate(plan, lr.defMid, lr.defEnd, ref, sym.sideStream(), nullptr, 0, sym.bulkExtraLds, sideMask);
@@ -1581,18 +1616,10 @@
           plan.foldDescs.as<PanelDesc>(), ref);
       timer.end();
     }
-    if (sideUsed) {
-      hipEvent_t join = sym.eventFromPool();
-      hipCHECK(hipEventRecord(join, sym.sideStream()));
-      hipCHECK(hipStreamWaitEvent(sym.stream, join, 0));
-    }
-    if (dueUsed) {
-      hipEvent_t join = sym.eventFromPool();
-      hipCHECK(hipEventRecord(join, sym.dueSideStream()));
-      hipCHECK(hipStreamWaitEvent(sym.stream, join, 0));
-    }
+    if (sideUsed) sym.waitEvent(sym.stream, sym.recordEvent(sym.sideStream(), false));
+    if (dueUsed) sym.waitEvent(sym.stream, sym.recordEvent(sym.dueSideStream(), false));
     if (chunks) {
-      waitChunk(sym.stream, waitedExec, (int32_t)gatherChunkDone.size() - 1);
+      waitChunk(sym.stream, (int32_t)gatherChunkDone.size() - 1);
       gatherChunkDone.clear();
     }
   }
@@ -1644,15 +1671,12 @@
                              plan.host.lookaheadPays(batchSize, sym.lookaheadMinFlops);
         if (overlap) {
           hipStream_t gs = sym.streams().batch[0];
-          hipEvent_t factored = sym.eventFromPool();
-          hipCHECK(hipEventRecord(factored, sym.stream));
-          hipCHECK(hipStreamWaitEvent(gs, factored, 0));
+          sym.waitEvent(gs, sym.recordEvent(sym.stream));
           gatherRange(er.chunkItemPtr[0], er.chunkItemPtr[1], sym.stream);
-          gatherChunkDone.assign(nChunks, nullptr);
+          gatherChunkDone.assign(nChunks, {});
           for (size_t c = 1; c < nChunks; c++) {
             gatherRange(er.chunkItemPtr[c], er.chunkItemPtr[c + 1], gs, sym.gatherOverlapLds);
-            gatherChunkDone[c] = sym.eventFromPool();
-            hipCHECK(hipEventRecord(gatherChunkDone[c], gs));
+            gatherChunkDone[c] = sym.recordEvent(gs);
           }
           sym.counters.gatherChunksOverlapped += (int64_t)nChunks - 1;
         } else {
@@ -1701,8 +1725,7 @@
       const int total = batchSize;
       const int parts = std::max(2, std::min({sym.subBatchParts, 4, total / std::max(1, sym.subBatchMin / 2)}));
       hipStream_t mainStream = sym.stream;
-      hipEvent_t fork = sym.eventFromPool();
-      hipCHECK(hipEventRecord(fork, mainStream));
+      const auto fork = sym.recordEvent(mainStream, false);
       struct Restore {
         HipNumericCtx& c;
         hipStream_t st;
@@ -1719,15 +1742,13 @@
         subBatchBase = b0;
         batchSize = b1 - b0;
         sym.stream = g ? sym.streams().batch[g - 1] : mainStream;
-        if (g) hipCHECK(hipStreamWaitEvent(sym.stream, fork, 0));
+        if (g) sym.waitEvent(sym.stream, fork);
         sym.counters.subBatchesEnqueued++;
         hipk::DataRef<BT> sub{nullptr, ref.many + subBatchBase};
         for (const ElimRangePlan& er : plan.host.elimRanges) launchElim(plan, er, sub, timer);
         launchLevels(plan, plan.host.levels, sub, timer);
         if (g) {
-          hipEvent_t join = sym.eventFromPool();
-          hipCHECK(hipEventRecord(join, sym.stream));
-          hipCHECK(hipStreamWaitEvent(mainStream, join, 0));
+          sym.waitEvent(mainStream, sym.recordEvent(sym.stream, false));
         }
       }
       return;
@@ -1884,7 +1905,7 @@
   HipSymbolicCtx& sym;
   int batchSize;
   int subBatchBase = 0, subBatchTotal = 0;
-  vector<hipEvent_t> gatherChunkDone;
+  vector<typename HipSymbolicCtx::PoolEvent> gatherChunkDone;
   int64_t tempBufSize = 0;
   DevBuf temp, spanToChainOffset;
   vector<std::unique_ptr<DevPlan>> opPlans;
@@ -2606,6 +2627,12 @@
   return out;
 }
 
+void hipBackendSetStreamOrderBypass(SymbolicCtx& sym, bool on) {
+  HipSymbolicCtx* h = dynamic_cast<HipSymbolicCtx*>(&sym);
+  BASPACHO_CHECK_NOTNULL(h);
+  h->streamOrderBypass = on;
+}
+
 void hipBackendSetFault(SymbolicCtx& sym, int kind) {
   HipSymbolicCtx* h = dynamic_cast<HipSymbolicCtx*>(&sym);
   BASPACHO_CHECK_NOTNULL(h);
@@ -2641,6 +2668,8 @@
   c.potrfFoldedLevels = h->counters.potrfFoldedLevels;
   c.selinvLaunches = h->counters.selinvLaunches;
   c.selinvChunks = h->counters.selinvChunks;
+  c.streamWaits = h->counters.streamWaits;
+  c.eventRecords = h->counters.eventRecords;
   c.sweepsRetired = h->sweepBroken ? 1 : 0;
   c.sweepErrorPending = (h->sweepHostErr && *reinterpret_cast<volatile unsigned*>(h->sweepHostErr)) ? 1 : 0;
   return c;
diff --git a/baspacho_amd/csrc/hip_plan.cpp b/baspacho_amd/csrc/hip_plan.cpp
--- a/baspacho_amd/csrc/hip_plan.cpp
+++ b/baspacho_amd/csrc/hip_plan.cpp
@@ -802,6 +802,17 @@
     for (size_t li = 1; li < out.size(); li++) {
       if (out[li].tail == 1) out[li - 1].flushDue = 1;
     }
+    int64_t lastOptLevel = -1;
+    for (size_t li = 0; li < out.size(); li++) {
+      const LevelRange& lr = out[li];
+      if (lr.waitDefLevel >= 0) out[lr.waitDefLevel].defWaited = 1;
+      if (lr.optWaitLevel >= 0) out[lr.optWaitLevel].optWaited = 1;
+      if (lr.waitDefLevel >= 0 && out[lr.waitDefLevel].waitDefLevel >= 0) {
+        out[out[lr.waitDefLevel].waitDefLevel].optWaited = 1;
+      }
+      if (lr.flushDue && lastOptLevel >= 0) out[lastOptLevel].optWaited = 1;
+      if (lr.defEnd > lr.defMid) lastOptLevel = (int64_t)li;
+    }
     for (size_t li = 0; li < out.size(); li++) {
       const LevelRange& lr = out[li];
       const bool directUpd = lr.directPanel >= 0 && lr.directSeg >= 0 && lr.updEnd > lr.updBegin;
diff --git a/baspacho_amd/csrc/hip_plan.h b/baspacho_amd/csrc/hip_plan.h
--- a/baspacho_amd/csrc/hip_plan.h
+++ b/baspacho_amd/csrc/hip_plan.h
@@ -106,6 +106,8 @@
   int32_t gatherNow = -1, gatherDue = -1, gatherOpt = -1;
   int32_t tail = 0, tailPanels = 0;
   int32_t flushDue = 0;
+  int32_t defWaited = 0;
+  int32_t optWaited = 0;
 };
 
 struct ElimGatherItem {
diff --git a/baspacho_amd/csrc/stream_order.h b/baspacho_amd/csrc/stream_order.h
--- /dev/null
+++ b/baspacho_amd/csrc/stream_order.h
@@ -0,0 +1,60 @@
+#pragma once
+
+#include <algorithm>
+#include <array>
+#include <cstdint>
+#include <stdexcept>
+#include <vector>
+
+namespace BaSpaCho {
+
+class StreamOrder {
+ public:
+  static constexpr int kMaxStreams = 8;
+  using Clock = std::array<uint32_t, kMaxStreams>;
+
+  void reset() {
+    streams.clear();
+    events.clear();
+    for (Clock& c : clocks) c.fill(0);
+    counts.fill(0);
+  }
+
+  int streamIndex(const void* handle) {
+    for (size_t i = 0; i < streams.size(); i++) {
+      if (streams[i] == handle) return (int)i;
+    }
+    if ((int)streams.size() == kMaxStreams) throw std::runtime_error("StreamOrder: too many streams in one call");
+    streams.push_back(handle);
+    return (int)streams.size() - 1;
+  }
+
+  int record(int s) {
+    Clock c = clocks[s];
+    c[s] = ++counts[s];
+    events.push_back(Event{s, c});
+    return (int)events.size() - 1;
+  }
+
+  bool wait(int s, int ev) {
+    const Event& e = events[ev];
+    if (e.stream == s) return false;
+    if (clocks[s][e.stream] >= e.clock[e.stream]) return false;
+    for (int t = 0; t < kMaxStreams; t++) {
+      if (t != s) clocks[s][t] = std::max(clocks[s][t], e.clock[t]);
+    }
+    return true;
+  }
+
+ private:
+  struct Event {
+    int stream;
+    Clock clock;
+  };
+  std::vector<const void*> streams;
+  std::vector<Event> events;
+  std::array<Clock, kMaxStreams> clocks = {};
+  std::array<uint32_t, kMaxStreams> counts = {};
+};
+
+}
diff --git a/include/baspacho_amd.h b/include/baspacho_amd.h
--- a/include/baspacho_amd.h
+++ b/include/baspacho_amd.h
@@ -43,6 +43,7 @@
   int32_t chain_contraction;
   int32_t dense_merge;
   int32_t expected_batch;
+  int32_t device_scope_events;
   double lookahead_min_gf;
   double bulk_ahead;
   double level_cost_us;
@@ -300,6 +301,11 @@
   int64_t selinv_chunks;
 } bsp_run_counters;
 int bsp_run_counters_get(bsp_solver* s, bsp_run_counters* out);
+typedef struct bsp_stream_counters {
+  int64_t stream_waits;
+  int64_t event_records;
+} bsp_stream_counters;
+int bsp_stream_counters_get(bsp_solver* s, bsp_stream_counters* out);
 
 enum {
   BSP_PROF_ELIM_FACTOR = 0,
diff --git a/include/baspacho_amd_testing.h b/include/baspacho_amd_testing.h
--- a/include/baspacho_amd_testing.h
+++ b/include/baspacho_amd_testing.h
@@ -16,6 +16,10 @@
 
 int bsp_test_read_sweep_trace(bsp_solver* s, long long* out, int32_t max_blocks, int32_t* n_blocks);
 
+int bsp_test_set_stream_order_bypass(bsp_solver* s, int32_t on);
+
+int bsp_test_stream_order(const int32_t* ops, int64_t n, int32_t* out);
+
 #ifdef __cplusplus
 }
 #endif
diff --git a/profiles/bulk_boundaries.py b/profiles/bulk_boundaries.py
--- /dev/null
+++ b/profiles/bulk_boundaries.py
@@ -0,0 +1,26 @@
+import glob
+import sqlite3
+import sys
+
+f = (glob.glob(sys.argv[1] + '/*/*.db') + glob.glob(sys.argv[1] + '/*.db'))[0]
+min_grid = int(sys.argv[2]) if len(sys.argv) > 2 else 1000
+db = sqlite3.connect(f)
+rows = db.execute("select name,start,end,stream_id,grid_x,workgroup_x from kernels order by start").fetchall()
+idx = [i for i, r in enumerate(rows) if 'elimFactor' in r[0]]
+gmax = max(rows[i][4] for i in idx)
+heads = [i for i in idx if rows[i][4] == gmax]
+pick = min(4, len(heads) - 2)
+seg = rows[heads[pick]:heads[pick + 1]]
+for s in sorted(set(r[3] for r in seg)):
+    ks = [r for r in seg if r[3] == s]
+    bulk = [i for i, r in enumerate(ks) if 'updateTileBulk' in r[0] and r[4] // max(1, r[5]) >= min_grid]
+    d = [(ks[b][1] - ks[a][2]) / 1e3 for a, b in zip(bulk, bulk[1:]) if b == a + 1]
+    back = [x for x in d if x < 30.0]
+    if not d:
+        continue
+    print("stream %d: %d large updateTileBulk launches, %d consecutive pairs" % (s, len(bulk), len(d)))
+    print("  end-to-start us: " + " ".join("%.1f" % x for x in d))
+    if back:
+        back.sort()
+        print("  back-to-back pairs (< 30 us): %d, min %.1f median %.1f max %.1f, sum %.1f us" % (
+            len(back), back[0], back[len(back) // 2], back[-1], sum(back)))
```
